# MCG-NKU/E2FGVI

Hardware: AMD Instinct MI355X
Metric: inpainted frames/sec at 432x240 T=10 (higher is better)
Workload: dtype f32; 1 GPU; BASELINE.json configs[1]: e2fgvi 432x240 T=10 l_t=10, 1 clip(s) per GPU per forward (1 in the job), random-init weights, torch.rand frames + box mask (SURVEY.md 8d); clips_per_gpu=1, precision=fp32, kernel_selection=e2fgvi_amd/tile_table.py (checked in, deterministic: ops.py), hip_graph=True, forwards_in_flight=2

## Files before the change

### e2fgvi_amd/csrc/attention_x3.hip

```cpp
#include "common.h"
#include <stdlib.h>

namespace {

constexpr int HD = 128, NH = 4, CQ = 1536, CP = 1024;
constexpr int WS0 = 5, WS1 = 9, WTOK = 45, SLOTS = 210;
constexpr int TK = 32;
constexpr float LOG2E = 1.4426950408889634f;
constexpr int X_KB = TK * HD * 2;
constexpr int X_STAGE = 6 * X_KB;

typedef __bf16 bf16x8 __attribute__((ext_vector_type(8)));
typedef unsigned int u32x4 __attribute__((ext_vector_type(4)));
typedef __attribute__((address_space(3))) void x_lds_void;
typedef int x_i32x4 __attribute__((ext_vector_type(4)));
typedef short s16x4 __attribute__((ext_vector_type(4)));
typedef short s16x8 __attribute__((ext_vector_type(8)));
typedef __attribute__((address_space(3))) s16x4 x_lds_s16x4;

__device__ __forceinline__ void x_dma16(x_i32x4 rsrc, unsigned lds_dst, unsigned voff) {
    unsigned keep;
    asm volatile("s_nop 4\n\ts_mov_b32 %0, m0\n\ts_mov_b32 m0, %3\n\ts_nop 0\n\tbuffer_load_dwordx4 %1, %2, 0 offen lds\n\ts_mov_b32 m0, %0"
                 : "=&s"(keep) : "v"(voff), "s"(rsrc), "s"(lds_dst) : "memory");
}
__device__ __forceinline__ x_i32x4 x_rsrc_words(const void* base, unsigned bytes) {
    const unsigned long long b = (unsigned long long)base;
    x_i32x4 r;
    r[0] = __builtin_amdgcn_readfirstlane((int)(unsigned)b);
    r[1] = __builtin_amdgcn_readfirstlane((int)((unsigned)(b >> 32) & 0xFFFFu));
    r[2] = __builtin_amdgcn_readfirstlane((int)bytes);
    r[3] = 0x00020000;
    return r;
}

__device__ __forceinline__ void x_split8(const f32x4& v0, const f32x4& v1, bf16x8& hi, bf16x8& mid, bf16x8& lo) {
    e2_split8(v0, v1, hi, mid, lo);
}

__global__ void split3_kv_kernel(const float* __restrict__ src, unsigned short* __restrict__ planes, long long rows) {
    const long long idx = (long long)blockIdx.x * blockDim.x + threadIdx.x;
    if (idx >= rows * (CP / 8)) return;
    const long long row = idx / (CP / 8);
    const int c8 = (int)(idx - row * (CP / 8)) * 8;
    const float* s = src + row * CQ + 512 + c8;
    bf16x8 hi, mid, lo;
    x_split8(*reinterpret_cast<const f32x4*>(s), *reinterpret_cast<const f32x4*>(s + 4), hi, mid, lo);
    const long long plane = rows * CP;
    unsigned short* o = planes + row * CP + c8;
    *reinterpret_cast<bf16x8*>(o) = hi;
    *reinterpret_cast<bf16x8*>(o + plane) = mid;
    *reinterpret_cast<bf16x8*>(o + 2 * plane) = lo;
}

template <int NW, int KS>
__global__ __launch_bounds__(64 * NW * KS, 1) void focal_attn_x3_kernel(const float* __restrict__ qkv, const int* __restrict__ key_tab,
                                                                  int tab_ld, const int* __restrict__ nkeys,
                                                                  float* __restrict__ out, int B, int T, int fh, int fw,
                                                                  const char* planes, unsigned planes_bytes, unsigned plane_stride,
                                                                  unsigned pooled_row0) {
#if defined(__HIP_DEVICE_COMPILE__)
    constexpr int NT = 64 * NW;
    constexpr int PIECES = 8 / NW;
    constexpr unsigned OOB = 0xFFFFF000u;
    static_assert(NW == 2 || NW == 4 || NW == 8, "waves per workgroup");
    constexpr int RING = KS == 1 ? 2 * X_STAGE : 9 * X_KB;
    __shared__ __attribute__((aligned(1024))) unsigned char smem[KS * RING];
    __shared__ int stab[256];
    extern __shared__ __attribute__((aligned(16))) unsigned ktab[];

    const int kg = (KS == 1) ? 0 : __builtin_amdgcn_readfirstlane((int)(threadIdx.x / NT));
    const int tid = threadIdx.x - kg * NT;
    const int lane = tid & 63, wave = __builtin_amdgcn_readfirstlane(tid >> 6);
    const int i = lane & 31, h = lane >> 5;
    const int nWw = fw / WS1, nWh = fh / WS0, nWin = nWh * nWw;
    const int nqc = (T * WTOK + 32 * NW - 1) / (32 * NW);
    const int logical = (int)blockIdx.x;
    const int qchunk = logical % nqc;
    const int wh = (logical / nqc) % (nWin * NH);
    const int b = logical / (nqc * nWin * NH);
    const int win = wh / NH, head = wh - win * NH;
    const int wy = win / nWw, wx = win - wy * nWw;
    const int NQ = T * WTOK;
    const int ntok = fh * fw;
    const x_i32x4 rsrc = x_rsrc_words(planes, planes_bytes);

    const int nv = nkeys[win];
    const int NK = T * nv;
    const int ntiles = (NK + TK - 1) / TK;
    const int nIter = (ntiles + KS - 1) / KS;
    const int* tab = key_tab + (long long)win * tab_ld;
    for (int e = threadIdx.x; e < nv && e < 256; e += KS * NT) stab[e] = tab[e];
    __syncthreads();
    {
        int t = 0, sl = threadIdx.x;
        while (sl >= nv) { sl -= nv; ++t; }
        const unsigned head_off = (unsigned)(head * HD * 2);
        for (int k = threadIdx.x; k < KS * nIter * TK; k += KS * NT) {
            unsigned e = OOB;
            if (k < NK) {
                const int ref = stab[sl];
                const bool pooled = ref < 0;
                const unsigned rowi = pooled ? pooled_row0 + (unsigned)((b * T + t) * nWin + (-(ref + 1))) : (unsigned)((b * T + t) * ntok + ref);
                e = rowi * (unsigned)(CP * 2) + head_off;
            }
            ktab[k] = e;
            sl += KS * NT;
            while (sl >= nv) { sl -= nv; ++t; }
        }
    }
    __syncthreads();

    const int q0 = (qchunk * NW + wave) * 32;
// ... 175 lines not shown
        const unsigned char* const ring = smem + kg * RING;
        issue_half(kg, 0u, false);
        issue_half(kg, 6u * X_KB, true);
        asm volatile("s_waitcnt vmcnt(0)" ::: "memory");
        __syncthreads();
        int cur = 0;
        if (kg == 1) __syncthreads();
        for (int itr = 0; itr < nIter; ++itr) {
            const int kt = kg + itr * KS;
            const bool more = itr + 1 < nIter;
            if (more) issue_half(kt + KS, (unsigned)((cur ^ 1) * 3 * X_KB), false);
            if (wave_active) s_phase(ring + cur * 3 * X_KB, kt);
            if (more) asm volatile("s_waitcnt vmcnt(%0)" ::"n"(3 * PIECES) : "memory");
            else asm volatile("s_waitcnt vmcnt(0)" ::: "memory");
            __syncthreads();
            if (wave_active) pv_phase(ring + 6 * X_KB);
            asm volatile("s_waitcnt vmcnt(0)" ::: "memory");
            __syncthreads();
            if (more) issue_half(kt + KS, 6u * X_KB, true);
            cur ^= 1;
        }
        if (kg == 0) __syncthreads();
        float* scr = reinterpret_cast<float*>(smem + RING);
        if (kg > 0) {
            scr[tid] = m_run;
            scr[NT + tid] = l_run;
#pragma unroll
            for (int dt = 0; dt < 4; ++dt)
#pragma unroll
                for (int r = 0; r < 16; ++r) scr[(2 + dt * 16 + r) * NT + tid] = acc[dt][r];
        }
        __syncthreads();
        if (kg > 0) return;
        {
            const float m_o = scr[tid], l_o = scr[NT + tid];
            const float m_new = fmaxf(m_run, m_o);
            const float a0 = __builtin_amdgcn_exp2f(m_run - m_new), a1 = __builtin_amdgcn_exp2f(m_o - m_new);
            l_run = l_run * a0 + l_o * a1;
            m_run = m_new;
#pragma unroll
            for (int dt = 0; dt < 4; ++dt)
#pragma unroll
                for (int r = 0; r < 16; ++r) acc[dt][r] = acc[dt][r] * a0 + scr[(2 + dt * 16 + r) * NT + tid] * a1;
        }
    }

    if (wave_active) {
        float l = l_run + __shfl_xor(l_run, 32);
        const float nmask = (float)(T * (SLOTS - nv));
        l = add_pad_mass(l, nmask, m_run);
        const float inv = 1.f / l;
        bool ok;
        const long long row = query_row(ok);
        if (ok) {
            float* op = out + row * (NH * HD) + head * HD;
#pragma unroll
            for (int dt = 0; dt < 4; ++dt)
#pragma unroll
                for (int rq = 0; rq < 4; ++rq) {
                    const f32x4 v = {acc[dt][rq * 4 + 0] * inv, acc[dt][rq * 4 + 1] * inv, acc[dt][rq * 4 + 2] * inv, acc[dt][rq * 4 + 3] * inv};
                    *reinterpret_cast<f32x4*>(op + dt * 32 + 8 * rq + 4 * h) = v;
                }
        }
    }
#endif
}

}

extern "C" int e2fgvi_split3_kv(const float* qkv_rows, void* planes, int64_t rows, void* stream) {
    E2_REQUIRE(qkv_rows && planes && rows > 0, E2FGVI_EINVAL, "split3_kv: null pointer / no rows");
    E2_REQUIRE(((uintptr_t)qkv_rows & 15) == 0 && ((uintptr_t)planes & 15) == 0, E2FGVI_EINVAL, "split3_kv: buffers must be 16-byte aligned");
    const long long items = rows * (CP / 8);
    hipLaunchKernelGGL(split3_kv_kernel, dim3((unsigned)cdiv64(items, 256)), dim3(256), 0, (hipStream_t)stream, qkv_rows,
                       (unsigned short*)planes, (long long)rows);
    E2_LAUNCH_CHECK("split3_kv");
    return 0;
}

extern "C" int e2fgvi_focal_attention_x3(const float* qkv, const void* planes, const int32_t* key_tab, int32_t tab_ld,
                                         const int32_t* nkeys, float* out, int32_t B, int32_t T, int32_t fh, int32_t fw,
                                         int32_t waves, void* stream) {
    E2_REQUIRE(qkv && planes && key_tab && nkeys && out, E2FGVI_EINVAL, "focal_attention_x3: null pointer");
    E2_REQUIRE(B > 0 && T > 0 && fh > 0 && fw > 0 && fh % WS0 == 0 && fw % WS1 == 0, E2FGVI_EINVAL,
               "focal_attention_x3: token grid %dx%d must be a positive multiple of (5,9)", fh, fw);
    E2_REQUIRE(tab_ld >= SLOTS, E2FGVI_EINVAL, "focal_attention_x3: tab_ld < 210");
    E2_REQUIRE(((uintptr_t)qkv & 15) == 0 && ((uintptr_t)planes & 15) == 0 && ((uintptr_t)out & 15) == 0, E2FGVI_EINVAL,
               "focal_attention_x3: buffers must be 16-byte aligned");
    const int nWin = (fh / WS0) * (fw / WS1);
    const long long rows = (long long)B * T * fh * fw + (long long)B * T * nWin;
    const long long plane_bytes = rows * CP * 2;
    E2_REQUIRE(3 * plane_bytes < 0xFFFFF000LL, E2FGVI_EUNSUP, "focal_attention_x3: the three k / v planes span >= 4 GiB (split the batch)");
    int ks = 1;
    if (waves == 14) { ks = 2; waves = 4; }
    const int ntiles = cdiv(T * SLOTS, TK);
    size_t dyn = (size_t)ntiles * TK * 4;
    const size_t dyn2 = (size_t)cdiv(ntiles, 2) * 2 * TK * 4;
    const bool fits2 = dyn2 + 2 * 9 * X_KB + 1024 + 256 <= 160 * 1024;
    E2_REQUIRE(dyn + 2 * X_STAGE + 1024 + 256 <= 160 * 1024, E2FGVI_EUNSUP, "focal_attention_x3: window of %d frames does not fit the LDS key table", T);
    if (waves <= 0) {
        const long long wg4 = (long long)cdiv(T * WTOK, 128) * nWin * NH * B;
        const long long qblocks = (long long)cdiv(T * WTOK, 32) * nWin * NH * B;
        waves = wg4 >= 512 ? 8 : 4;
        if (wg4 < 192) waves = 2;
        if (waves == 4 && qblocks < 2048 && fits2) ks = 2;
    }
    E2_REQUIRE(waves == 2 || waves == 4 || waves == 8, E2FGVI_EINVAL, "focal_attention_x3: waves must be 0, 2, 4, 8 or 14");
    E2_REQUIRE(ks == 1 || fits2, E2FGVI_EUNSUP, "focal_attention_x3: two key groups do not fit the LDS for a window of %d frames", T);
    if (ks == 2) dyn = dyn2;
    const long long nblk = (long long)cdiv(T * WTOK, 32 * waves) * nWin * NH * B;
    E2_REQUIRE(nblk < 2147483647LL, E2FGVI_EUNSUP, "focal_attention_x3: more than 2^31 workgroups");
    dim3 grid((unsigned)nblk), block(64 * waves * ks);
#define E2_ATT_X3(NW_, KS_)                                                                                                       \
    do {                                                                                                                          \
        hipError_t ea = hipFuncSetAttribute((const void*)focal_attn_x3_kernel<NW_, KS_>, hipFuncAttributeMaxDynamicSharedMemorySize, \
                                            (int)dyn);                                                                            \
        E2_REQUIRE(ea == hipSuccess, (int)ea, "focal_attention_x3: cannot reserve %zu bytes of dynamic LDS", dyn);                \
        hipLaunchKernelGGL((focal_attn_x3_kernel<NW_, KS_>), grid, block, dyn, (hipStream_t)stream, qkv, key_tab, tab_ld, nkeys, out, \
                           B, T, fh, fw, (const char*)planes, (unsigned)(3 * plane_bytes), (unsigned)plane_bytes,                 \
                           (unsigned)((long long)B * T * fh * fw));                                                               \
    } while (0)
    if (ks == 2) E2_ATT_X3(4, 2);
    else if (waves == 2) E2_ATT_X3(2, 1);
    else if (waves == 4) E2_ATT_X3(4, 1);
    else E2_ATT_X3(8, 1);
#undef E2_ATT_X3
    E2_LAUNCH_CHECK("focal_attention_x3");
    return 0;
}
```

### e2fgvi_amd/csrc/common.h

```cpp
#pragma once
#include <hip/hip_runtime.h>
#include <stdint.h>
#include <stdio.h>
#include <stdarg.h>

#include "../../include/e2fgvi_hip.h"

typedef float f32x4 __attribute__((ext_vector_type(4)));
typedef float f32x16 __attribute__((ext_vector_type(16)));

void e2fgvi_set_error(const char* fmt, ...);

#define E2_REQUIRE(cond, code, ...)            \
    do {                                       \
        if (!(cond)) {                         \
            e2fgvi_set_error(__VA_ARGS__);     \
            return (code);                     \
        }                                      \
    } while (0)

#define E2_LAUNCH_CHECK(name)                                                        \
    do {                                                                             \
        hipError_t e__ = hipGetLastError();                                          \
        if (e__ != hipSuccess) {                                                     \
// ... 6 lines not shown
static inline int64_t cdiv64(int64_t a, int64_t b) { return (a + b - 1) / b; }
static inline int round_up(int a, int b) { return cdiv(a, b) * b; }

template <int TM, int TN, int BK, int LDA, int BN>
__device__ __forceinline__ void mma_ktile(const float* __restrict__ sA, const float* __restrict__ sB,
                                          f32x16 (&acc)[TM][TN], int a_row0, int b_col0, int lane) {
    const int i = lane & 31, h = lane >> 5;
#pragma unroll
    for (int m8 = 0; m8 < BK / 8; ++m8) {
        f32x4 a[TM], b[TN];
#pragma unroll
        for (int tm = 0; tm < TM; ++tm)
            a[tm] = *reinterpret_cast<const f32x4*>(sA + (a_row0 + tm * 32 + i) * LDA + (2 * m8 + h) * 4);
#pragma unroll
        for (int tn = 0; tn < TN; ++tn)
            b[tn] = *reinterpret_cast<const f32x4*>(sB + ((2 * m8 + h) * BN + b_col0 + tn * 32 + i) * 4);
#pragma unroll
        for (int e = 0; e < 4; ++e)
#pragma unroll
            for (int tm = 0; tm < TM; ++tm)
#pragma unroll
                for (int tn = 0; tn < TN; ++tn)
                    acc[tm][tn] = __builtin_amdgcn_mfma_f32_32x32x2f32(a[tm][e], b[tn][e], acc[tm][tn], 0, 0, 0);
    }
}

__device__ __forceinline__ int xcd_remap(int bid, int nblk) {
    const int q = nblk >> 3, r = nblk & 7;
    const int xcd = bid & 7, idx = bid >> 3;
    return (xcd < r ? xcd * (q + 1) : r * (q + 1) + (xcd - r) * q) + idx;
}

__device__ __forceinline__ float e2_fast_sigmoid(float x) {
    return __builtin_amdgcn_rcpf(1.f + __builtin_amdgcn_exp2f(-1.4426950408889634f * x));
}
__device__ __forceinline__ float e2_fast_tanh(float x) {
    return 1.f - 2.f * __builtin_amdgcn_rcpf(1.f + __builtin_amdgcn_exp2f(2.8853900817779268f * x));
}

__device__ __forceinline__ float add_pad_mass(float l, float nmask, float m_run) {
    if (nmask > 0.f) l += nmask * __builtin_amdgcn_exp2f(-100.f * 1.4426950408889634f - m_run);
    return l;
}

__device__ __forceinline__ void e2_split2(float x0, float x1, unsigned& H, unsigned& M, unsigned& L) {
    const unsigned b0 = __builtin_bit_cast(unsigned, x0), b1 = __builtin_bit_cast(unsigned, x1);
    const float r0 = x0 - __builtin_bit_cast(float, b0 & 0xFFFF0000u), r1 = x1 - __builtin_bit_cast(float, b1 & 0xFFFF0000u);
    const unsigned rb0 = __builtin_bit_cast(unsigned, r0), rb1 = __builtin_bit_cast(unsigned, r1);
    const float s0 = r0 - __builtin_bit_cast(float, rb0 & 0xFFFF0000u), s1 = r1 - __builtin_bit_cast(float, rb1 & 0xFFFF0000u);
    H = __builtin_amdgcn_perm(b1, b0, 0x07060302u);
    M = __builtin_amdgcn_perm(rb1, rb0, 0x07060302u);
    L = __builtin_amdgcn_perm(__builtin_bit_cast(unsigned, s1), __builtin_bit_cast(unsigned, s0), 0x07060302u);
}
typedef __bf16 e2_bf16x8 __attribute__((ext_vector_type(8)));
typedef unsigned int e2_u32x4 __attribute__((ext_vector_type(4)));
__device__ __forceinline__ void e2_split8(const f32x4& v0, const f32x4& v1, e2_bf16x8& hi, e2_bf16x8& mid, e2_bf16x8& lo) {
    float x[8];
#pragma unroll
    for (int j = 0; j < 4; ++j) { x[j] = v0[j]; x[4 + j] = v1[j]; }
    e2_u32x4 H, M, L;
#pragma unroll
    for (int j = 0; j < 4; ++j) {
        unsigned h, m, l;
        e2_split2(x[2 * j], x[2 * j + 1], h, m, l);
        H[j] = h; M[j] = m; L[j] = l;
    }
    hi = __builtin_bit_cast(e2_bf16x8, H);
    mid = __builtin_bit_cast(e2_bf16x8, M);
    lo = __builtin_bit_cast(e2_bf16x8, L);
}

typedef _Float16 e2_f16x8 __attribute__((ext_vector_type(8)));
template <bool F16> struct e2_h16;
template <> struct e2_h16<false> { typedef __bf16 T; typedef e2_bf16x8 V8; };
template <> struct e2_h16<true> { typedef _Float16 T; typedef e2_f16x8 V8; };
__device__ __forceinline__ f32x16 e2_mfma16(e2_bf16x8 a, e2_bf16x8 b, f32x16 c) {
    return __builtin_amdgcn_mfma_f32_32x32x16_bf16(a, b, c, 0, 0, 0);
}
__device__ __forceinline__ f32x16 e2_mfma16(e2_f16x8 a, e2_f16x8 b, f32x16 c) {
    return __builtin_amdgcn_mfma_f32_32x32x16_f16(a, b, c, 0, 0, 0);
}
template <bool F16> __device__ __forceinline__ float e2_h16_to_f32(unsigned short b) {
    if constexpr (F16) return (float)__builtin_bit_cast(_Float16, b);
    else return __builtin_bit_cast(float, (unsigned)b << 16);
}

__device__ __forceinline__ float apply_act(float v, int act, float slope) {
    if (act == E2FGVI_ACT_RELU) return fmaxf(v, 0.f);
    if (act == E2FGVI_ACT_LRELU) return v > 0.f ? v : v * slope;
    if (act == E2FGVI_ACT_TANH) return tanhf(v);
    return v;
}
```

### e2fgvi_amd/csrc/conv_bf16x.hip

```cpp
#include "common.h"

namespace {

typedef __bf16 bf16x8 __attribute__((ext_vector_type(8)));
typedef unsigned int u32x4 __attribute__((ext_vector_type(4)));
typedef __attribute__((address_space(3))) void lds_void;

struct ConvXParams {
    const void* src[E2FGVI_MAX_SRC];
    int ld[E2FGVI_MAX_SRC];
    int coff[E2FGVI_MAX_SRC];
    int cpg[E2FGVI_MAX_SRC];
    unsigned src_bytes[E2FGVI_MAX_SRC];
    int nsrc;
    int N, H, W, Ho, Wo, KH, KW, stride, pad;
    int padx;
    int osy, osx, opy, opx, oH, oW;
    int res_bcast;
    int Cout, Cout_g, Npad;
    int M;
    int tilesM, tilesN;
    int nsteps;
    unsigned wgroup_bytes;
    long long wgroup_elems;
    const void* w;
    const float* bias;
    const void* res;
    int res_ld, res_coff, res_bf16;
    void* dst;
    int dst_ld, dst_coff, dst_bf16, dst_nchw;
    __bf16* dst2;
    int dst2_ld, dst2_coff;
    int split_from;
    long long split_plane;
    int act;
    float slope;
    int tp_cq;
    unsigned tp_magic;
    unsigned tp_magic_cq;
    int dbg_noload;
};

__device__ __forceinline__ __amdgpu_buffer_rsrc_t make_rsrc(const void* base, unsigned bytes) {
    return __builtin_amdgcn_make_buffer_rsrc(const_cast<void*>(base), 0, (int)bytes, 0x00020000);
}

__device__ __forceinline__ float dcn_post(float v, int co, int C, const f32x4& fl, float max_residue) {
    const int noff = (C / 3) * 2;
    if (co >= noff) return e2_fast_sigmoid(v);
    const int which = (co * 2 >= noff) ? 2 : 0;
    return max_residue * e2_fast_tanh(v) + fl[which + ((co & 1) ? 0 : 1)];
}


__device__ __forceinline__ void split8(const f32x4& v0, const f32x4& v1, bf16x8& hi, bf16x8& mid, bf16x8& lo) {
    e2_split8(v0, v1, hi, mid, lo);
}

typedef int pp_i32x4 __attribute__((ext_vector_type(4)));
__device__ __forceinline__ pp_i32x4 pp_rsrc_words(const void* base, unsigned bytes) {
    const unsigned long long b = (unsigned long long)base;
    pp_i32x4 r;
    r[0] = __builtin_amdgcn_readfirstlane((int)(unsigned)b);
    r[1] = __builtin_amdgcn_readfirstlane((int)((unsigned)(b >> 32) & 0xFFFFu));
    r[2] = __builtin_amdgcn_readfirstlane((int)bytes);
    r[3] = 0x00020000;
    return r;
}
__device__ __forceinline__ void pp_dma16(pp_i32x4 rsrc, unsigned lds_dst, unsigned voff, unsigned soff) {
    unsigned keep;
    asm volatile("s_nop 4\n\ts_mov_b32 %0, m0\n\ts_mov_b32 m0, %3\n\ts_nop 0\n\tbuffer_load_dwordx4 %1, %2, %4 offen lds\n\ts_mov_b32 m0, %0"
                 : "=&s"(keep) : "v"(voff), "s"(rsrc), "s"(lds_dst), "s"(soff) : "memory");
}

template <int BM, int BN, int WGM, int WGN, bool S3, int MODE, bool PP = false>
__global__ __launch_bounds__(64 * WGM * WGN) void conv_bf16x_kernel(const ConvXParams p) {
#if defined(__HIP_DEVICE_COMPILE__)
    constexpr bool F32 = MODE == 1, X3 = MODE == 2, F16 = MODE == 3;
    typedef typename e2_h16<F16>::T E16;
    typedef typename e2_h16<F16>::V8 e16x8;
    static_assert(!PP || (X3 && !S3 && WGM * WGN == 8), "ping-pong halves: split-operand mode, 8 waves, no row-shift stages");
    constexpr int NT = 64 * WGM * WGN;
    constexpr int ESZ = (F32 || X3) ? 4 : 2;
    constexpr int CH = 16 / ESZ;
    constexpr int KC = 8 * CH;
    constexpr int TM = BM / (32 * WGM), TN = BN / (32 * WGN);
    constexpr int AR = S3 ? BM + 2 : BM;
    constexpr int B_CH = X3 ? 12 : 8;
    constexpr int A_BYTES = AR * 128, B_BYTES = BN * B_CH * 16;
    constexpr int A_IT = (AR * 8 + NT - 1) / NT, B_IT = (BN * B_CH + NT - 1) / NT;
    constexpr bool A_PART = (AR * 8) % NT != 0;
    constexpr bool B_PART = (BN * B_CH) % NT != 0;
    constexpr int R = TM * 32, CN = TN * 32;
    constexpr int ES = (WGM * WGN * R * (CN + 4) * 4 <= 150 * 1024) ? 1 : (TN % 2 == 0 ? 2 : TN);
    constexpr int TNH = TN / ES, CNH = CN / ES, LDE = CNH + 4;
    constexpr int EPI = WGM * WGN * R * LDE * 4;
    static_assert(TN % ES == 0 && EPI <= 160 * 1024, "epilogue region");
    constexpr int SMEM = 2 * (A_BYTES + B_BYTES) > EPI ? 2 * (A_BYTES + B_BYTES) : EPI;
    constexpr unsigned OOB = 0xFFFFFFFFu;
    static_assert(TM >= 1 && TN >= 1 && (BM * 8) % NT == 0 && (BN * B_CH) % 64 == 0 && SMEM <= 160 * 1024, "tile");

    __shared__ __attribute__((aligned(1024))) unsigned char smem[SMEM];

    const int tid = threadIdx.x;
    const int lane = tid & 63, wave = __builtin_amdgcn_readfirstlane(tid >> 6);
    const int wm = wave / WGN, wn = wave % WGN;
    const int g = blockIdx.y;
    const int logical = xcd_remap(blockIdx.x, p.tilesM * p.tilesN);
    const int tile_m = logical / p.tilesN, tile_n = logical - tile_m * p.tilesN;
    const int m0 = tile_m * BM, n0 = tile_n * BN;
    const int HoWo = p.Ho * p.Wo;

    int a_pix[A_IT];
    unsigned a_msk[A_IT];
    unsigned a_ch16[A_IT];
#pragma unroll
    for (int it = 0; it < A_IT; ++it) {
        const int item = tid + it * NT;
        const int row = item >> 3, slot = item & 7;
        a_ch16[it] = (unsigned)((slot ^ ((row >> 1) & 7)) * 16);
        const int m = S3 ? m0 + row - 1 : m0 + row;
        const bool ok = m >= 0 && m < p.M;
        const int mm = ok ? m : 0;
        const int img = mm / HoWo;
        const int rem = mm - img * HoWo;
        const int oy = rem / p.Wo, ox = rem - oy * p.Wo;
        const int by = oy * p.stride - p.pad;
        const int bx = S3 ? ox : ox * p.stride - p.padx;
        unsigned msk = 0;
        for (int k = 0; k < p.KH; ++k) msk |= ((unsigned)(by + k) < (unsigned)p.H ? 1u : 0u) << k;
        for (int k = 0; k < (S3 ? 1 : p.KW); ++k) msk |= ((unsigned)(bx + k) < (unsigned)p.W ? 1u : 0u) << (8 + k);
        a_msk[it] = ok ? msk : 0u;
        a_pix[it] = (img * p.H + by) * p.W + bx;
    }
    unsigned b_off[B_IT];
#pragma unroll
    for (int it = 0; it < B_IT; ++it) {
        const int item = tid + it * NT;
        const int koct = item / BN, n = item - koct * BN;
        b_off[it] = ((n0 + n) < p.Npad && koct < B_CH) ? (unsigned)((koct * p.Npad + n0 + n) * 16) : OOB;
    }
    const __amdgpu_buffer_rsrc_t wrsrc = make_rsrc(reinterpret_cast<const char*>(p.w) + (long long)g * p.wgroup_bytes, p.wgroup_bytes);
    const unsigned b_step = (unsigned)B_CH * (unsigned)p.Npad * 16u;

    const void* const sp0 = p.src[0]; const void* const sp1 = p.src[1]; const void* const sp2 = p.src[2]; const void* const sp3 = p.src[3];
    const unsigned sb0 = p.src_bytes[0], sb1 = p.src_bytes[1], sb2 = p.src_bytes[2], sb3 = p.src_bytes[3];
    const unsigned sl0 = (unsigned)p.ld[0] * ESZ, sl1 = (unsigned)p.ld[1] * ESZ, sl2 = (unsigned)p.ld[2] * ESZ, sl3 = (unsigned)p.ld[3] * ESZ;
    const unsigned sc0 = (unsigned)(p.coff[0] + g * p.cpg[0]) * ESZ, sc1 = (unsigned)(p.coff[1] + g * p.cpg[1]) * ESZ,
                   sc2 = (unsigned)(p.coff[2] + g * p.cpg[2]) * ESZ, sc3 = (unsigned)(p.coff[3] + g * p.cpg[3]) * ESZ;
    const int sg0 = p.cpg[0], sg1 = p.cpg[1], sg2 = p.cpg[2], sg3 = p.cpg[3];
    int ky = 0, kx = 0, s = 0, c0 = 0;
    int blk = 0;
    const void* cur_src = sp0;
    unsigned cur_bytes = sb0;
    unsigned cur_ld2 = sl0, cur_chan = sc0;
    int cur_cpg = sg0;
    unsigned a_off[A_IT];
    auto retarget = [&]() {
        if (p.nsrc > 1) {
            cur_src = s == 0 ? sp0 : s == 1 ? sp1 : s == 2 ? sp2 : sp3;
            cur_bytes = s == 0 ? sb0 : s == 1 ? sb1 : s == 2 ? sb2 : sb3;
            cur_ld2 = s == 0 ? sl0 : s == 1 ? sl1 : s == 2 ? sl2 : sl3;
            cur_chan = s == 0 ? sc0 : s == 1 ? sc1 : s == 2 ? sc2 : sc3;
            cur_cpg = s == 0 ? sg0 : s == 1 ? sg1 : s == 2 ? sg2 : sg3;
        }
        const int kxe = S3 ? 0 : kx;
        const int tap = ky * p.W + kxe;
#pragma unroll
        for (int it = 0; it < A_IT; ++it) {
            const bool ok = ((a_msk[it] >> ky) & (a_msk[it] >> (8 + kxe)) & 1u) != 0;
            a_off[it] = ok ? (unsigned)(a_pix[it] + tap) * cur_ld2 + cur_chan + a_ch16[it] : OOB;
        }
    };
    retarget();
    unsigned char* const smem_b = smem + 2 * A_BYTES;
    auto issue_a = [&](int stage) {
        if (p.dbg_noload & 16) return;
        unsigned char* sa = smem + stage * A_BYTES + wave * 1024;
        const __amdgpu_buffer_rsrc_t arsrc = make_rsrc(cur_src, cur_bytes);
        const unsigned soff = (unsigned)c0 * (unsigned)ESZ;
        if (c0 + KC <= cur_cpg) {
#pragma unroll
            for (int it = 0; it < A_IT; ++it)
                if (!A_PART || it + 1 < A_IT || tid + it * NT < AR * 8)
                    __builtin_amdgcn_raw_ptr_buffer_load_lds(arsrc, (lds_void*)(sa + it * NT * 16), 16, a_off[it], soff, 0, 0);
        } else {
#pragma unroll
            for (int it = 0; it < A_IT; ++it)
                if (!A_PART || it + 1 < A_IT || tid + it * NT < AR * 8)
                    __builtin_amdgcn_raw_ptr_buffer_load_lds(arsrc, (lds_void*)(sa + it * NT * 16), 16,
                                                             (c0 + (int)(a_ch16[it] / ESZ) < cur_cpg) ? a_off[it] : OOB, soff, 0, 0);
        }
    };
    auto issue_b = [&](int stage, int step) {
        if (p.dbg_noload & 32) return;
        unsigned char* sb = smem_b + stage * B_BYTES + wave * 1024;
        const unsigned soff = (unsigned)step * b_step;
#pragma unroll
        for (int it = 0; it < B_IT; ++it)
            if (!B_PART || it + 1 < B_IT || tid + it * NT < BN * B_CH)
                __builtin_amdgcn_raw_ptr_buffer_load_lds(wrsrc, (lds_void*)(sb + it * NT * 16), 16, b_off[it], soff, 0, 0);
    };
    auto advance = [&]() -> bool {
        c0 += KC;
        ++blk;
        if (c0 < cur_cpg) return false;
        c0 = 0;
        ++s;
        if (s == p.nsrc) {
            s = 0;
            blk = 0;
            if (S3) ++ky;
            else { ++kx; if (kx == p.KW) { kx = 0; ++ky; } }
        }
        return true;
    };

    f32x16 acc[TM][TN];
#pragma unroll
    for (int tm = 0; tm < TM; ++tm)
#pragma unroll
        for (int tn = 0; tn < TN; ++tn)
#pragma unroll
            for (int r = 0; r < 16; ++r) acc[tm][tn][r] = 0.f;

    const int i = lane & 31, h = lane >> 5;
    int a_row[TM], b_rd[TN];
    bool okl[TM], okr[TM];
#pragma unroll
    for (int tm = 0; tm < TM; ++tm) {
        a_row[tm] = (wm * TM + tm) * 32 + i;
        const int ox = (m0 + a_row[tm]) % p.Wo;
        okl[tm] = ox != 0;
        okr[tm] = ox != p.Wo - 1;
    }
#pragma unroll
    for (int tn = 0; tn < TN; ++tn) b_rd[tn] = ((wn * TN + tn) * 32 + i) * 16;

    auto compute = [&](const unsigned char* st, const unsigned char* stb, int kxs) {
        int a_rd[TM], a_key[TM];
        bool zero[TM];
#pragma unroll
        for (int tm = 0; tm < TM; ++tm) {
            const int row = a_row[tm] + (S3 ? kxs : 0);
            a_rd[tm] = row * 128;
            a_key[tm] = (row >> 1) & 7;
            zero[tm] = S3 && ((kxs == 0 && !okl[tm]) || (kxs == 2 && !okr[tm]));
        }
        if constexpr (X3) {
#pragma unroll
            for (int kk = 0; kk < 2; ++kk) {
                const int q = 2 * kk + h;
                bf16x8 ah[TM], am[TM], al[TM];
#pragma unroll
                for (int tm = 0; tm < TM; ++tm)
                    split8(*reinterpret_cast<const f32x4*>(st + a_rd[tm] + (((2 * q) ^ a_key[tm]) << 4)),
                           *reinterpret_cast<const f32x4*>(st + a_rd[tm] + (((2 * q + 1) ^ a_key[tm]) << 4)), ah[tm], am[tm], al[tm]);
#pragma unroll
                for (int tn = 0; tn < TN; ++tn) {
                    const bf16x8 bh = *reinterpret_cast<const bf16x8*>(stb + b_rd[tn] + q * (BN * 16));
                    const bf16x8 bm = *reinterpret_cast<const bf16x8*>(stb + b_rd[tn] + (4 + q) * (BN * 16));
                    const bf16x8 bl = *reinterpret_cast<const bf16x8*>(stb + b_rd[tn] + (8 + q) * (BN * 16));
#pragma unroll
                    for (int tm = 0; tm < TM; ++tm) acc[tm][tn] = __builtin_amdgcn_mfma_f32_32x32x16_bf16(al[tm], bh, acc[tm][tn], 0, 0, 0);
#pragma unroll
                    for (int tm = 0; tm < TM; ++tm) acc[tm][tn] = __builtin_amdgcn_mfma_f32_32x32x16_bf16(ah[tm], bl, acc[tm][tn], 0, 0, 0);
#pragma unroll
                    for (int tm = 0; tm < TM; ++tm) acc[tm][tn] = __builtin_amdgcn_mfma_f32_32x32x16_bf16(am[tm], bm, acc[tm][tn], 0, 0, 0);
#pragma unroll
                    for (int tm = 0; tm < TM; ++tm) acc[tm][tn] = __builtin_amdgcn_mfma_f32_32x32x16_bf16(am[tm], bh, acc[tm][tn], 0, 0, 0);
#pragma unroll
                    for (int tm = 0; tm < TM; ++tm) acc[tm][tn] = __builtin_amdgcn_mfma_f32_32x32x16_bf16(ah[tm], bm, acc[tm][tn], 0, 0, 0);
#pragma unroll
                    for (int tm = 0; tm < TM; ++tm) acc[tm][tn] = __builtin_amdgcn_mfma_f32_32x32x16_bf16(ah[tm], bh, acc[tm][tn], 0, 0, 0);
                }
            }
        } else {
#pragma unroll
        for (int kk = 0; kk < 4; ++kk) {
            if constexpr (F32) {
                f32x4 a[TM], b[TN];
#pragma unroll
                for (int tm = 0; tm < TM; ++tm)
                    a[tm] = *reinterpret_cast<const f32x4*>(st + a_rd[tm] + (((2 * kk + h) ^ a_key[tm]) << 4));
#pragma unroll
                for (int tn = 0; tn < TN; ++tn)
                    b[tn] = *reinterpret_cast<const f32x4*>(stb + b_rd[tn] + (2 * kk + h) * (BN * 16));
#pragma unroll
                for (int e = 0; e < 4; ++e)
#pragma unroll
                    for (int tm = 0; tm < TM; ++tm)
#pragma unroll
                        for (int tn = 0; tn < TN; ++tn)
                            acc[tm][tn] = __builtin_amdgcn_mfma_f32_32x32x2f32(a[tm][e], b[tn][e], acc[tm][tn], 0, 0, 0);
            } else {
                e16x8 a[TM], b[TN];
#pragma unroll
                for (int tm = 0; tm < TM; ++tm) {
                    a[tm] = *reinterpret_cast<const e16x8*>(st + a_rd[tm] + (((2 * kk + h) ^ a_key[tm]) << 4));
                    if (S3) {
                        u32x4 q = __builtin_bit_cast(u32x4, a[tm]);
#pragma unroll
                        for (int e = 0; e < 4; ++e) q[e] = zero[tm] ? 0u : q[e];
                        a[tm] = __builtin_bit_cast(e16x8, q);
                    }
                }
#pragma unroll
                for (int tn = 0; tn < TN; ++tn)
                    b[tn] = *reinterpret_cast<const e16x8*>(stb + b_rd[tn] + (2 * kk + h) * (BN * 16));
#pragma unroll
// ... 58 lines not shown
                for (int tm = 0; tm < TM; ++tm) acc[tm][tn] = __builtin_amdgcn_mfma_f32_32x32x16_bf16(fa[tm][0], bh, acc[tm][tn], 0, 0, 0);
                __builtin_amdgcn_sched_barrier(0);
            }
        };
        const unsigned smem_lds = (unsigned)(unsigned long long)(lds_void*)smem;
        const pp_i32x4 wrsrc_w = pp_rsrc_words(reinterpret_cast<const char*>(p.w) + (long long)g * p.wgroup_bytes, p.wgroup_bytes);
        auto pp_issue = [&](int stage, int step) __attribute__((always_inline)) {
            const pp_i32x4 arsrc_w = pp_rsrc_words(cur_src, cur_bytes);
            const unsigned soff = (unsigned)__builtin_amdgcn_readfirstlane(c0 * ESZ);
            const unsigned la = smem_lds + (unsigned)(stage * A_BYTES + wave * 1024);
            const bool whole = c0 + KC <= cur_cpg;
#pragma unroll
            for (int it = 0; it < A_IT; ++it)
                pp_dma16(arsrc_w, (unsigned)__builtin_amdgcn_readfirstlane((int)(la + it * NT * 16)),
                         (whole || c0 + (int)(a_ch16[it] / ESZ) < cur_cpg) ? a_off[it] : OOB, soff);
            const unsigned lb = smem_lds + (unsigned)(2 * A_BYTES + stage * B_BYTES + wave * 1024);
            const unsigned sb = (unsigned)__builtin_amdgcn_readfirstlane((int)((unsigned)step * b_step));
#pragma unroll
            for (int it = 0; it < B_IT; ++it)
                if (!B_PART || it + 1 < B_IT || tid + it * NT < BN * B_CH)
                    pp_dma16(wrsrc_w, (unsigned)__builtin_amdgcn_readfirstlane((int)(lb + it * NT * 16)), b_off[it], sb);
        };
        if (trail) pp_bar();
        for (int step = 0; step < p.nsteps; ++step) {
            const int cur = step & 1;
            const unsigned char* const sA = smem + cur * A_BYTES;
            const unsigned char* const sB = smem_b + cur * B_BYTES;
            if (trail) { if (step + 1 < p.nsteps) { if (advance()) retarget(); pp_issue((step & 1) ^ 1, step + 1); } }
            prep(sA, 0);
            pp_bar();
            mma(sB, 0);
            pp_bar();
            prep(sA, 1);
            if (!trail) { if (step + 1 < p.nsteps) { if (advance()) retarget(); pp_issue((step & 1) ^ 1, step + 1); } }
            if (trail) asm volatile("s_waitcnt vmcnt(0)" ::: "memory");
            pp_bar();
            mma(sB, 1);
            if (!trail) asm volatile("s_waitcnt vmcnt(0)" ::: "memory");
            pp_bar();
        }
        if (!trail) pp_bar();
    } else
    if constexpr (!S3) {
        if (p.tp_cq) {
            const int cq = p.tp_cq, KK = p.KH * p.KW;
            int t_c[A_IT];
#pragma unroll
            for (int it = 0; it < A_IT; ++it) t_c[it] = (int)(a_ch16[it] >> 4);
            const __amdgpu_buffer_rsrc_t arsrc = make_rsrc(sp0, sb0);
            auto issue_a_packed = [&](int stage, int step) {
                unsigned char* sa = smem + stage * A_BYTES + wave * 1024;
#pragma unroll
                for (int it = 0; it < A_IT; ++it) {
                    const int L = 8 * step + t_c[it];
                    const int tap = cq == 1 ? L : (int)__umulhi((unsigned)L, p.tp_magic_cq);
                    const int cc = L - tap * cq;
                    const int tky = (int)__umulhi((unsigned)tap, p.tp_magic), tkx = tap - tky * p.KW;
                    const bool ok = tap < KK && ((a_msk[it] >> tky) & (a_msk[it] >> (8 + tkx)) & 1u) != 0;
                    const unsigned off = ok ? (unsigned)(a_pix[it] + tky * p.W + tkx) * sl0 + sc0 + (unsigned)cc * 16u : OOB;
                    __builtin_amdgcn_raw_ptr_buffer_load_lds(arsrc, (lds_void*)(sa + it * NT * 16), 16, off, 0, 0, 0);
                }
            };
            issue_a_packed(0, 0);
            asm volatile("s_waitcnt vmcnt(0)" ::: "memory");
            __syncthreads();
            for (int step = 0; step < p.nsteps; ++step) {
                const int cur = step & 1;
                if (step + 1 < p.nsteps) {
                    issue_a_packed(cur ^ 1, step + 1);
                    issue_b(cur ^ 1, step + 1);
                }
                compute(smem + cur * A_BYTES, smem_b + cur * B_BYTES, 0);
                asm volatile("s_waitcnt vmcnt(0)" ::: "memory");
                __syncthreads();
            }
        } else
        for (int step = 0; step < p.nsteps; ++step) {
            const int cur = step & 1;
            const bool more = step + 1 < p.nsteps && !(p.dbg_noload & 1);
            if (more) {
                if (advance()) retarget();
                issue_a(cur ^ 1);
                issue_b(cur ^ 1, step + 1);
            }
            compute(smem + cur * A_BYTES, smem_b + cur * B_BYTES, 0);
            asm volatile("s_waitcnt vmcnt(0)" ::: "memory");
            __syncthreads();
        }
    } else if constexpr (!S3) {
        for (int step = 0; step < p.nsteps; ++step) {
            const int cur = step & 1;
            const bool more = step + 1 < p.nsteps && !(p.dbg_noload & 1);
            if (more) {
                if (advance()) retarget();
                issue_a(cur ^ 1);
                issue_b(cur ^ 1, step + 1);
            }
            compute(smem + cur * A_BYTES, smem_b + cur * B_BYTES, 0);
            asm volatile("s_waitcnt vmcnt(0)" ::: "memory");
            __syncthreads();
        }
    } else {
        const int spt = p.nsteps / 9;
        int acur = 0, kxs = 0;
        for (int step = 0; step < p.nsteps; ++step) {
            const bool more = step + 1 < p.nsteps && !(p.dbg_noload & 1);
            int kxn = kxs + 1;
            bool newblk = false;
            if (kxn == 3) {
                kxn = 0;
                if (more) { if (advance()) retarget(); newblk = true; }
            }
// ... 282 lines not shown
    if (idx >= p.total) return;
    const int g = (int)(idx / p.wgroup_elems);
    long long rem = idx - (long long)g * p.wgroup_elems;
    const int e = (int)(rem % p.ch);
    rem /= p.ch;
    const int n = (int)(rem % p.Npad);
    rem /= p.Npad;
    const int koct = (int)(rem & 7);
    const int step = (int)(rem >> 3);
    wp[idx] = (T)pack_value(w, p, g, step, koct, n, e);
}

__global__ void pack_conv_weight_x3_kernel(const float* __restrict__ w, unsigned short* __restrict__ wp, const PackX p) {
    const long long idx = (long long)blockIdx.x * blockDim.x + threadIdx.x;
    if (idx >= p.total) return;
    const int g = (int)(idx / p.wgroup_elems);
    long long rem = idx - (long long)g * p.wgroup_elems;
    const int e = (int)(rem & 3);
    rem >>= 2;
    const int n = (int)(rem % p.Npad);
    rem /= p.Npad;
    const int koct = (int)(rem & 7);
    const int step = (int)(rem >> 3);
    const float v = pack_value(w, p, g, step, koct, n, e);
    const unsigned xb = __builtin_bit_cast(unsigned, v);
    const float r = v - __builtin_bit_cast(float, xb & 0xFFFF0000u);
    const unsigned rb = __builtin_bit_cast(unsigned, r);
    const float r2 = r - __builtin_bit_cast(float, rb & 0xFFFF0000u);
    const long long plane = 4LL * p.Npad * 8;
    unsigned short* o = wp + (long long)g * p.wgroup_elems * 3 + (long long)step * 3 * plane +
                        ((long long)(koct >> 1) * p.Npad + n) * 8 + (koct & 1) * 4 + e;
    o[0] = (unsigned short)(xb >> 16);
    o[plane] = (unsigned short)(rb >> 16);
    o[2 * plane] = (unsigned short)(__builtin_bit_cast(unsigned, r2) >> 16);
}

template <int BM, int BN, int WGM, int WGN, bool S3, bool PP = false>
int launch_x(ConvXParams& p, int groups, hipStream_t st, int mode = 0) {
    p.tilesM = cdiv(p.M, BM);
    p.tilesN = cdiv(p.Cout_g, BN);
    if constexpr (PP) {
        if (mode != 2 || p.tp_cq) {
            e2fgvi_set_error("conv2d_x: the ping-pong tiles (107, 108) are for the split-operand mode without tap-packed weights");
            return E2FGVI_EUNSUP;
        }
        hipLaunchKernelGGL((conv_bf16x_kernel<BM, BN, WGM, WGN, false, 2, true>), dim3(p.tilesM * p.tilesN, groups, 1), dim3(64 * WGM * WGN), 0, st, p);
        E2_LAUNCH_CHECK("conv2d_x");
        return 0;
    } else {
    if (S3 && !(p.KH == 3 && p.KW == 3 && p.stride == 1 && p.pad == 1)) {
        e2fgvi_set_error("conv2d_x: the row-shift tiles (11..17) are for 3x3 stride-1 pad-1 layers");
        return E2FGVI_EINVAL;
    }
    if (mode == 1 || mode == 2) {
        if constexpr (!S3) {
            if (mode == 2)
                hipLaunchKernelGGL((conv_bf16x_kernel<BM, BN, WGM, WGN, false, 2>), dim3(p.tilesM * p.tilesN, groups, 1), dim3(64 * WGM * WGN), 0, st, p);
            else
                hipLaunchKernelGGL((conv_bf16x_kernel<BM, BN, WGM, WGN, false, 1>), dim3(p.tilesM * p.tilesN, groups, 1), dim3(64 * WGM * WGN), 0, st, p);
        } else {
            e2fgvi_set_error("conv2d_x: the row-shift tiles (11..18) take bf16 operands only");
            return E2FGVI_EUNSUP;
        }
    } else if (mode == 3) {
        hipLaunchKernelGGL((conv_bf16x_kernel<BM, BN, WGM, WGN, S3, 3>), dim3(p.tilesM * p.tilesN, groups, 1), dim3(64 * WGM * WGN), 0, st, p);
    } else {
        hipLaunchKernelGGL((conv_bf16x_kernel<BM, BN, WGM, WGN, S3, 0>), dim3(p.tilesM * p.tilesN, groups, 1), dim3(64 * WGM * WGN), 0, st, p);
    }
    E2_LAUNCH_CHECK("conv2d_x");
    return 0;
    }
}

}

static bool geometry_taps(int Cout, int KH, int KW, int cin, PackX* q, bool f32 = false) {
    const int32_t cpg[1] = {cin};
    if (cin > 56 || KW < 2 || !geometry_x(Cout, 1, KH, KW, 1, cpg, q, f32)) return false;
    q->tp_cq = cin / q->ch;
    const int steps = cdiv(KH * KW * q->tp_cq, 8);
    q->wgroup_elems = (long long)steps * q->kc * q->Npad;
    q->total = q->wgroup_elems;
    return true;
}

static int mode_x(const char* who, int32_t code) {
    switch (code) {
        case E2FGVI_BF16: return 0;
        case E2FGVI_F32: return 1;
        case E2FGVI_BF16X3: return 2;
        case E2FGVI_F16: return 3;
        default: break;
    }
    e2fgvi_set_error("%s: mode %d is none of E2FGVI_F32 (0), E2FGVI_BF16 (1), E2FGVI_BF16X3 (2), E2FGVI_F16 (3)", who, code);
    return -1;
}

static bool pack_geometry(const char* who, int mode, int tap_packed, int Cout, int groups, int KH, int KW, int nsrc,
                          const int32_t* src_cpg, PackX* q) {
    const bool f32 = mode == 1 || mode == 2;
    const int ch = f32 ? 4 : 8;
    if (!src_cpg) {
        e2fgvi_set_error("%s: null src_cpg", who);
        return false;
    }
    if (tap_packed) {
        if (groups == 1 && nsrc == 1 && geometry_taps(Cout, KH, KW, src_cpg[0], q, f32)) return true;
        e2fgvi_set_error("%s: tap-packed weights: one source of %d ... 56 channels (multiple of %d), no groups, KW >= 2", who, ch, ch);
        return false;
    }
    if (geometry_x(Cout, groups, KH, KW, nsrc, src_cpg, q, f32)) return true;
    e2fgvi_set_error("%s: bad geometry (channels per source must be multiples of %d)", who, ch);
    return false;
}

extern "C" int64_t e2fgvi_packed_conv_weight_x_size(int32_t mode, int32_t tap_packed, int32_t Cout, int32_t groups, int32_t KH,
                                                    int32_t KW, int32_t nsrc, const int32_t* src_cpg) {
    PackX q;
    const int m = mode_x("packed_conv_weight_x_size", mode);
    if (m < 0 || !pack_geometry("packed_conv_weight_x_size", m, tap_packed, Cout, groups, KH, KW, nsrc, src_cpg, &q)) return E2FGVI_EINVAL;
    return m == 2 ? 3 * q.total : q.total;
}

extern "C" int e2fgvi_pack_conv_weight_x(const float* w, void* wpacked, int32_t mode, int32_t tap_packed, int32_t Cout, int32_t groups,
                                         int32_t KH, int32_t KW, int32_t nsrc, const int32_t* src_cpg, void* stream) {
    PackX q;
    E2_REQUIRE(w && wpacked, E2FGVI_EINVAL, "pack_conv_weight_x: null pointer");
    const int m = mode_x("pack_conv_weight_x", mode);
    if (m < 0 || !pack_geometry("pack_conv_weight_x", m, tap_packed, Cout, groups, KH, KW, nsrc, src_cpg, &q)) return E2FGVI_EINVAL;
    const dim3 grid((unsigned)cdiv64(q.total, 256)), block(256);
    hipStream_t st = (hipStream_t)stream;
    switch (m) {
        case 0: hipLaunchKernelGGL(pack_conv_weight_x_kernel<__bf16>, grid, block, 0, st, w, (__bf16*)wpacked, q); break;
        case 1: hipLaunchKernelGGL(pack_conv_weight_x_kernel<float>, grid, block, 0, st, w, (float*)wpacked, q); break;
        case 2: hipLaunchKernelGGL(pack_conv_weight_x3_kernel, grid, block, 0, st, w, (unsigned short*)wpacked, q); break;
        default: hipLaunchKernelGGL(pack_conv_weight_x_kernel<_Float16>, grid, block, 0, st, w, (_Float16*)wpacked, q); break;
    }
    E2_LAUNCH_CHECK("pack_conv_weight_x");
    return 0;
}

static int conv2d_x(const e2fgvi_convx_desc* d, void* stream, int mode) {
    const bool f32 = mode == 1 || mode == 2;
    const int dt16 = mode == 3 ? E2FGVI_F16 : E2FGVI_BF16;
    E2_REQUIRE(d, E2FGVI_EINVAL, "conv2d_x: null descriptor");
    PackX q;
    const int esz = f32 ? 4 : 2;
    const int wbytes_num = mode == 2 ? 6 : esz;
    E2_REQUIRE(geometry_x(d->Cout, d->groups, d->KH, d->KW, d->nsrc, d->src_cpg, &q, f32), E2FGVI_EINVAL,
               "conv2d_x: bad geometry (channels per source must be multiples of 8 bf16 / 4 fp32)");
    E2_REQUIRE(d->N > 0 && d->H > 0 && d->W > 0 && d->Ho > 0 && d->Wo > 0 && d->stride > 0 && d->pad >= 0, E2FGVI_EINVAL,
               "conv2d_x: bad sizes");
    if (d->out_grid) {
        E2_REQUIRE(d->pad_left >= 0 && d->act != E2FGVI_ACT_DCNPOST && !d->dst_nchw && !d->tap_packed && (d->tile < 10 || d->tile > 20),
                   E2FGVI_EINVAL, "conv2d_x: explicit output grids take plain NHWC tiles only");
        if (d->out_sy || d->out_sx)
            E2_REQUIRE(d->out_sy > 0 && d->out_sx > 0 && d->out_py >= 0 && d->out_px >= 0 && d->out_H > 0 && d->out_W > 0 &&
                       (d->Ho - 1) * d->out_sy + d->out_py < d->out_H && (d->Wo - 1) * d->out_sx + d->out_px < d->out_W &&
                       (long long)d->N * d->out_H * d->out_W < 2147483647LL,
                       E2FGVI_EINVAL, "conv2d_x: the output scatter leaves the [N, out_H, out_W] image");
    } else {
        E2_REQUIRE(d->Ho == (d->H + 2 * d->pad - d->KH) / d->stride + 1 && d->Wo == (d->W + 2 * d->pad - d->KW) / d->stride + 1,
                   E2FGVI_EINVAL, "conv2d_x: Ho/Wo inconsistent with H/W/k/stride/pad");
        E2_REQUIRE(!d->out_sy && !d->out_sx && !d->pad_left, E2FGVI_EINVAL, "conv2d_x: pad_left / out_s* need out_grid = 1");
    }
    E2_REQUIRE(!d->res_bcast || (d->residual && d->act != E2FGVI_ACT_DCNPOST), E2FGVI_EINVAL, "conv2d_x: res_bcast without a residual");
    E2_REQUIRE((long long)d->N * d->Ho * d->Wo < 2147483647LL, E2FGVI_EUNSUP, "conv2d_x: more than 2^31 output pixels");
    E2_REQUIRE(d->KH <= 8 && d->KW <= 8, E2FGVI_EUNSUP, "conv2d_x: kernels larger than 8x8 are not supported");
    E2_REQUIRE(d->wpacked && d->dst, E2FGVI_EINVAL, "conv2d_x: null weight/dst");
    E2_REQUIRE((d->dst_dtype == E2FGVI_F32 || d->dst_dtype == dt16) && (d->res_dtype == E2FGVI_F32 || d->res_dtype == dt16),
               E2FGVI_EINVAL, mode == 3 ? "conv2d_x: dtype must be E2FGVI_F32 or E2FGVI_F16"
                                        : "conv2d_x: dtype must be E2FGVI_F32 or E2FGVI_BF16");
    ConvXParams p;
    for (int s = 0; s < E2FGVI_MAX_SRC; ++s) { p.src[s] = nullptr; p.ld[s] = 0; p.coff[s] = 0; p.cpg[s] = 0; p.src_bytes[s] = 0; }
    for (int s = 0; s < d->nsrc; ++s) {
        E2_REQUIRE(d->src[s], E2FGVI_EINVAL, "conv2d_x: null source %d", s);
        E2_REQUIRE(d->src_ld[s] % q.ch == 0 && d->src_coff[s] % q.ch == 0 && ((uintptr_t)d->src[s] & 15) == 0, E2FGVI_EINVAL,
                   "conv2d_x: source %d not 16-byte addressable (ld / coff multiples of 8 bf16 / 4 fp32)", s);
        E2_REQUIRE(d->src_coff[s] + d->groups * d->src_cpg[s] <= d->src_ld[s], E2FGVI_EINVAL,
                   "conv2d_x: source %d channel range exceeds its pixel stride", s);
        const long long bytes = (long long)d->N * d->H * d->W * d->src_ld[s] * esz;
        E2_REQUIRE(bytes < 4294967295LL, E2FGVI_EUNSUP, "conv2d_x: source %d spans >= 4 GiB (split the batch)", s);
        p.src[s] = d->src[s]; p.ld[s] = d->src_ld[s]; p.coff[s] = d->src_coff[s]; p.cpg[s] = d->src_cpg[s];
        p.src_bytes[s] = (unsigned)bytes;
    }
    E2_REQUIRE(q.wgroup_elems * wbytes_num < 4294967295LL, E2FGVI_EUNSUP, "conv2d_x: packed weight group >= 4 GiB");
    E2_REQUIRE(((uintptr_t)d->wpacked & 15) == 0, E2FGVI_EINVAL, "conv2d_x: packed weight not 16-byte aligned");
    if (d->dst_nchw)
        E2_REQUIRE(d->dst_dtype == E2FGVI_F32 && !d->dst2, E2FGVI_EINVAL, "conv2d_x: the NCHW destination is fp32, without a second copy");
    else
        E2_REQUIRE(d->dst_coff >= 0 && d->dst_coff + d->Cout <= d->dst_ld, E2FGVI_EINVAL, "conv2d_x: dst slice exceeds dst_ld");
    E2_REQUIRE(((uintptr_t)d->dst & 15) == 0 && (!d->dst2 || ((uintptr_t)d->dst2 & 15) == 0) &&
               (!d->residual || ((uintptr_t)d->residual & 15) == 0), E2FGVI_EINVAL, "conv2d_x: dst / dst2 / residual not 16-byte aligned");
    E2_REQUIRE(mode != 3 || !d->dst2_plane_stride, E2FGVI_EINVAL, "conv2d_x: no split planes (dst2 is an fp16 copy)");
    if (d->dst2_plane_stride) {
        E2_REQUIRE(d->dst2 && d->dst2_plane_stride > 0 && d->dst_dtype == E2FGVI_F32 && !d->dst_nchw && d->groups == 1 &&
                       !(d->out_grid && d->out_sy), E2FGVI_EINVAL,
                   "conv2d_x: split planes need dst2, an fp32 NHWC dst, groups = 1 and no output scatter");
        E2_REQUIRE(d->Cout % 8 == 0 && d->dst2_split_from >= 0 && d->dst2_split_from <= d->Cout && d->dst2_split_from % 8 == 0 &&
                       d->dst2_ld % 8 == 0 && d->dst2_coff % 8 == 0 && d->dst2_plane_stride % 8 == 0 && d->dst2_coff >= 0 &&
                       d->dst2_coff + d->Cout - d->dst2_split_from <= d->dst2_ld, E2FGVI_EINVAL,
                   "conv2d_x: split planes: Cout, dst2_split_from, dst2_ld, dst2_coff and dst2_plane_stride in multiples of 8, "
                   "the split channels inside dst2_ld");
    } else if (d->dst2)
        E2_REQUIRE(d->dst2_coff >= 0 && d->dst2_coff + d->Cout <= d->dst2_ld, E2FGVI_EINVAL, "conv2d_x: dst2 slice exceeds dst2_ld");
    if (d->act == E2FGVI_ACT_DCNPOST)
        E2_REQUIRE(d->residual && d->res_dtype == E2FGVI_F32 && d->Cout % 3 == 0 && d->groups == 1, E2FGVI_EINVAL,
                   "conv2d_x: ACT_DCNPOST needs the fp32 [pixel][4] flows as residual, Cout %% 3 == 0, groups == 1");
    p.nsrc = d->nsrc;
    p.N = d->N; p.H = d->H; p.W = d->W; p.Ho = d->Ho; p.Wo = d->Wo;
    p.KH = d->KH; p.KW = d->KW; p.stride = d->stride; p.pad = d->pad;
    p.padx = d->out_grid ? d->pad_left : d->pad;
    p.osy = d->out_grid ? d->out_sy : 0; p.osx = d->out_sx; p.opy = d->out_py; p.opx = d->out_px; p.oH = d->out_H; p.oW = d->out_W;
    p.res_bcast = d->res_bcast;
    p.Cout = d->Cout; p.Cout_g = q.Cout_g; p.Npad = q.Npad;
    p.M = d->N * d->Ho * d->Wo;
    p.nsteps = d->KH * d->KW * q.steps_per_tap;
    p.tp_cq = 0; p.tp_magic = 0; p.tp_magic_cq = 0;
    if (d->tap_packed) {
        PackX qt;
        E2_REQUIRE(d->nsrc == 1 && d->groups == 1 && geometry_taps(d->Cout, d->KH, d->KW, d->src_cpg[0], &qt, f32), E2FGVI_EINVAL,
                   "conv2d_x: tap-packed weights are for one source of <= 56 channels, no groups, KW >= 2");
        E2_REQUIRE(d->tile < 10 || d->tile > 20, E2FGVI_EUNSUP, "conv2d_x: the row-shift tiles do not take tap-packed weights");
        q.wgroup_elems = qt.wgroup_elems;
        p.tp_cq = qt.tp_cq;
        p.tp_magic = 0xFFFFFFFFu / (unsigned)d->KW + 1u;
        p.tp_magic_cq = qt.tp_cq > 1 ? 0xFFFFFFFFu / (unsigned)qt.tp_cq + 1u : 0u;
        p.nsteps = cdiv(d->KH * d->KW * qt.tp_cq, 8);
    }
    p.wgroup_elems = q.wgroup_elems; p.wgroup_bytes = (unsigned)(q.wgroup_elems * wbytes_num);
    p.w = d->wpacked; p.bias = d->bias;
    p.res = d->residual; p.res_ld = d->res_ld; p.res_coff = d->res_coff; p.res_bf16 = d->res_dtype == dt16;
    p.dst = d->dst; p.dst_ld = d->dst_ld; p.dst_coff = d->dst_coff; p.dst_bf16 = d->dst_dtype == dt16;
    p.dst_nchw = d->dst_nchw;
    p.dst2 = (__bf16*)d->dst2; p.dst2_ld = d->dst2_ld; p.dst2_coff = d->dst2_coff;
    p.split_from = d->dst2_split_from; p.split_plane = d->dst2_plane_stride;
    p.act = d->act; p.slope = d->slope;
    hipStream_t st = (hipStream_t)stream;
    int tile = d->tile;
    p.dbg_noload = 0;
    if (tile == 21 || tile == 24 || tile == 26 || tile == 27) { p.dbg_noload = 1; tile -= 20; }
    if (tile == 31 || tile == 34 || tile == 36) { p.dbg_noload = 2; tile -= 30; }
    if (tile == 41 || tile == 44 || tile == 46) { p.dbg_noload = 3; tile -= 40; }
    if (tile == 61 || tile == 66) { p.dbg_noload = 8; tile -= 60; }
    if (tile == 71 || tile == 74 || tile == 76 || tile == 77) { p.dbg_noload = 16; tile -= 70; }
    if (tile == 81 || tile == 84 || tile == 86 || tile == 87) { p.dbg_noload = 32; tile -= 80; }
    if (!tile) {
        if (p.Cout_g <= 32) tile = 3;
        else if (p.Cout_g <= 64) tile = 2;
        else tile = ((long long)cdiv(p.M, 128) * cdiv(p.Cout_g, 128) * d->groups >= 384) ? 1 : 4;
    }
    switch (tile) {
        case 1: return launch_x<128, 128, 2, 2, false>(p, d->groups, st, mode);
        case 2: return launch_x<128, 64, 2, 2, false>(p, d->groups, st, mode);
        case 3: return launch_x<128, 32, 4, 1, false>(p, d->groups, st, mode);
        case 4: return launch_x<64, 128, 2, 2, false>(p, d->groups, st, mode);
        case 5: return launch_x<64, 64, 2, 2, false>(p, d->groups, st, mode);
        case 6: return launch_x<256, 128, 4, 2, false>(p, d->groups, st, mode);
        case 7: return launch_x<256, 256, 4, 2, false>(p, d->groups, st, mode);
        case 8: return launch_x<256, 192, 4, 2, false>(p, d->groups, st, mode);
        case 107: return launch_x<256, 256, 4, 2, false, true>(p, d->groups, st, mode);
        case 108: return launch_x<256, 192, 4, 2, false, true>(p, d->groups, st, mode);
        case 11: return launch_x<128, 128, 2, 2, true>(p, d->groups, st, mode);
        case 12: return launch_x<128, 64, 2, 2, true>(p, d->groups, st, mode);
        case 13: return launch_x<128, 32, 4, 1, true>(p, d->groups, st, mode);
        case 14: return launch_x<64, 128, 2, 2, true>(p, d->groups, st, mode);
        case 16: return launch_x<256, 128, 4, 2, true>(p, d->groups, st, mode);
        case 17: return launch_x<256, 256, 4, 2, true>(p, d->groups, st, mode);
        case 18: return launch_x<256, 64, 4, 2, true>(p, d->groups, st, mode);
        default: break;
    }
    e2fgvi_set_error("conv2d_x: unknown tile %d", tile);
    return E2FGVI_EINVAL;
}

extern "C" int e2fgvi_conv2d_x(const e2fgvi_convx_desc* d, int32_t mode, void* stream) {
    const int m = mode_x("conv2d_x", mode);
    return m < 0 ? E2FGVI_EINVAL : conv2d_x(d, stream, m);
}
```

### e2fgvi_amd/csrc/misc.hip

```cpp
#include "common.h"

#include <type_traits>

namespace {

constexpr int NTH = 256;

typedef unsigned int u32x2 __attribute__((ext_vector_type(2)));
typedef __bf16 bf16x4 __attribute__((ext_vector_type(4)));
typedef _Float16 f16x4 __attribute__((ext_vector_type(4)));
typedef _Float16 f16x8 __attribute__((ext_vector_type(8)));
template <typename T> __device__ __forceinline__ f32x4 ld4(const T* p);
template <> __device__ __forceinline__ f32x4 ld4<float>(const float* p) { return *reinterpret_cast<const f32x4*>(p); }
template <> __device__ __forceinline__ f32x4 ld4<__bf16>(const __bf16* p) {
    const u32x2 q = *reinterpret_cast<const u32x2*>(p);
    f32x4 v = {__builtin_bit_cast(float, q[0] << 16), __builtin_bit_cast(float, q[0] & 0xFFFF0000u),
               __builtin_bit_cast(float, q[1] << 16), __builtin_bit_cast(float, q[1] & 0xFFFF0000u)};
    return v;
}
template <> __device__ __forceinline__ f32x4 ld4<_Float16>(const _Float16* p) {
    const f16x4 h = *reinterpret_cast<const f16x4*>(p);
    f32x4 v = {(float)h[0], (float)h[1], (float)h[2], (float)h[3]};
    return v;
}
// ... 690 lines not shown
            hipLaunchKernelGGL((prop_cond_kernel<T, T>), dim3(blocks_for(total)), dim3(NTH), 0, (hipStream_t)stream,
                               (const T*)feat_prop, fp_ld, (const T*)feat_n2, f2_ld, flow_a, flow_b, (long long)flow_img_stride,
                               (T*)cond, flows, (T*)flows8_bf16, N, H, W, C);
    });
    E2_LAUNCH_CHECK("prop_cond");
    return 0;
}

template <typename TO>
static int layernorm_launch(const float* x, const float* gamma, const float* beta, TO* y, int64_t rows, int32_t C, hipStream_t st) {
    const int wpb = 4;
    dim3 grid((unsigned)cdiv64(rows, wpb)), block(64 * wpb);
    switch (C / 256) {
        case 1: hipLaunchKernelGGL((layernorm_kernel<1, TO>), grid, block, 0, st, x, gamma, beta, y, (long long)rows, C); break;
        case 2: hipLaunchKernelGGL((layernorm_kernel<2, TO>), grid, block, 0, st, x, gamma, beta, y, (long long)rows, C); break;
        case 3: hipLaunchKernelGGL((layernorm_kernel<3, TO>), grid, block, 0, st, x, gamma, beta, y, (long long)rows, C); break;
        default: hipLaunchKernelGGL((layernorm_kernel<4, TO>), grid, block, 0, st, x, gamma, beta, y, (long long)rows, C); break;
    }
    E2_LAUNCH_CHECK("layernorm");
    return 0;
}
extern "C" int e2fgvi_layernorm(const float* x, const float* gamma, const float* beta, void* y, int32_t y_dtype, int64_t rows,
                                int32_t C, void* stream) {
    E2_REQUIRE(x && gamma && beta && y && rows > 0 && E2_DT_OK(y_dtype), E2FGVI_EINVAL, "layernorm: bad arguments");
    E2_REQUIRE(C == 256 || C == 512 || C == 768 || C == 1024, E2FGVI_EUNSUP, "layernorm: C must be 256/512/768/1024");
    int rc = 0;
    with_dtype(y_dtype, [&](auto z) { rc = layernorm_launch(x, gamma, beta, (E2_ELEM(z)*)y, rows, C, (hipStream_t)stream); });
    return rc;
}

extern "C" int e2fgvi_window_pool(const void* x, int32_t dtype, const float* w45, const float* bias1, void* pooled,
                                  int32_t BT, int32_t fh, int32_t fw, int32_t C, void* stream) {
    E2_REQUIRE(x && w45 && bias1 && pooled && BT > 0 && fh > 0 && fw > 0 && fh % 5 == 0 && fw % 9 == 0 && C % 4 == 0 &&
                   E2_DT_OK(dtype),
               E2FGVI_EINVAL, "window_pool: bad arguments");
    E2_REQUIRE(dtype == E2FGVI_F32 || C % 8 == 0, E2FGVI_EINVAL, "window_pool: 16-bit needs C %% 8 == 0");
    const long long total = (long long)BT * (fh / 5) * (fw / 9) * (C / (E2_DT16(dtype) ? 8 : 4));
    with_dtype(dtype, [&](auto z) {
        using T = E2_ELEM(z);
        hipLaunchKernelGGL(window_pool_kernel<T>, dim3(blocks_for(total)), dim3(NTH), 0, (hipStream_t)stream,
                           (const T*)x, w45, bias1, (T*)pooled, BT, fh, fw, C);
    });
    E2_LAUNCH_CHECK("window_pool");
    return 0;
}

static int check_fold(const char* name, int F, int fh, int fw, int H, int W, int C) {
    E2_REQUIRE(F > 0 && C > 0 && C % 4 == 0, E2FGVI_EINVAL, "%s: bad arguments", name);
    E2_REQUIRE(fh == (H + 6 - 7) / 3 + 1 && fw == (W + 6 - 7) / 3 + 1, E2FGVI_EINVAL,
               "%s: token grid %dx%d inconsistent with %dx%d", name, fh, fw, H, W);
    return 0;
}

extern "C" int e2fgvi_ffn_fold(const void* hid, void* folded, int32_t dtype, int32_t gelu, int32_t F, int32_t fh, int32_t fw,
                               int32_t H, int32_t W, int32_t C, void* stream) {
    const char* name = gelu ? "ffn_fold_gelu" : "ffn_fold";
    E2_REQUIRE(hid && folded && E2_DT_OK(dtype), E2FGVI_EINVAL, "%s: bad arguments", name);
    if (int rc = check_fold(name, F, fh, fw, H, W, C)) return rc;
    E2_REQUIRE(dtype == E2FGVI_F32 || C % 8 == 0, E2FGVI_EINVAL, "%s: 16-bit needs C %% 8 == 0", name);
    const long long total = (long long)F * H * W * (C / (E2_DT16(dtype) ? 8 : 4));
    with_dtype(dtype, [&](auto z) {
        using T = E2_ELEM(z);
        if (gelu)
            hipLaunchKernelGGL((fold_kernel<true, T, T, T, true>), dim3(blocks_for(total)), dim3(NTH), 0, (hipStream_t)stream,
                               (const T*)hid, (const float*)nullptr, (const T*)nullptr, (T*)folded, F, fh, fw, H, W, C);
        else
            hipLaunchKernelGGL((fold_kernel<true, T, T, T>), dim3(blocks_for(total)), dim3(NTH), 0, (hipStream_t)stream,
                               (const T*)hid, (const float*)nullptr, (const T*)nullptr, (T*)folded, F, fh, fw, H, W, C);
    });
    E2_LAUNCH_CHECK(name);
    return 0;
}

extern "C" int e2fgvi_ffn_unfold(const void* folded, void* out, int32_t dtype, int32_t gelu, int32_t F, int32_t fh, int32_t fw,
                                 int32_t H, int32_t W, int32_t C, void* stream) {
    const char* name = gelu ? "ffn_unfold_gelu" : "ffn_unfold";
    E2_REQUIRE(folded && out && E2_DT_OK(dtype), E2FGVI_EINVAL, "%s: bad arguments", name);
    if (int rc = check_fold(name, F, fh, fw, H, W, C)) return rc;
    E2_REQUIRE(dtype == E2FGVI_F32 || C % 8 == 0, E2FGVI_EINVAL, "%s: 16-bit needs C %% 8 == 0", name);
    const long long total = (long long)F * fh * fw * 49 * (C / (E2_DT16(dtype) ? 8 : 4));
    with_dtype(dtype, [&](auto z) {
        using T = E2_ELEM(z);
        if (gelu)
            hipLaunchKernelGGL(unfold_gelu_kernel<T>, dim3(blocks_for(total)), dim3(NTH), 0, (hipStream_t)stream,
                               (const T*)folded, (T*)out, F, fh, fw, H, W, C);
        else
            hipLaunchKernelGGL((unfold_gelu_kernel<T, false>), dim3(blocks_for(total)), dim3(NTH), 0, (hipStream_t)stream,
                               (const T*)folded, (T*)out, F, fh, fw, H, W, C);
    });
    E2_LAUNCH_CHECK(name);
    return 0;
}

extern "C" int e2fgvi_softcomp_fold(const void* emb, const float* bias_hwc, const void* residual, void* dst, int32_t dtype, int32_t F,
                                    int32_t fh, int32_t fw, int32_t H, int32_t W, int32_t C, void* stream) {
    E2_REQUIRE(emb && dst, E2FGVI_EINVAL, "softcomp_fold: null pointer");
    E2_REQUIRE(E2_DT_OK(dtype), E2FGVI_EINVAL, "softcomp_fold: dtype must be E2FGVI_F32, E2FGVI_BF16 or E2FGVI_F16");
    if (int rc = check_fold("softcomp_fold", F, fh, fw, H, W, C)) return rc;
    E2_REQUIRE(dtype == E2FGVI_F32 || C % 8 == 0, E2FGVI_EINVAL, "softcomp_fold: C %% 8 != 0");
    const long long total = (long long)F * H * W * (C / (E2_DT16(dtype) ? 8 : 4));
    with_dtype(dtype, [&](auto z) {
        using T = E2_ELEM(z);
        hipLaunchKernelGGL((fold_kernel<false, T, T, T>), dim3(blocks_for(total)), dim3(NTH), 0, (hipStream_t)stream,
                           (const T*)emb, bias_hwc, (const T*)residual, (T*)dst, F, fh, fw, H, W, C);
    });
    E2_LAUNCH_CHECK("softcomp_fold");
    return 0;
}

extern "C" int e2fgvi_cast(const void* src, int32_t src_dtype, void* dst, int32_t dst_dtype, int64_t n, void* stream) {
    E2_REQUIRE(src && dst && n > 0 && n % 4 == 0 && E2_DT_OK(src_dtype) && E2_DT_OK(dst_dtype) &&
                   (src_dtype == E2FGVI_F32) != (dst_dtype == E2FGVI_F32) && (((uintptr_t)src | (uintptr_t)dst) & 7) == 0,
// ... 40 lines not shown
```

### e2fgvi_amd/engine.py

```python
import numpy as np
import os

import torch

from . import ops
from .ops import ACT_DCNPOST, ACT_LRELU, ACT_RELU, ACT_TANH, PackedConvX

BF16 = torch.bfloat16
F16 = torch.float16
FC2_CONV = ops.X3_ENABLED
WIN = (5, 9)
JOIN_AT = int(os.environ.get("E2FGVI_JOIN_AT", "0") or 0)
if JOIN_AT not in (0, 10, 12, 14, 16, 18):
    raise ValueError("E2FGVI_JOIN_AT=%d: the join sits in front of encoder.layers.10 / 12 / 14 / 16 or behind the encoder (18)" % JOIN_AT)
PROP_SPLIT = os.environ.get("E2FGVI_PROP_SPLIT", "1") != "0"


def token_grid(h, w):
    return (h + 6 - 7) // 3 + 1, (w + 6 - 7) // 3 + 1


def build_key_table(fh, fw, valid_ind_rolled):
    nwh, nww = fh // WIN[0], fw // WIN[1]
    ex = (WIN[0] // 2, WIN[1] // 2)
    shifts = ((-ex[0], -ex[1]), (-ex[0], ex[1]), (ex[0], -ex[1]), (ex[0], ex[1]))
    vi = [int(v) for v in valid_ind_rolled]
    tab = np.zeros((nwh * nww, 212), np.int32)
    nk = np.zeros((nwh * nww,), np.int32)
    for wy in range(nwh):
        for wx in range(nww):
            refs = []
            for p in range(45):
                refs.append((wy * 5 + p // 9) * fw + wx * 9 + p % 9)
            for v in vi:
                n, p = divmod(v, 45)
                sy, sx = shifts[n]
                y = (wy * 5 + p // 9 - sy) % fh
                x = (wx * 9 + p % 9 - sx) % fw
                refs.append(y * fw + x)
            for ki in range(5):
                for kj in range(9):
                    py, px = wy - 2 + ki, wx - 4 + kj
                    if 0 <= py < nwh and 0 <= px < nww:
                        refs.append(-(py * nww + px + 1))
            w = wy * nww + wx
            nk[w] = len(refs)
            tab[w, :len(refs)] = refs
    return tab, nk


def split_prop_weights(w_off0, w_bb0, ch=128):
    return dict(off_rec=torch.cat([w_off0[:, :ch], w_off0[:, 2 * ch:]], 1).contiguous(), off_cur=w_off0[:, ch:2 * ch].contiguous(),
                bb_rec=w_bb0[:, -ch:].contiguous(), bb_pre=w_bb0[:, :-ch].contiguous())


class Engine:
    def __init__(self, state_dict, model="e2fgvi", device="cuda", precision="fp32", winograd=True, autotune=True):
        if precision not in ("fp32", "bf16", "fp16"):
            raise ValueError("precision must be 'fp32', 'bf16' or 'fp16'")
        self.precision = precision
        self.hq = model == "e2fgvi_hq"
        self.device = torch.device(device)
        sd = {k: v.detach().to(self.device) for k, v in state_dict.items()}
        self.sd = sd
        f = lambda k: sd[k].float().contiguous()
        self.x16 = x16 = precision in ("bf16", "fp16")
        self.dtype = {"bf16": BF16, "fp16": F16}.get(precision, torch.float32)
        x3 = not x16 and ops.X3_ENABLED
# ... 49 lines not shown
            if PROP_SPLIT and not x16:
                ws = split_prop_weights(f(p + "conv_offset.0.weight"), f(b + "0.weight"))
                self.prop_split[d] = dict(
                    off_rec=layer("deform_align.%sconv_offset.0 (recurrent part)" % d, None, [128, 128, 4], w=ws["off_rec"],
                                  b=f(p + "conv_offset.0.bias"), pad=1),
                    off_cur=layer("deform_align.%sconv_offset.0 (current-frame part)" % d, None, [128], w=ws["off_cur"], pad=1),
                    bb_rec=layer("backbone.%s0 (recurrent part)" % d, None, [128], w=ws["bb_rec"], b=f(b + "0.bias"), pad=1),
                    bb_pre=layer("backbone.%s0 (non-recurrent part)" % d, None, [128] * (nparts - 1), w=ws["bb_pre"], pad=1))
        self.fusion = layer("fusion", "feat_prop_module.fusion", [128, 128], tune=True)

        self.ss = layer("ss.embedding", "ss.embedding", [128], w=f("ss.embedding.weight").view(512, 128, 7, 7), stride=3, pad=3,
                        tune=True)
        wsc = f("sc.embedding.weight").view(128, 49, 512).permute(1, 0, 2).reshape(6272, 512).contiguous()
        bsc = f("sc.embedding.bias").view(128, 49).t().reshape(6272).contiguous()
        self.sc = layer("sc.embedding", None, w=wsc, b=bsc, tune=True)
        self.sc_bias_conv = layer("sc.bias_conv", "sc.bias_conv", [128], pad=1) if self.hq else None
        self.sc_bias_hwc = None if self.hq else f("sc.bias").permute(1, 2, 0).contiguous()
        self.sc_gather = (ops.SoftCompGather(f("sc.embedding.weight"), f("sc.embedding.bias"), 128, dtype=self.dtype)
                          if x16 and self.hq else None)

        self.blocks = []
        for i in range(8):
            p = "transformer.%d." % i
            w1 = f(p + "mlp.conv1.0.weight").view(40, 49, 512).permute(1, 0, 2).reshape(1960, 512).contiguous()
            b1 = f(p + "mlp.conv1.0.bias").view(40, 49).t().reshape(1960).contiguous()
            if FC2_CONV or x16:
                fc2 = layer(p + "fc2", p + "mlp.conv2.1", [40], w=f(p + "mlp.conv2.1.weight").view(512, 40, 7, 7), stride=3, pad=3,
                            taps=True, tune=True)
            else:
                w2 = f(p + "mlp.conv2.1.weight").view(512, 40, 49).permute(0, 2, 1).reshape(512, 1960).contiguous()
                fc2 = layer(p + "fc2", p + "mlp.conv2.1", w=w2, tune=True)
            self.blocks.append(dict(
                pool_w=f(p + "pool_layers.0.weight").view(45), pool_b=f(p + "pool_layers.0.bias"),
                n1w=f(p + "norm1.weight"), n1b=f(p + "norm1.bias"), n2w=f(p + "norm2.weight"), n2b=f(p + "norm2.bias"),
                qkv=layer(p + "qkv", p + "attn.qkv", tune=True),
                proj=layer(p + "proj", p + "attn.proj", tune=True),
                fc1=layer(p + "fc1", None, w=w1, b=b1, tune=True),
                fc2=fc2,
                valid=sd[p + "attn.valid_ind_rolled"].cpu().tolist()))

        self.spy = [[layer("spynet.%d.%d" % (lv, j), "update_spynet.basic_module.%d.basic_module.%d.conv" % (lv, j), [cin], pad=3,
                           nopk=True)
                     for j, cin in enumerate((8, 32, 64, 32, 16))] for lv in range(6)]
        mean = f("update_spynet.mean").view(3)
        std = f("update_spynet.std").view(3)
        one = torch.ones(1, device=self.device)
        self.spy_scale = torch.cat([1.0 / std, one]).contiguous()
        self.spy_shift = torch.cat([-mean / std, 0 * one]).contiguous()
        self.half = torch.full((4,), 0.5, device=self.device)
        self._tables = {}
        self._zeros = {}
        self.overlap_flows = True
        self._side = None
        self._given = None
        self.counters = {"encoder_frames": 0, "flow_pairs": 0, "decoder_frames": 0}
        torch.cuda.synchronize(self.device)

    def weight_bytes(self):
        seen, total = set(), 0

        def walk(o):
            nonlocal total
            if id(o) in seen:
                return
            seen.add(id(o))
            if isinstance(o, (list, tuple)):
                for v in o:
                    walk(v)
            elif isinstance(o, dict):
                for v in o.values():
                    walk(v)
            elif hasattr(o, "weight_bytes") and o is not self:
                total += o.weight_bytes()
            elif isinstance(getattr(o, "wpacked", None), torch.Tensor):
                total += o.wpacked.numel() * o.wpacked.element_size()
            elif hasattr(o, "__dict__") and type(o).__module__.startswith("e2fgvi_amd") and o is not self:
                walk(list(vars(o).values()))
        walk(list(vars(self).values()))
        return total

    def _fork_ok(self):
        return self.overlap_flows and not torch.cuda.is_current_stream_capturing()

    def _side_stream(self):
        if self._side is None:
            self._side = {}
        key = torch.cuda.current_stream(self.device).cuda_stream
        if key not in self._side:
            self._side[key] = torch.cuda.Stream(device=self.device)
        return self._side[key]

    def _zero(self, shape, dtype=torch.float32):
        return ops._lazy(self._zeros, (dtype,) + tuple(shape), "zero buffer %s" % (tuple(shape),),
                         lambda: torch.zeros(tuple(shape), dtype=dtype, device=self.device))

    def _table(self, fh, fw, blk):
        key = (fh, fw, tuple(blk["valid"]))
        if key not in self._tables:
            tab, nk = build_key_table(fh, fw, blk["valid"])
            self._tables[key] = (torch.from_numpy(tab).to(self.device), torch.from_numpy(nk).to(self.device))
        return self._tables[key]

    def pair_table(self, pairs):
        ref = [int(i) for i, _ in pairs]
        supp = [int(j) for _, j in pairs]
        return torch.tensor([ref + supp, supp + ref], dtype=torch.int32, device=self.device)
# ... 109 lines not shown
            beside([("off backward_", sb["off_cur"], [lb]), ("bb backward_", sb["bb_pre"], [lb]), ("off forward_", sf["off_cur"], [lf])])

        def partial(key, slot):
            ev = ready.pop(key, None)
            if ev is not None:
                main.wait_event(ev)
            return pre[key][slot]
        for name, flows in (("backward_", flows_a), ("forward_", flows_b)):
            off_convs, dcn, bb = self.prop[name]
            sp = self.prop_split.get(name) if split else None
            if sp is not None and name == "forward_":
                beside([("bb forward_", sp["bb_pre"], [lf, flat(feats["backward_"][1:])])])
            store = torch.empty((l_t, b, h, w, ch), dtype=self.dtype, device=dev)
            order = list(range(l_t))
            if name == "backward_":
                order = order[::-1]
            img_stride = (l_t - 1) * h * w * 2
            hist = []
            hist_dcn = [] if x16 else hist
            aligned = zero
            for i, idx in enumerate(order):
                cur = loc[idx]
                if i > 0:
                    flow_a = flows[0, i - 1]
                    flow_b = flows[0, i - 2] if i > 1 else None
                    feat_n2 = hist[-2] if i > 1 else None
                    if x16:
                        cond, fl, fl_src = ops.prop_cond(hist[-1], feat_n2, flow_a, flow_b, img_stride, cond_dtype=self.dtype, flows8=True)
                    else:
                        cond, fl = ops.prop_cond(hist[-1], feat_n2, flow_a, flow_b, img_stride)
                        fl_src = fl
                    if sp is not None:
                        slot = idx if name == "backward_" else idx - 1
                        x = sp["off_rec"]([(cond, 0), (cond, ch), fl], residual=partial("off " + name, slot), **lk)
                    else:
                        x = off_convs[0]([(cond, 0), cur, (cond, ch), fl_src], **lk)
                    x = off_convs[1]([x], **lk)
                    x = off_convs[2]([x], **lk)
                    offs = off_convs[3]([x], out_dtype=torch.float32, residual=fl, act=ACT_DCNPOST, slope=10.0)
                    aligned = dcn([hist_dcn[-1], hist_dcn[-2] if i > 1 else zero_dcn], offs, out_dtype=self.dtype, planar=x16)
                if sp is not None and i > 0:
                    y = sp["bb_rec"]([aligned], residual=partial("bb " + name, idx if name == "backward_" else idx - 1), **lk)
                else:
                    srcs = [cur, feats["backward_"][idx], aligned] if name == "forward_" else [cur, aligned]
                    y = bb[0](srcs, **lk)
                hist.append(bb[1]([y], residual=aligned, out=store[idx]))
                if x16 and i + 1 < l_t:
                    hist_dcn.append(ops.to_planar16(store[idx]))
            feats[name] = store
        out = self.fusion([feats["backward_"].view(l_t * b, h, w, ch), feats["forward_"].view(l_t * b, h, w, ch)],
                          residual=loc.view(l_t * b, h, w, ch), out=loc.view(l_t * b, h, w, ch) if inplace else None)
        return out.view(l_t, b, h, w, ch)

    def soft_split(self, feat):
        return self.ss([feat], out_dtype=torch.float32)

    def block(self, i, x, b, t, fh, fw, hw, out2=None):
        blk = self.blocks[i]
        H, W = hw
        tab, nk = self._table(fh, fw, blk)
        rows = x.shape[0]
        prow = b * t * (fh // 5) * (fw // 9)
        nbuf = torch.empty((rows + prow, 512), dtype=self.dtype, device=x.device)
        n1 = ops.layernorm(x, blk["n1w"], blk["n1b"], out=nbuf[:rows])
        ops.window_pool(n1, blk["pool_w"], blk["pool_b"], b * t, fh, fw, out=nbuf[rows:])
        if self.x16:
            both = blk["qkv"](nbuf)
            att = ops.focal_attention_bf16(both[:rows], both[rows:], tab, nk, b, t, fh, fw)
        elif ops.attention_x3_applies(b, t, fh, fw):
            planes = torch.empty((3, rows + prow, 1024), dtype=torch.bfloat16, device=x.device)
            both = blk["qkv"](nbuf, kv_planes=planes)
            att = ops.focal_attention_x3(both[:rows], planes, tab, nk, b, t, fh, fw)
        else:
            both = blk["qkv"](nbuf)
            att = ops.focal_attention(both[:rows], both[rows:], tab, nk, b, t, fh, fw)
        x1 = blk["proj"](att, out_dtype=torch.float32, residual=x)
        n2 = ops.layernorm(x1, blk["n2w"], blk["n2b"], out_dtype=self.dtype)
        hid = blk["fc1"](n2)
        folded = ops.ffn_fold_gelu(hid, b * t, fh, fw, H, W, 40)
        if isinstance(blk["fc2"], PackedConvX):
            y = torch.empty((rows, 512), dtype=torch.float32, device=x.device)
            blk["fc2"]([folded], out=y.view(b * t, fh, fw, 512), residual=x1.view(b * t, fh, fw, 512),
                       out2=None if out2 is None else out2.view(b * t, fh, fw, 512))
            return y, x1
        unf = ops.ffn_unfold(folded, fh, fw, out=hid)
        return blk["fc2"](unf, residual=x1), x1

    def compose(self, tokens, enc, b, t, fh, fw):
        _, h, w, ch = enc.shape
        if self.sc_gather is not None and (h, w) == (3 * fh, 3 * fw):
            folded = self.sc_gather(tokens.view(b * t, fh, fw, 512))
            return self.sc_bias_conv([folded], residual=enc)
        emb = self.sc(tokens)
        if self.hq:
            folded = ops.softcomp_fold(emb, b * t, fh, fw, h, w, ch)
            return self.sc_bias_conv([folded], residual=enc)
        return ops.softcomp_fold(emb, b * t, fh, fw, h, w, ch, bias_hwc=self.sc_bias_hwc, residual=enc)

    def decode(self, x):
        n, h, w, _ = x.shape
        self.counters["decoder_frames"] += n
        lr = dict(act=ACT_LRELU, slope=0.2)
        d = self.dec
        x = ops.resize_bilinear(x, (2 * h, 2 * w), True)
        x = d[0]([x], **lr)
        x = d[1]([x], **lr)
        x = ops.resize_bilinear(x, (4 * h, 4 * w), True)
        x = d[2]([x], **lr)
        return d[3]([x], act=ACT_TANH, out_nchw=True)

    def forward(self, frames, l_t, trace=None, given=None, decode_local=False):
        if given is None:
            given = self._given
        if frames is None:
            if given is None:
                raise ValueError("frames may be None only with given=((fwd, bwd), enc)")
            (g_fwd, _), g_enc = given
            b = g_fwd.shape[0]
            t, c, H, W = g_enc.shape[0] // b, 3, 4 * g_enc.shape[1], 4 * g_enc.shape[2]
        else:
            b, t, c, H, W = frames.shape
        if H % 4 or W % 4:
            raise ValueError("H and W must be multiples of 4")
        h, w = H // 4, W // 4
        fh, fw = token_grid(h, w)
        if fh % 5 or fw % 9:
            raise ValueError("token grid %dx%d is not a multiple of (5,9): pad H to a multiple of 60 and W to a "
                             "multiple of 108 (reference test.py:156-165)" % (fh, fw))
        if not self.hq and (h, w) != (60, 108):
            raise ValueError("model 'e2fgvi' is fixed to 432x240 inputs (sc.bias is [128,60,108]); use e2fgvi_hq")
        if not (1 <= l_t <= t):
            raise ValueError("num_local_frames must be in [1, t]")
        if decode_local and b != 1:
# ... 64 lines not shown
```

### e2fgvi_amd/lib.py

```python
import ctypes as C
import os

_HERE = os.path.dirname(os.path.abspath(__file__))
LIB_PATH = os.environ.get("E2FGVI_LIB") or os.path.join(_HERE, "csrc", "libe2fgvi_hip.so")

ABI_VERSION = 9
MAX_SRC = 4
ACT_NONE, ACT_RELU, ACT_LRELU, ACT_TANH, ACT_DCNPOST = 0, 1, 2, 3, 4
DT_F32, DT_BF16 = 0, 1
DT_BF16X3 = 2
DT_F16 = 3

_fp = C.c_void_p


class ConvDesc(C.Structure):
    _fields_ = [
        ("src", _fp * MAX_SRC), ("src_ld", C.c_int32 * MAX_SRC), ("src_coff", C.c_int32 * MAX_SRC),
        ("src_cpg", C.c_int32 * MAX_SRC), ("nsrc", C.c_int32),
        ("N", C.c_int32), ("H", C.c_int32), ("W", C.c_int32), ("Ho", C.c_int32), ("Wo", C.c_int32),
        ("KH", C.c_int32), ("KW", C.c_int32), ("stride", C.c_int32), ("pad", C.c_int32),
        ("groups", C.c_int32), ("Cout", C.c_int32), ("bk", C.c_int32),
        ("wpacked", _fp), ("bias", _fp), ("residual", _fp), ("res_ld", C.c_int32), ("res_coff", C.c_int32),
        ("dst", _fp), ("dst_ld", C.c_int32), ("dst_coff", C.c_int32), ("dst_nchw", C.c_int32),
        ("act", C.c_int32), ("slope", C.c_float), ("tile", C.c_int32),
    ]


class ConvXDesc(C.Structure):
    _fields_ = [
        ("src", _fp * MAX_SRC), ("src_ld", C.c_int32 * MAX_SRC), ("src_coff", C.c_int32 * MAX_SRC),
        ("src_cpg", C.c_int32 * MAX_SRC), ("nsrc", C.c_int32),
        ("N", C.c_int32), ("H", C.c_int32), ("W", C.c_int32), ("Ho", C.c_int32), ("Wo", C.c_int32),
        ("KH", C.c_int32), ("KW", C.c_int32), ("stride", C.c_int32), ("pad", C.c_int32),
        ("groups", C.c_int32), ("Cout", C.c_int32),
        ("wpacked", _fp), ("bias", _fp), ("residual", _fp), ("res_ld", C.c_int32), ("res_coff", C.c_int32),
        ("res_dtype", C.c_int32),
        ("dst", _fp), ("dst_ld", C.c_int32), ("dst_coff", C.c_int32), ("dst_dtype", C.c_int32),
        ("dst2", _fp), ("dst2_ld", C.c_int32), ("dst2_coff", C.c_int32),
        ("act", C.c_int32), ("slope", C.c_float), ("tile", C.c_int32), ("dst_nchw", C.c_int32), ("tap_packed", C.c_int32),
        ("out_grid", C.c_int32), ("pad_left", C.c_int32),
        ("out_sy", C.c_int32), ("out_sx", C.c_int32), ("out_py", C.c_int32), ("out_px", C.c_int32),
        ("out_H", C.c_int32), ("out_W", C.c_int32), ("res_bcast", C.c_int32),
        ("dst2_split_from", C.c_int32), ("dst2_plane_stride", C.c_int64),
    ]


class MdcnDesc(C.Structure):
    _fields_ = [
        ("src", _fp * 2), ("src_ld", C.c_int32 * 2), ("src_c", C.c_int32 * 2), ("nsrc", C.c_int32),
        ("N", C.c_int32), ("H", C.c_int32), ("W", C.c_int32), ("Ho", C.c_int32), ("Wo", C.c_int32),
        ("KH", C.c_int32), ("KW", C.c_int32), ("stride", C.c_int32), ("pad", C.c_int32), ("dil", C.c_int32),
        ("deform_groups", C.c_int32), ("Cout", C.c_int32),
        ("offset", _fp), ("off_ld", C.c_int32), ("mask", _fp), ("mask_ld", C.c_int32),
        ("flows", _fp), ("max_residue", C.c_float),
        ("wpacked", _fp), ("bias", _fp),
        ("dst", _fp), ("dst_ld", C.c_int32), ("dst_coff", C.c_int32), ("tile", C.c_int32), ("dst_dtype", C.c_int32),
        ("mfma_dtype", C.c_int32), ("src_dtype", C.c_int32), ("src_planar", C.c_int32),
    ]


_i32, _i64, _f = C.c_int32, C.c_int64, C.c_float
SYMBOLS = {
    "e2fgvi_last_error": (C.c_char_p, []),
    "e2fgvi_abi_version": (C.c_int, []),
    "e2fgvi_nhwc_to_planar16": (C.c_int, [_fp, _fp, _i64, _i32, _fp]),
    "e2fgvi_conv2d_nhwc": (C.c_int, [C.POINTER(ConvDesc), _fp]),
    "e2fgvi_conv2d_nhwc_nopk": (C.c_int, [C.POINTER(ConvDesc), _fp]),
    "e2fgvi_conv2d_x": (C.c_int, [C.POINTER(ConvXDesc), _i32, _fp]),
    "e2fgvi_packed_conv_weight_x_size": (_i64, [_i32, _i32, _i32, _i32, _i32, _i32, _i32, C.POINTER(_i32)]),
    "e2fgvi_pack_conv_weight_x": (C.c_int, [_fp, _fp, _i32, _i32, _i32, _i32, _i32, _i32, _i32, C.POINTER(_i32), _fp]),
    "e2fgvi_packed_conv_weight_size": (_i64, [_i32, _i32, _i32, _i32, _i32, C.POINTER(_i32), _i32]),
    "e2fgvi_pack_conv_weight": (C.c_int, [_fp, _fp, _i32, _i32, _i32, _i32, _i32, C.POINTER(_i32), _i32, _fp]),
    "e2fgvi_packed_winograd_weight_size": (_i64, [_i32, _i32, _i32, C.POINTER(_i32)]),
    "e2fgvi_pack_winograd_weight": (C.c_int, [_fp, _fp, _i32, _i32, _i32, C.POINTER(_i32), _fp]),
    "e2fgvi_conv3x3_winograd": (C.c_int, [C.POINTER(ConvDesc), _fp]),
    "e2fgvi_packed_winograd_weight_x3_size": (_i64, [_i32, _i32, _i32, C.POINTER(_i32)]),
    "e2fgvi_pack_winograd_weight_x3": (C.c_int, [_fp, _fp, _i32, _i32, _i32, C.POINTER(_i32), _fp]),
    "e2fgvi_conv3x3_winograd_x3": (C.c_int, [C.POINTER(ConvDesc), _fp]),
    "e2fgvi_packed_winograd4_weight_size": (_i64, [_i32, _i32, _i32, C.POINTER(_i32), _i32]),
    "e2fgvi_pack_winograd4_weight": (C.c_int, [_fp, _fp, _i32, _i32, _i32, C.POINTER(_i32), _i32, _fp]),
    "e2fgvi_conv3x3_winograd4": (C.c_int, [C.POINTER(ConvDesc), _i32, _fp]),
    "e2fgvi_packed_tail_weight_size": (_i64, [_i32, _i32]),
    "e2fgvi_pack_tail_weight": (C.c_int, [_fp, _fp, _i32, _i32, _i32, _fp]),
    "e2fgvi_conv3x3_tail": (C.c_int, [_fp, _i32, _i32, _fp, _fp, _fp, _i32, _i32, _i32, _i32, C.c_float, _fp]),
    "e2fgvi_mdcn_nhwc": (C.c_int, [C.POINTER(MdcnDesc), _fp]),
    "e2fgvi_packed_dcn_weight_size": (_i64, [_i32, _i32, _i32, _i32, _i32]),
    "e2fgvi_pack_dcn_weight": (C.c_int, [_fp, _fp, _i32, _i32, _i32, _i32, _i32, _i32, _fp]),
    "e2fgvi_focal_attention": (C.c_int, [_fp, _fp, _fp, _i32, _fp, _fp, _i32, _i32, _i32, _i32, _i32, _fp]),
    "e2fgvi_split3_kv": (C.c_int, [_fp, _fp, _i64, _fp]),
    "e2fgvi_focal_attention_x3": (C.c_int, [_fp, _fp, _fp, _i32, _fp, _fp, _i32, _i32, _i32, _i32, _i32, _fp]),
    "e2fgvi_nchw_to_nhwc": (C.c_int, [_fp, _fp, _i32, _i32, _i32, _i32, _i32, _i32, _f, _f, _fp]),
    "e2fgvi_nhwc_to_nchw": (C.c_int, [_fp, _i32, _fp, _i32, _i32, _i32, _i32, _fp]),
    "e2fgvi_resize_bilinear": (C.c_int, [_fp, _i32, _i32, _i32, _fp, _i32, _i32, _i32, _i32, _i32, _i32, _i32, _i32, _fp, _fp, _fp]),
    "e2fgvi_avgpool2_nhwc": (C.c_int, [_fp, _fp, _i32, _i32, _i32, _i32, _fp]),
    "e2fgvi_spynet_level_input": (C.c_int, [_fp, _fp, _fp, _fp, _fp, _fp, _i32, _i32, _i32, _i32, _fp]),
    "e2fgvi_prop_cond": (C.c_int, [_fp, _i32, _fp, _i32, _i32, _fp, _fp, _i64, _fp, _i32, _fp, _fp, _i32, _i32, _i32, _i32, _fp]),
    "e2fgvi_layernorm": (C.c_int, [_fp, _fp, _fp, _fp, _i32, _i64, _i32, _fp]),
    "e2fgvi_window_pool": (C.c_int, [_fp, _i32, _fp, _fp, _fp, _i32, _i32, _i32, _i32, _fp]),
    "e2fgvi_ffn_fold": (C.c_int, [_fp, _fp, _i32, _i32, _i32, _i32, _i32, _i32, _i32, _i32, _fp]),
    "e2fgvi_ffn_unfold": (C.c_int, [_fp, _fp, _i32, _i32, _i32, _i32, _i32, _i32, _i32, _i32, _fp]),
    "e2fgvi_mask_prepare": (C.c_int, [_fp, _i32, _i32, _i32, _fp, _fp, _fp, _i32, _i32, _i32, _fp]),
    "e2fgvi_masked_clip": (C.c_int, [_fp, _fp, _fp, _i32, _i32, _i32, _fp, _i32, _i32, _fp]),
    "e2fgvi_composite": (C.c_int, [_fp, _fp, _fp, _i32, _fp, _fp, _fp, _i32, _i32, _i32, _i32, _fp]),
    "e2fgvi_resample_u8": (C.c_int, [_fp, _fp, _i32, _i32, _i32, _i32, _i32, _fp, _fp, _i32, _fp]),
    "e2fgvi_restore_u8": (C.c_int, [_fp, _fp, _fp, _fp, _i32, _i32, _i32, _i32, _i32, _fp, _fp, _fp, _fp, _i32, _fp, _fp, _i32, _fp]),
    "e2fgvi_resample_rows_u8": (C.c_int, [_fp, _fp, _i32, _i32, _i32, _i32, _i32, _i32, _fp, _fp, _i32, _fp]),
    "e2fgvi_restore_box_u8": (C.c_int, [_fp, _fp, _fp, _fp, _i32, _i32, _i32, _i32, _i32, _i32, _i32, _i32, _i32, _fp, _fp, _fp, _fp, _i32,
                                        _fp, _fp, _i32, _fp]),
    "e2fgvi_hole_bbox": (C.c_int, [_fp, _i32, _i32, _i32, _fp, _fp]),
    "e2fgvi_hole_bbox_frames": (C.c_int, [_fp, _i32, _i32, _i32, _fp, _fp]),
    "e2fgvi_mask_prepare_ids": (C.c_int, [_fp, _i32, _fp, _i32, _i32, _i32, _fp, _fp, _fp, _i32, _i32, _i32, _fp]),
    "e2fgvi_resample_ids_u8": (C.c_int, [_fp, _i32, _fp, _i32, _fp, _i32, _i32, _i32, _i32, _fp, _fp, _i32, _fp]),
    "e2fgvi_resample_rows_ids_u8": (C.c_int, [_fp, _i32, _fp, _i32, _fp, _i32, _i32, _i32, _i32, _i32, _fp, _fp, _i32, _fp]),
    "e2fgvi_restore_blend": (C.c_int, [_fp, _fp, _fp, _fp, _fp, _fp] + [_i32] * 14 + [_fp, _fp, _fp, _fp, _i32, _fp, _fp, _i32, _fp]),
    "e2fgvi_u8_to_float": (C.c_int, [_fp, _fp, _i64, _fp]),
    "e2fgvi_float_to_u8": (C.c_int, [_fp, _fp, _i64, _fp]),
    "e2fgvi_pred_to_u8": (C.c_int, [_fp, _fp, _i32, _i32, _i32, _i32, _i32, _fp]),
    "e2fgvi_gather_slabs": (C.c_int, [_fp, _i32, _fp, _i32, _i64, _fp, _fp]),
    "e2fgvi_scatter_slabs": (C.c_int, [_fp, _fp, _i32, _i64, _fp, _i32, _fp]),
    "e2fgvi_psnr_ssim_workspace": (_i64, [_i32, _i32, _i32]),
    "e2fgvi_psnr_ssim": (C.c_int, [_fp, _fp, _i32, _i32, _i32, _i32, _fp, _fp, _fp]),
    "e2fgvi_softcomp_fold": (C.c_int, [_fp, _fp, _fp, _fp, _i32, _i32, _i32, _i32, _i32, _i32, _i32, _fp]),
    "e2fgvi_focal_attention_16": (C.c_int, [_fp, _fp, _fp, _i32, _fp, _fp, _i32, _i32, _i32, _i32, _i32, _fp]),
    "e2fgvi_focal_attention_16_variant": (C.c_int, [C.c_int]),
    "e2fgvi_cast": (C.c_int, [_fp, _i32, _fp, _i32, _i64, _fp]),
}

_lib = None

TRACE = None
NEXT_META = None


X3_PIPE = 6 * 157.3 / 2500.0


def useful_macs(kernel, macs, issued):
    import re
    k = str(kernel)
    f = 1.0
    m = re.match(r"conv_wino4<F\((\d)x4\)", k)
    if m:
        fy = int(m.group(1))
# ... 84 lines not shown
```

### e2fgvi_amd/ops.py

```python
import collections
import ctypes as C
import math
import os

import torch

from . import lib as _L

ACT_NONE, ACT_RELU, ACT_LRELU, ACT_TANH, ACT_DCNPOST = _L.ACT_NONE, _L.ACT_RELU, _L.ACT_LRELU, _L.ACT_TANH, _L.ACT_DCNPOST


def _stream():
    return C.c_void_p(torch.cuda.current_stream().cuda_stream)


def _chk(t, name, dtype=torch.float32):
    if not isinstance(t, torch.Tensor) or not t.is_cuda:
        raise TypeError("%s must be a CUDA (ROCm) tensor -- the HIP path has no CPU fallback" % name)
    if t.dtype != dtype:
        raise TypeError("%s must be %s, got %s" % (name, dtype, t.dtype))
    if not t.is_contiguous():
        raise ValueError("%s must be contiguous" % name)
    return t


def _ptr(t):
    return C.c_void_p(t.data_ptr()) if t is not None else C.c_void_p(0)


def empty_nhwc(n, h, w, c, device):
    return torch.empty((n, h, w, c), dtype=torch.float32, device=device)


TUNE_CANDIDATES = (0, 213, 223, 211, 219, 216)
WINO_CANDIDATES = (64, 132, 164, 32)
W4_CODES = {2464: (2, 64)}
_W4_MINPIX = 20000
XTUNE_CANDIDATES = (1, 4, 6, 7, 8, 2, 5, 3, 107, 108)
XTUNE_ROWSHIFT = (11, 16, 17, 12, 13, 18)
X3_ENABLED = os.environ.get("E2FGVI_X3", "1") != "0"
X3_MARGIN = 0.97
X3_BASE = 30000
W3_BASE = 40000
W3_CANDIDATES = (132, 164, 32, 5132, 6064)
W3_WIDE = 6064
W3_WIDE_FALLBACK = 164
DMA_BASE = 2000


def _decode(code):
    if code >= W3_BASE:
        return "w3", code - W3_BASE
    if code >= X3_BASE:
        return "x3", code - X3_BASE
    if code in W4_CODES:
        return "w4", code
    if DMA_BASE <= code < DMA_BASE + 100:
        return "dma", code - DMA_BASE
    return "own", code


_TUNED = {}
AUTOTUNE = os.environ.get("E2FGVI_AUTOTUNE", "0") == "1"
TUNE_REPS = max(1, int(os.environ.get("E2FGVI_TUNE_REPS", "1") or 1))
TABLE_FORMAT = 2
_SIZE_FIELD = 8


def _default_tune_file():
    try:
        st = os.stat(_L.LIB_PATH)
        d = os.environ.get("E2FGVI_CACHE_DIR") or os.path.join(os.path.dirname(os.path.abspath(__file__)), ".tile_cache")
        os.makedirs(d, exist_ok=True)
        dev = "gpu"
        if torch.cuda.is_available():
            dev = "".join(ch for ch in torch.cuda.get_device_properties(0).gcnArchName.split(":")[0] if ch.isalnum())
        return os.path.join(d, "tiles_v%d_%s_%x_%x.txt" % (TABLE_FORMAT, dev, st.st_size, int(st.st_mtime)))
    except (OSError, RuntimeError):
        return None


_TUNE_FILE = None
if AUTOTUNE:
    _TUNE_FILE = os.environ.get("E2FGVI_TUNE_FILE")
    if _TUNE_FILE is None:
        _TUNE_FILE = _default_tune_file()
    elif _TUNE_FILE in ("", "0"):
        _TUNE_FILE = None
    if _TUNE_FILE and os.path.exists(_TUNE_FILE):
        import ast
        for _line in open(_TUNE_FILE):
            try:
                _k, _v = ast.literal_eval(_line)
                _TUNED[_k] = _v
# ... 145 lines not shown

    def _srcs_out(self, sources, out, out_nchw, out_dtype):
        srcs = [(s, 0) if isinstance(s, torch.Tensor) else s for s in sources]
        if len(srcs) != len(self.cpg):
            raise ValueError("expected %d sources, got %d" % (len(self.cpg), len(srcs)))
        if out is None:
            N, H, W, _ = srcs[0][0].shape
            Ho, Wo = self.out_hw(H, W)
            out = torch.empty((N, self.Cout, Ho, Wo) if out_nchw else (N, Ho, Wo, self.Cout),
                              dtype=torch.float32 if out_nchw else out_dtype, device=srcs[0][0].device)
        return srcs, out

    def _x_alternative(self, **kw):
        alt = PackedConvX(self._w_raw, self.bias, self.cpg, groups=self.groups, stride=self.stride, pad=self.pad, dtype=torch.float32, **kw)
        alt.name = self.name
        return alt

    def _fill(self, d, src_dtype, chk, srcs, out, out_coff, act, slope, out_nchw):
        N, H, W, _ = srcs[0][0].shape
        Ho, Wo = self.out_hw(H, W)
        for i, (t, coff) in enumerate(srcs):
            _chk(t, "source %d" % i, src_dtype)
            if t.dim() != 4 or tuple(t.shape[:3]) != (N, H, W):
                raise ValueError("source %d shape %s does not match [%d,%d,%d,*]" % (i, tuple(t.shape), N, H, W))
            d.src[i], d.src_ld[i], d.src_coff[i], d.src_cpg[i] = t.data_ptr(), t.shape[3], coff, self.cpg[i]
        d.nsrc = len(srcs)
        d.N, d.H, d.W, d.Ho, d.Wo = N, H, W, Ho, Wo
        d.KH, d.KW, d.stride, d.pad = self.KH, self.KW, self.stride, self.pad
        d.groups, d.Cout = self.groups, self.Cout
        d.bias = self.bias.data_ptr() if self.bias is not None else None
        chk(out, "out")
        if out_nchw:
            if tuple(out.shape) != (N, self.Cout, Ho, Wo) or out.dtype != torch.float32:
                raise ValueError(self._NCHW_ERROR % dict(got=tuple(out.shape), want=(N, self.Cout, Ho, Wo)))
            d.dst_ld, d.dst_coff, d.dst_nchw = 0, 0, 1
        else:
            if out.dim() != 4 or tuple(out.shape[:3]) != (N, Ho, Wo):
                raise ValueError("out shape %s != [%d,%d,%d,*]" % (tuple(out.shape), N, Ho, Wo))
            d.dst_ld, d.dst_coff, d.dst_nchw = out.shape[3], out_coff, 0
        d.dst = out.data_ptr()
        d.act, d.slope, d.tile = act, slope, 0
        return d

    @staticmethod
    def _fill_residual(d, chk, residual, res_coff):
        if residual is not None:
            chk(residual, "residual")
            if residual.dim() != 4 or tuple(residual.shape[:3]) != (d.N, d.Ho, d.Wo):
                raise ValueError("residual shape %s != [%d,%d,%d,*]" % (tuple(residual.shape), d.N, d.Ho, d.Wo))
            d.residual, d.res_ld, d.res_coff = residual.data_ptr(), residual.shape[3], res_coff


_Plan = collections.namedtuple("_Plan", "family tile static from_table use_wino")
_Call = collections.namedtuple("_Call", "d srcs kw kv_planes")


class PackedConv(_ConvLayer):

    _NCHW_ERROR = "NCHW out shape %(got)s != %(want)s"

    def __init__(self, weight, bias, cpg, groups=1, stride=1, pad=0, bk=None, precision="fp32", algo="igemm"):
        lib = _L.load()
        w = self._init_layer(weight, bias, cpg, groups, stride, pad)
        if precision != "fp32":
            raise ValueError("PackedConv is the fp32 layer; the bf16 data path uses PackedConvX")
        self.precision = precision
        self.nopk = False
        self.alt = None
        self._w_raw = w
        if algo not in ("igemm", "winograd", "auto"):
            raise ValueError("algo must be 'igemm', 'winograd' or 'auto'")
        wino_ok = (self.KH, self.KW, stride, pad) == (3, 3, 1, 1) and not any(c % 4 for c in self.cpg)
        if algo == "winograd" and not wino_ok:
            raise ValueError("winograd needs fp32, 3x3 / stride 1 / pad 1 and channels per source in multiples of 4")
        if algo == "auto":
            algo = "auto" if wino_ok else "igemm"
        self.algo = algo
        self._w4 = {}
        self._w3 = None
        self._w_oihw = w if algo in ("winograd", "auto") else None
        self._own = {}
        if algo in ("winograd", "auto"):
            _L.check(min(0, int(lib.e2fgvi_packed_winograd_weight_size(*self._wgeom()))), "packed_winograd_weight_size")
        if algo == "winograd":
            self.bk = 8
            return
        if bk is None:
            pad32 = sum((c + 31) // 32 * 32 for c in self.cpg)
            pad16 = sum((c + 15) // 16 * 16 for c in self.cpg)
            bk = 32 if pad32 <= 1.08 * sum(self.cpg) else (16 if pad16 <= 1.08 * sum(self.cpg) else 8)
        self.bk = bk
        _L.check(min(0, int(lib.e2fgvi_packed_conv_weight_size(self.Cout, groups, self.KH, self.KW, len(self.cpg), self._cpg_arr(), bk))),
                 "packed_conv_weight_size")

    def _wgeom(self):
        return self.Cout, self.groups, len(self.cpg), self._cpg_arr()

    @property
    def wino_packed(self):
        if self.algo not in ("winograd", "auto"):
            return None

        def build():
            lib = _L.load()
            return _pack_weights(lib.e2fgvi_packed_winograd_weight_size, lib.e2fgvi_pack_winograd_weight, self._w_raw, torch.float32,
                                 "winograd_weight", *self._wgeom())
        return _lazy(self._own, "wino", self.name + " (Winograd F(2x2,3x3) weights)", build)
# ... 32 lines not shown

    def _wino_x3(self):
        if self._w_oihw is None:
            return None

        def build():
            lib = _L.load()
            return _pack_weights(lib.e2fgvi_packed_winograd_weight_x3_size, lib.e2fgvi_pack_winograd_weight_x3, self._w_oihw,
                                 torch.bfloat16, "winograd_weight_x3", *self._wgeom())
        return _lazy(vars(self), "_w3", self.name + " (split-operand Winograd weights)", build)

    def _alt3(self):
        if any(c % 4 for c in self.cpg):
            return self.alt3
        return _lazy(vars(self), "alt3", self.name + " (split-operand GEMM alternative)", lambda: self._x_alternative(x3=True))

    def _work(self, d, use_wino, family, tile):
        N, H, W, Ho, Wo = d.N, d.H, d.W, d.Ho, d.Wo
        cin_g, cout_g, K2 = sum(self.cpg), self.Cout // self.groups, self.KH * self.KW
        macs = N * Ho * Wo * self.Cout * cin_g * K2
        asked = int(tile)
        if family == "w4":
            fy, bn = W4_CODES[tile]
            pix = N * (-(-H // (8 * fy)) * 8 * fy) * (-(-W // 16) * 16)
            cin_p = sum(-(-c // 8) * 8 for c in self.cpg)
            issued = pix * (-(-cout_g // bn) * bn) * self.groups * cin_p * (fy + 2) * 6 // (fy * 4)
            kern = "conv_wino4<F(%dx4),%d>" % (fy, bn)
        elif family == "w3":
            asked = W3_BASE + tile
            shape = tile % 1000
            mt, bn = (2, shape) if shape < 100 else (1, shape - 100)
            pix = N * (-(-H // (8 * mt)) * 8 * mt) * (-(-W // 16) * 16)
            cin_p = -(-sum(-(-c // 8) for c in self.cpg) // 2) * 16
            issued = int(pix * (-(-cout_g // bn) * bn) * self.groups * cin_p * 4 * 6 * 157.3 / 2500.0)
            kern = ("conv_wino_x3w<%d>" % bn) if tile >= 6000 else ("conv_wino_x3p4<%d>" % bn) if tile >= 5000 else "conv_wino_x3<%d,%d>" % (mt, bn)
        elif use_wino:
            if not tile:
                big = N * -(-H // 16) * -(-W // 16) * -(-cout_g // 64) * self.groups
                tile = 64 if (cout_g >= 256 and big >= 128) else 132
            mt, bn = (2, tile) if tile < 100 else (1, tile - 100)
            pix = N * (-(-H // (8 * mt)) * 8 * mt) * (-(-W // 16) * 16)
            cin_p = sum(-(-c // 8) * 8 for c in self.cpg)
            issued = pix * (-(-cout_g // bn) * bn) * self.groups * cin_p * 4
            kern = "conv_wino<%d,%d>" % (mt, bn)
        else:
            g = self.bk
            cin_p = sum(-(-c // g) * g for c in self.cpg)
            issued = N * Ho * Wo * (-(-cout_g // 32) * 32) * self.groups * cin_p * K2
            kern = "conv_igemm/halo tile=%d" % tile
        return dict(layer=self.name, kernel=kern, shape="N%d %dx%d %d->%d k%d s%d g%d" % (
            N, H, W, cin_g * self.groups, self.Cout, self.KH, self.stride, self.groups), macs=macs, issued=issued, tile=asked)

    def __call__(self, sources, out=None, out_coff=0, residual=None, res_coff=0, act=ACT_NONE, slope=0.0,
                 out_nchw=False, tile=0, kv_planes=None, out_dtype=None):
        if out_dtype not in (None, torch.float32):
            raise ValueError("PackedConv writes fp32 results")
        srcs, out = self._srcs_out(sources, out, out_nchw, torch.float32)
        N, H, W, _ = srcs[0][0].shape
        kw = dict(out_coff=out_coff, res_coff=res_coff, act=act, slope=slope, out_nchw=out_nchw)
        chunks = list(_image_chunks(N, max(H * W * t.shape[3] * 4 for t, _ in srcs)))
        if len(chunks) > 1:
            for n0, n1 in chunks:
                self([(t[n0:n1], c) for t, c in srcs], out=out[n0:n1], residual=None if residual is None else residual[n0:n1],
                     tile=tile, **kw)
        else:
            kw.update(out=out, residual=residual)
            call = _Call(self._desc(srcs, **kw), srcs, kw, kv_planes)
            if self._launch(call, self._select(call, tile)):
                return out
        if kv_planes is not None:
            split3_kv(out.view(-1, out.shape[-1]), out=kv_planes)
        return out

    def _desc(self, srcs, out, out_coff, residual, res_coff, act, slope, out_nchw):
        d = self._fill(_L.ConvDesc(), torch.float32, _chk, srcs, out, out_coff, act, slope, out_nchw)
        self._fill_residual(d, _chk, residual, res_coff)
        d.bk = self.bk
        return d

    def _select(self, call, tile):
        d, kw = call.d, call.kw
        N, H, W, Ho, Wo = d.N, d.H, d.W, d.Ho, d.Wo
        out, residual = kw["out"], kw["residual"]
        use_wino = self.algo == "winograd" or (self.algo == "auto" and H % 2 == 0 and W % 2 == 0 and not kw["out_nchw"]
                                               and (tile in (0, 32, 64, 132, 164) or _decode(tile)[0] in ("w4", "w3")))
        asked = _decode(tile) if use_wino else ("own", tile)
        static = self._wino4_rule(N, H, W) if use_wino and (tile == 0 or asked[0] == "w3") else tile
        own = ("w4" if use_wino and static in W4_CODES else "own", static)
        family, arg = asked if asked[0] == "w3" else own
        plan = _Plan(family, arg, own, False, use_wino)
        x3 = self.try_x3 and X3_ENABLED
        if not (tile == 0 and (static == 0 or not self.tune) and (self.tune or x3) and N * Ho * Wo >= 2048):
            return plan
        key = (self.Cout, tuple(self.cpg), self.KH, self.KW, self.stride, self.pad, self.groups, self.bk,
               int(4.0 * math.log2(N * Ho * Wo)), residual is not None, kw["act"], use_wino, bool(self.tune), int(static)) + (("x3",) if x3 else ())
        best = _decision(key)
        from_table = best is not None
        if best is None and AUTOTUNE and not torch.cuda.is_current_stream_capturing() and (
                residual is None or residual.data_ptr() != out.data_ptr()):
            best = _remember(key, self._tune(call, own, use_wino, x3))
        family, arg = _decode(best or 0)
        if family in ("w3", "x3") or (self.tune and (family == "dma" or (family == "own" and arg < DMA_BASE))):
            plan = plan._replace(family=family, tile=arg)
        return plan._replace(from_table=from_table)

    def _tune(self, call, own, use_wino, x3):
        d, srcs, kw, kv_planes = call
        best = self._autotune(d, use_wino) if self.tune else own[1]
        base = own if own[0] == "w4" else ("own", best)
        mine = None

        def time_mine():
            self._run(d, *base, use_wino)
            return min(_time_launches(lambda: self._run(d, *base, use_wino), 3) for _ in range(TUNE_REPS))
        if self.tune and not use_wino and not self.nopk:
            alt = self._alt()
            mine = time_mine()
            res = alt._time_tiles(alt._desc(srcs, out2=None, **kw))
            if res and min(res.values()) < mine:
                best, mine = DMA_BASE + min(res, key=res.get), min(res.values())
        if x3 and self._alt3() is not None:
            if mine is None:
                mine = time_mine()
            d3 = self.alt3._desc(srcs, out2=None, **kw)
            if kv_planes is not None:
                self.alt3._set_planes(d3, kv_planes, self.Cout - kv_planes.shape[2], d.N * d.Ho * d.Wo)
            res = self.alt3._time_tiles(d3)
            if res and min(res.values()) < X3_MARGIN * mine:
                best, mine = X3_BASE + min(res, key=res.get), min(res.values())
        if x3 and use_wino and self._wino_x3() is not None:
            w3 = {}
            for shape in W3_CANDIDATES:
                def run():
                    return self._run(d, "w3", shape, use_wino)[0]
                if run() == 0:
                    w3[shape] = min(_time_launches(run, 3) for _ in range(TUNE_REPS))
            if w3 and min(w3.values()) < X3_MARGIN * mine:
                best, mine = W3_BASE + min(w3, key=w3.get), min(w3.values())
        return best

    def _autotune(self, d, wino):
        lib = _L.load()
        best, best_ms = 0, float("inf")
        st = _stream()
        fn = lib.e2fgvi_conv3x3_winograd if wino else lib.e2fgvi_conv2d_nhwc
        d.tile, d.wpacked = 0, (self.wino_packed if wino else self.wpacked).data_ptr()
        for _ in range(3):
            fn(C.byref(d), st)
        for code in (WINO_CANDIDATES if wino else TUNE_CANDIDATES):
            d.tile = code
            if fn(C.byref(d), st) != 0:
                continue
            ms = min(_time_launches(lambda: fn(C.byref(d), st), 2) for _ in range(TUNE_REPS))
            if ms < best_ms:
                best, best_ms = code, ms
        return best

    def _run(self, d, family, tile, use_wino):
        lib, st = _L.load(), _stream()
        if family == "w3":
            d.tile, d.wpacked = tile, self._wino_x3().data_ptr()
            return lib.e2fgvi_conv3x3_winograd_x3(C.byref(d), st), "conv3x3_winograd_x3"
        if family == "w4":
            fy, d.tile = W4_CODES[tile]
            d.wpacked = self._wino4(fy).data_ptr()
            return lib.e2fgvi_conv3x3_winograd4(C.byref(d), fy, st), "conv3x3_winograd4"
        d.tile = tile
        d.wpacked = (self.wino_packed if use_wino else self.wpacked).data_ptr()
        if use_wino:
            return lib.e2fgvi_conv3x3_winograd(C.byref(d), st), "conv3x3_winograd"
        if self.nopk:
            return lib.e2fgvi_conv2d_nhwc_nopk(C.byref(d), st), "conv2d_nhwc_nopk"
        return lib.e2fgvi_conv2d_nhwc(C.byref(d), st), "conv2d_nhwc"

    def _launch(self, call, plan):
        d, srcs, kw, kv_planes = call
        family, tile = plan.family, plan.tile
        try:
            if family == "x3" and self._alt3() is not None:
                self.alt3(srcs, tile=tile, planes=kv_planes, split_from=(self.Cout - kv_planes.shape[2]) if kv_planes is not None else 0,
                          **kw)
                return True
            if family == "dma":
                self._alt()(srcs, tile=tile, **kw)
                return False
            if family == "x3" or (family == "w3" and self._wino_x3() is None):
                family, tile = plan.static
        except _L.HipError:
            if not plan.from_table:
                raise
            family, tile = plan.static
        if _L.TRACE is not None:
            _L.annotate(**self._work(d, plan.use_wino, family, tile))
        rc, what = self._run(d, family, tile, plan.use_wino)
        if rc != 0 and (family, tile) != plan.static:
            rc, what = self._run(d, *plan.static, plan.use_wino)
        _L.check(rc, what)
        return False


HALF16 = (torch.bfloat16, torch.float16)


_DT_CODE = {torch.float32: _L.DT_F32, torch.bfloat16: _L.DT_BF16, torch.float16: _L.DT_F16}


def _dt(t):
    try:
        return _DT_CODE[t.dtype]
    except KeyError:
        raise TypeError("tensor must be float32, bfloat16 or float16, got %s" % t.dtype) from None


def _dt_key(t):
    return _L.DT_BF16 if t.dtype == torch.float16 else _dt(t)


def _chk_any(t, name):
    if not isinstance(t, torch.Tensor) or not t.is_cuda:
        raise TypeError("%s must be a CUDA (ROCm) tensor -- the HIP path has no CPU fallback" % name)
    if not t.is_contiguous():
        raise ValueError("%s must be contiguous" % name)
    _dt(t)
    return t


class PackedConvX(_ConvLayer):

    _NCHW_ERROR = "NCHW out must be fp32 %(want)s"

    def __init__(self, weight, bias, cpg, groups=1, stride=1, pad=0, dtype=torch.bfloat16, taps=None, x3=False):
        lib = _L.load()
        w = self._init_layer(weight, bias, cpg, groups, stride, pad)
        self.dtype = dtype
        self.f32 = dtype == torch.float32
        self.x3 = bool(x3)
        if self.x3 and not self.f32:
            raise ValueError("x3 splitting is for fp32 sources")
        self.f16 = dtype == torch.float16
        if not self.f32 and dtype not in HALF16:
            raise TypeError("PackedConvX: dtype must be float32, bfloat16 or float16")
        self._mode = mode = _L.DT_BF16X3 if self.x3 else _DT_CODE[dtype]
        conv2d_x = lib.e2fgvi_conv2d_x
        self._fn = lambda desc_ref, stream: conv2d_x(desc_ref, mode, stream)
        self._w_raw = w if (self.f32 and not self.x3) else None
        self._taps_arg = taps
        self.taps = (len(self.cpg) == 1 and groups == 1 and self.cpg[0] <= 56 and self.KW > 1
                     and (taps is True if self.f32 else taps is not False))
        self._wdtype = torch.bfloat16 if self.x3 else dtype
        self._wp = None
        if self._w_raw is None:
            self._wp = self._pack(w)
        else:
            _L.check(min(0, int(lib.e2fgvi_packed_conv_weight_x_size(*self._wgeom()))), "packed_conv_weight_x_size")

    @property
    def wpacked(self):
        return _lazy(vars(self), "_wp", self.name + " (LDS-DMA GEMM weights)", lambda: self._pack(self._w_raw))

    def weight_bytes(self):
        return (0 if self._wp is None else self._wp.numel() * self._wp.element_size()) + (self.alt3.weight_bytes() if self.alt3 is not None else 0)

    def _wgeom(self):
        return self._mode, int(self.taps), self.Cout, self.groups, self.KH, self.KW, len(self.cpg), self._cpg_arr()

    def _pack(self, w):
        lib = _L.load()
        return _pack_weights(lib.e2fgvi_packed_conv_weight_x_size, lib.e2fgvi_pack_conv_weight_x, w, self._wdtype, "conv_weight_x",
                             *self._wgeom())

    def _alt3(self):
        if self._w_raw is None:
            return self.alt3
        return _lazy(vars(self), "alt3", self.name + " (split-operand GEMM alternative)",
                     lambda: self._x_alternative(taps=self._taps_arg, x3=True))

    def _desc(self, srcs, out, out_coff, residual, res_coff, act, slope, out2, out_nchw):
        d = self._fill(_L.ConvXDesc(), self.dtype, _chk_any, srcs, out, out_coff, act, slope, out_nchw)
        d.wpacked = None if self._wp is None else self._wp.data_ptr()
        d.dst_dtype = _dt(out)
        if out2 is not None:
            _chk(out2, "out2", torch.float16 if self.f16 else torch.bfloat16)
            if out2.dim() != 4 or tuple(out2.shape[:3]) != (d.N, d.Ho, d.Wo):
                raise ValueError("out2 shape %s != [%d,%d,%d,*]" % (tuple(out2.shape), d.N, d.Ho, d.Wo))
            d.dst2, d.dst2_ld, d.dst2_coff = out2.data_ptr(), out2.shape[3], 0
        self._fill_residual(d, _chk_any, residual, res_coff)
        if residual is not None:
            d.res_dtype = _dt(residual)
        d.tap_packed = 1 if self.taps else 0
        return d

    @staticmethod
    def _set_planes(d, planes, split_from, rows):
        _chk(planes, "planes", torch.bfloat16)
        if planes.dim() != 3 or planes.shape[0] != 3 or planes.shape[1] != rows or planes.shape[2] != d.Cout - split_from:
            raise ValueError("planes must be [3, %d, %d] bf16, got %s" % (rows, d.Cout - split_from, tuple(planes.shape)))
        d.dst2, d.dst2_ld, d.dst2_coff = planes.data_ptr(), planes.shape[2], 0
        d.dst2_split_from, d.dst2_plane_stride = split_from, planes.shape[1] * planes.shape[2]

    def __call__(self, sources, out=None, out_dtype=None, out_coff=0, residual=None, res_coff=0, act=ACT_NONE,
                 slope=0.0, out2=None, tile=0, out_nchw=False, planes=None, split_from=0):
        if out_dtype is None:
            out_dtype = self.dtype
        srcs, out = self._srcs_out(sources, out, out_nchw, out_dtype)
        N, H, W, _ = srcs[0][0].shape
        Ho, Wo = self.out_hw(H, W)
        kw = dict(out_coff=out_coff, res_coff=res_coff, act=act, slope=slope, out_nchw=out_nchw)
        chunks = list(_image_chunks(N, max(H * W * t.shape[3] * (4 if self.f32 else 2) for t, _ in srcs)))
        if len(chunks) > 1:
            if planes is not None:
                raise ValueError("split planes: the batch spans >= 4 GiB (call in chunks)")
            for n0, n1 in chunks:
                self([(t[n0:n1], c) for t, c in srcs], out=out[n0:n1], residual=None if residual is None else residual[n0:n1],
                     out2=None if out2 is None else out2[n0:n1], tile=tile, **kw)
            return out
        kw.update(out=out, residual=residual, out2=out2)
        d = self._desc(srcs, **kw)
        if planes is not None:
            self._set_planes(d, planes, split_from, N * Ho * Wo)
        if tile == 0 and self.tune and N * Ho * Wo >= 2048:
            family, tile = self._select(d, srcs, kw)
            if family == "x3":
                try:
                    return self.alt3(srcs, out_dtype=out_dtype, tile=tile, planes=planes, split_from=split_from, **kw)
                except _L.HipError:
                    tile = 0
        d.tile = tile
        if _L.TRACE is not None:
            _L.annotate(**self._work(d))
        d.wpacked = self.wpacked.data_ptr()
        rc = self._fn(C.byref(d), _stream())
        if rc != 0 and d.tile and self.tune:
            d.tile = 0
            rc = self._fn(C.byref(d), _stream())
        _L.check(rc, "conv2d_x")
        return out

    def _select(self, d, srcs, kw):
        out, residual = kw["out"], kw["residual"]
        x3 = self.try_x3 and X3_ENABLED and self.f32 and not self.x3
        key = (("x3" if self.x3 else ("x32+3" if x3 else "x32")) if self.f32 else "x", self.Cout, tuple(self.cpg), self.KH, self.KW, self.stride, self.pad, self.groups,
               int(4.0 * math.log2(d.N * d.Ho * d.Wo)), _dt_key(out), kw["out_nchw"], self.taps)
        best = _decision(key)
        if best is None and AUTOTUNE and not torch.cuda.is_current_stream_capturing() and (
                residual is None or residual.data_ptr() != out.data_ptr()):
            best = _remember(key, self._tune(d, srcs, kw, x3))
        if _decode(best or 0)[0] in ("x3", "w3"):
            return ("x3", best - X3_BASE) if self._alt3() is not None else ("own", 0)
        return "own", best or 0

    def _tune(self, d, srcs, kw, x3):
        res = self._time_tiles(d)
        best = min(res, key=res.get) if res else 0
        if x3 and self._alt3() is not None:
            res3 = self.alt3._time_tiles(self.alt3._desc(srcs, **kw))
            if res3 and (not res or min(res3.values()) < X3_MARGIN * min(res.values())):
                best = X3_BASE + min(res3, key=res3.get)
        return best

    def _work(self, d):
        N, H, W, Ho, Wo, tile = d.N, d.H, d.W, d.Ho, d.Wo, d.tile
        cin_g, cout_g, K2 = sum(self.cpg), self.Cout // self.groups, self.KH * self.KW
        kc = 32 if self.f32 else 64
        cin_p = sum(-(-c // kc) * kc for c in self.cpg)
        if self.taps:
            cin_p = -(-K2 * (self.cpg[0] // (4 if self.f32 else 8)) // 8) * kc / K2
        return dict(layer=self.name, kernel="conv_%s tile=%d%s" % (("f32x3" if self.x3 else "f32x") if self.f32 else
                                                                   "f16x" if self.f16 else "bf16x", tile, " taps" if self.taps else ""),
                    shape="N%d %dx%d %d->%d k%d s%d g%d" % (N, H, W, cin_g * self.groups, self.Cout, self.KH, self.stride, self.groups),
                    macs=N * Ho * Wo * self.Cout * cin_g * K2, tile=int(tile),
                    issued=int(N * Ho * Wo * (-(-cout_g // 32) * 32) * self.groups * cin_p * K2 * (_L.X3_PIPE if self.x3 else 1)))

    def _time_tiles(self, d, reps=3, rounds=2):
        st = _stream()
        res = {}
        d.tile = 0
        d.wpacked = self.wpacked.data_ptr()

        def run():
            return self._fn(C.byref(d), st)
        for _ in range(2):
            run()
        for _ in range(rounds * TUNE_REPS):
            rowshift = (self.KH, self.KW, self.stride, self.pad) == (3, 3, 1, 1) and not self.f32 and not self.taps
            for code in XTUNE_CANDIDATES + (XTUNE_ROWSHIFT if rowshift else ()):
                if code % 10 == 3 and self.Cout // self.groups > 64:
                    continue
                if code in (12, 18) and self.Cout // self.groups > 64:
                    continue
                d.tile = code
                if run() == 0:
                    res[code] = min(res.get(code, float("inf")), _time_launches(run, reps))
        d.tile = 0
        return res


class SoftCompGather:

    def __init__(self, weight, bias, channels=128, dtype=torch.bfloat16):
        w = _chk(weight.detach().float().contiguous(), "weight")
        if w.dim() != 2 or w.shape[0] != 49 * channels:
            raise ValueError("SoftComp embedding weight must be [%d, hidden]" % (49 * channels))
        self.C, self.hidden, self.dtype = channels, w.shape[1], dtype
        w4 = w.view(channels, 7, 7, self.hidden)
        self.phases = []
        for py in range(3):
            ky_taps = [6, 3, 0] if py == 0 else [py + 3, py]
            for px in range(3):
                kx_taps = [6, 3, 0] if px == 0 else [px + 3, px]
                wp = w4[:, ky_taps][:, :, kx_taps].permute(0, 3, 1, 2).contiguous()
                layer = PackedConvX(wp, None, [self.hidden], dtype=dtype)
                layer.name = "sc.embedding phase (%d,%d)" % (py, px)
                self.phases.append((py, px, 1 if py == 0 else 0, 1 if px == 0 else 0, layer))
        self.bias = None if bias is None else _chk(bias.detach().float().contiguous(), "bias")
        self._bias_img = {}
        self.tile = 0

    def bias_image(self, fh, fw):
        if self.bias is None:
            return None
# ... 13 lines not shown
            out = torch.empty((F_, H, W, self.C), dtype=out_dtype or self.dtype, device=tokens.device)
        if tuple(out.shape) != (F_, H, W, self.C):
            raise ValueError("out must be [%d,%d,%d,%d]" % (F_, H, W, self.C))
        chunks = list(_image_chunks(F_, fh * fw * hid * tokens.element_size()))
        if len(chunks) > 1:
            for n0, n1 in chunks:
                self(tokens[n0:n1], out=out[n0:n1])
            return out
        bimg = self.bias_image(fh, fw)
        for py, px, pad_y, pad_x, layer in self.phases:
            d = _L.ConvXDesc()
            d.src[0], d.src_ld[0], d.src_coff[0], d.src_cpg[0], d.nsrc = tokens.data_ptr(), hid, 0, hid, 1
            d.N, d.H, d.W, d.Ho, d.Wo = F_, fh, fw, fh, fw
            d.KH, d.KW, d.stride, d.pad = layer.KH, layer.KW, 1, pad_y
            d.groups, d.Cout = 1, self.C
            d.wpacked = layer.wpacked.data_ptr()
            d.dst, d.dst_ld, d.dst_coff, d.dst_dtype = out.data_ptr(), self.C, 0, _dt(out)
            if bimg is not None:
                d.residual, d.res_ld, d.res_coff, d.res_dtype, d.res_bcast = bimg.data_ptr(), self.C, 0, _L.DT_F32, 1
            d.out_grid, d.pad_left = 1, pad_x
            d.out_sy, d.out_sx, d.out_py, d.out_px, d.out_H, d.out_W = 3, 3, py, px, H, W
            d.act, d.slope, d.tile = ACT_NONE, 0.0, self.tile
            if _L.TRACE is not None:
                kc = 32 if layer.f32 else 64
                macs = F_ * fh * fw * self.C * hid * layer.KH * layer.KW
                _L.annotate(layer=layer.name, kernel="conv_%s (gather-form SoftComp)" % ("f32x" if layer.f32 else "f16x" if layer.f16 else "bf16x"),
                            shape="N%d %dx%d %d->%d k%dx%d scatter s3" % (F_, fh, fw, hid, self.C, layer.KH, layer.KW),
                            macs=macs, issued=macs // hid * (-(-hid // kc) * kc))
            _L.check(layer._fn(C.byref(d), _stream()), "conv2d_x (SoftComp phase)")
        return out


class PackedLinearX(PackedConvX):

    def __init__(self, weight, bias, dtype=torch.bfloat16):
        super().__init__(weight, bias, [weight.shape[1]], dtype=dtype)

    def __call__(self, x, out=None, out_dtype=None, residual=None, act=ACT_NONE, slope=0.0, out2=None, tile=0):
        rows = x.numel() // x.shape[-1]
        if out is None:
            out = torch.empty((rows, self.Cout), dtype=out_dtype or self.dtype, device=x.device)
        r4 = None if residual is None else residual.view(rows, 1, 1, residual.shape[-1])
        o2 = None if out2 is None else out2.view(rows, 1, 1, out2.shape[-1])
        super().__call__([x.view(rows, 1, 1, x.shape[-1])], out=out.view(rows, 1, 1, out.shape[-1]), residual=r4, act=act,
                         slope=slope, out2=o2, tile=tile)
        return out


class PackedLinear(PackedConv):

    def __init__(self, weight, bias, bk=None, precision="fp32"):
        super().__init__(weight, bias, [weight.shape[1]], bk=bk, precision=precision)

    def __call__(self, x, out=None, residual=None, act=ACT_NONE, slope=0.0, tile=0, kv_planes=None, out_dtype=None):
        if out_dtype not in (None, torch.float32):
            raise ValueError("PackedLinear writes fp32 results")
        _chk(x, "x")
        rows = x.numel() // x.shape[-1]
        x4 = x.view(rows, 1, 1, x.shape[-1])
        if out is None:
            out = torch.empty((rows, self.Cout), dtype=torch.float32, device=x.device)
        o4 = out.view(rows, 1, 1, out.shape[-1])
        r4 = None if residual is None else residual.view(rows, 1, 1, residual.shape[-1])
        super().__call__([x4], out=o4, residual=r4, act=act, slope=slope, tile=tile, kv_planes=kv_planes)
        return out


class PackedTailConv:

    def __init__(self, weight, bias, dtype=torch.float32):
        lib = _L.load()
        w = _chk(weight.detach().float().contiguous(), "weight")
        self.Cout, self.Cin, self.KH, self.KW = w.shape
        if (self.KH, self.KW) != (3, 3):
            raise ValueError("PackedTailConv: 3x3 kernels only")
        self.dtype = dtype
        if dtype not in _DT_CODE:
            raise TypeError("tensor must be float32, bfloat16 or float16, got %s" % dtype)
        self.wpacked = _pack_weights(lib.e2fgvi_packed_tail_weight_size, lib.e2fgvi_pack_tail_weight, w, dtype, "tail_weight",
                                     self.Cout, self.Cin, extra=(_DT_CODE[dtype],))
        self.bias = None if bias is None else _chk(bias.detach().float().contiguous(), "bias")
        self.name = "conv_tail"

    def __call__(self, sources, out=None, act=ACT_NONE, slope=0.0, out_nchw=True, tile=0):
        x = sources[0] if isinstance(sources, (list, tuple)) else sources
        if not out_nchw:
            raise ValueError("PackedTailConv writes NCHW frames")
        _chk(x, "x", self.dtype)
        N, H, W, ld = x.shape
        if out is None:
            out = torch.empty((N, self.Cout, H, W), dtype=torch.float32, device=x.device)
        _chk(out, "out")
        if tuple(out.shape) != (N, self.Cout, H, W):
            raise ValueError("out shape %s != %s" % (tuple(out.shape), (N, self.Cout, H, W)))
        macs = N * H * W * self.Cout * self.Cin * 9
        tiles = N * -(-H // 16) * -(-W // 32)
        _L.annotate(layer=self.name, kernel="conv_tail", shape="N%d %dx%d %d->%d k3 s1 g1" % (N, H, W, self.Cin, self.Cout),
                    macs=macs, issued=tiles * 640 * 64 * 32)
        _L.check(_L.load().e2fgvi_conv3x3_tail(_ptr(x), _dt(x), ld, _ptr(self.wpacked), _ptr(self.bias), _ptr(out), N, H, W, act,
                                               float(slope), _stream()), "conv3x3_tail")
        return out


_DCN_PACKING = {"fp32": (_L.DT_F32, torch.float32, "mdcn"), "bf16": (_L.DT_BF16, torch.bfloat16, "mdcn_bf16"),
                "fp16": (_L.DT_F16, torch.float16, "mdcn_f16"), "x3": (_L.DT_BF16X3, torch.bfloat16, "mdcn_x3")}


class PackedDcn:
    def __init__(self, weight, bias, deform_groups, stride=1, pad=0, dil=1, mfma="fp32"):
        lib = _L.load()
        if mfma not in _DCN_PACKING:
            raise ValueError("mfma must be 'fp32', 'bf16', 'fp16' or 'x3'")
        self._mfma_dtype, wdtype, self._kernel = _DCN_PACKING[mfma]
        self.mfma_bf16, self.mfma_f16, self.mfma_x3 = mfma == "bf16", mfma == "fp16", mfma == "x3"
        w = _chk(weight.detach().float().contiguous(), "weight")
        self.Cout, self.C, self.KH, self.KW = w.shape
        self.dg, self.stride, self.pad, self.dil = deform_groups, stride, pad, dil
# ... 61 lines not shown
                        macs=m, issued=int(m * 6 * 157.3 / 2500.0) if self._mfma_dtype == _L.DT_BF16X3 else m)
        _L.check(lib.e2fgvi_mdcn_nhwc(C.byref(d), _stream()), "mdcn_nhwc")
        return out


def _attn_work(B, T, fh, fw, nkeys):
    qpad = -(-(45 * T) // 32) * 32
    return dict(shape="B%d T%d grid %dx%d" % (B, T, fh, fw), macs=B * (fh // 5) * (fw // 9) * 4 * (45 * T) * (210 * T) * 128 * 2,
                issued=B * 4 * qpad * 128 * 2 * sum(-(-(T * k) // 32) * 32 for k in nkeys.tolist()))


def focal_attention(qkv, kv_pool, key_tab, nkeys, B, T, fh, fw, out=None, waves=0):
    lib = _L.load()
    _chk(qkv, "qkv"); _chk(kv_pool, "kv_pool")
    _chk(key_tab, "key_tab", torch.int32); _chk(nkeys, "nkeys", torch.int32)
    rows = B * T * fh * fw
    if tuple(qkv.shape) != (rows, 1536):
        raise ValueError("qkv must be [%d,1536], got %s" % (rows, tuple(qkv.shape)))
    nwin = (fh // 5) * (fw // 9)
    if tuple(kv_pool.shape) != (B * T * nwin, 1536):
        raise ValueError("kv_pool must be [%d,1536], got %s" % (B * T * nwin, tuple(kv_pool.shape)))
    if key_tab.shape[0] != nwin or nkeys.shape[0] != nwin:
        raise ValueError("key table must have %d rows" % nwin)
    if out is None:
        out = torch.empty((rows, 512), dtype=torch.float32, device=qkv.device)
    _chk(out, "out")
    rpc, ppc = T * fh * fw, T * nwin
    chunks = list(_image_chunks(B, rpc * 1536 * 4))
    if len(chunks) > 1:
        for b0, b1 in chunks:
            focal_attention(qkv[b0 * rpc:b1 * rpc], kv_pool[b0 * ppc:b1 * ppc], key_tab, nkeys, b1 - b0, T, fh, fw,
                            out=out[b0 * rpc:b1 * rpc], waves=waves)
        return out
    if _L.TRACE is not None:
        _L.annotate(layer="attention", kernel="focal_attn", **_attn_work(B, T, fh, fw, nkeys))
    _L.check(lib.e2fgvi_focal_attention(_ptr(qkv), _ptr(kv_pool), _ptr(key_tab), key_tab.shape[1], _ptr(nkeys),
                                        _ptr(out), B, T, fh, fw, waves, _stream()), "focal_attention")
    return out


def split3_kv(rows_1536, out=None):
    lib = _L.load()
    _chk(rows_1536, "qkv rows")
    if rows_1536.dim() != 2 or rows_1536.shape[1] != 1536:
        raise ValueError("split3_kv takes [rows, 1536] fp32 rows")
    rows = rows_1536.shape[0]
    if out is None:
        out = torch.empty((3, rows, 1024), dtype=torch.bfloat16, device=rows_1536.device)
    _chk(out, "planes", torch.bfloat16)
    _L.check(lib.e2fgvi_split3_kv(_ptr(rows_1536), _ptr(out), rows, _stream()), "split3_kv")
    return out


def focal_attention_x3(qkv, planes, key_tab, nkeys, B, T, fh, fw, out=None, waves=0):
    lib = _L.load()
    _chk(qkv, "qkv"); _chk(planes, "planes", torch.bfloat16)
    _chk(key_tab, "key_tab", torch.int32); _chk(nkeys, "nkeys", torch.int32)
    rows = B * T * fh * fw
    nwin = (fh // 5) * (fw // 9)
    if tuple(qkv.shape) != (rows, 1536):
        raise ValueError("qkv must be [%d,1536], got %s" % (rows, tuple(qkv.shape)))
    if tuple(planes.shape) != (3, rows + B * T * nwin, 1024):
        raise ValueError("planes must be [3,%d,1024], got %s" % (rows + B * T * nwin, tuple(planes.shape)))
    if key_tab.shape[0] != nwin or nkeys.shape[0] != nwin:
        raise ValueError("key table must have %d rows" % nwin)
    if out is None:
        out = torch.empty((rows, 512), dtype=torch.float32, device=qkv.device)
    _chk(out, "out")
    if _L.TRACE is not None:
        work = _attn_work(B, T, fh, fw, nkeys)
        work["issued"] = int(work["issued"] * 6 * 157.3 / 2500.0)
        _L.annotate(layer="attention", kernel="focal_attn_x3", **work)
    _L.check(lib.e2fgvi_focal_attention_x3(_ptr(qkv), _ptr(planes), _ptr(key_tab), key_tab.shape[1], _ptr(nkeys), _ptr(out),
                                           B, T, fh, fw, waves, _stream()), "focal_attention_x3")
    return out


def attention_x3_applies(B, T, fh, fw):
    rows = B * T * (fh * fw + (fh // 5) * (fw // 9))
    return (X3_ENABLED and 3 * rows * 2048 < 0xFFFFF000
            and -(-(T * 210) // 32) * 128 + 2 * 49152 + 1280 <= 160 * 1024)


def focal_attention_bf16(qkv, kv_pool, key_tab, nkeys, B, T, fh, fw, out=None, variant=None):
    lib = _L.load()
    if variant is not None:
        prev = lib.e2fgvi_focal_attention_16_variant(int(variant))
        try:
            return focal_attention_bf16(qkv, kv_pool, key_tab, nkeys, B, T, fh, fw, out=out)
        finally:
            lib.e2fgvi_focal_attention_16_variant(prev)
    dt = qkv.dtype if isinstance(qkv, torch.Tensor) and qkv.dtype == torch.float16 else torch.bfloat16
    _chk(qkv, "qkv", dt); _chk(kv_pool, "kv_pool", dt)
    _chk(key_tab, "key_tab", torch.int32); _chk(nkeys, "nkeys", torch.int32)
    rows = B * T * fh * fw
    nwin = (fh // 5) * (fw // 9)
    if tuple(qkv.shape) != (rows, 1536) or tuple(kv_pool.shape) != (B * T * nwin, 1536):
        raise ValueError("qkv must be [%d,1536] and kv_pool [%d,1536]" % (rows, B * T * nwin))
    if key_tab.shape[0] != nwin or nkeys.shape[0] != nwin:
        raise ValueError("key table must have %d rows" % nwin)
    if out is None:
        out = torch.empty((rows, 512), dtype=dt, device=qkv.device)
    _chk(out, "out", dt)
    if _L.TRACE is not None:
        _L.annotate(layer="attention", kernel="focal_attn_f16" if dt == torch.float16 else "focal_attn_bf16",
                    **_attn_work(B, T, fh, fw, nkeys))
    _L.check(lib.e2fgvi_focal_attention_16(_ptr(qkv), _ptr(kv_pool), _ptr(key_tab), key_tab.shape[1], _ptr(nkeys), _ptr(out),
                                           _dt(qkv), B, T, fh, fw, _stream()),
             "focal_attention_f16" if dt == torch.float16 else "focal_attention_bf16")
    return out


def nchw_to_nhwc(x, ld=None, scale=1.0, shift=0.0, out_dtype=torch.float32):
    lib = _L.load()
    _chk(x, "x")
    N, Cc, H, W = x.shape
    ld = Cc if ld is None else ld
    out = torch.empty((N, H, W, ld), dtype=out_dtype, device=x.device)
    _L.check(lib.e2fgvi_nchw_to_nhwc(_ptr(x), _ptr(out), _dt(out), N, Cc, H, W, ld, scale, shift, _stream()), "nchw_to_nhwc")
    return out


def cast(x, dtype):
    lib = _L.load()
    _chk_any(x, "x")
    out = torch.empty(x.shape, dtype=dtype, device=x.device)
    _L.check(lib.e2fgvi_cast(_ptr(x), _dt(x), _ptr(out), _dt(out), x.numel(), _stream()), "cast")
# ... 72 lines not shown
                                           _dt(out16) if out16 is not None else _L.DT_F32, Np, h, w, _stream()),
             "spynet_level_input")
    return (out, out16) if copy_dtype is not None else out


def prop_cond(feat_prop, feat_n2, flow_a, flow_b, flow_img_stride, cond=None, flows=None, cond_dtype=torch.float32,
              flows8=False):
    lib = _L.load()
    _chk_any(feat_prop, "feat_prop")
    N, H, W, Cc = feat_prop.shape
    if cond is None:
        cond = torch.empty((N, H, W, 2 * Cc), dtype=cond_dtype, device=feat_prop.device)
    if flows is None:
        flows = empty_nhwc(N, H, W, 4, feat_prop.device)
    fl8 = (torch.empty((N, H, W, 8), dtype=cond.dtype if cond.dtype == torch.float16 else torch.bfloat16, device=feat_prop.device)
           if flows8 else None)
    f2_ld = 0
    if flow_b is not None:
        _chk(feat_n2, "feat_n2", feat_prop.dtype)
        f2_ld = feat_n2.shape[3]
    _L.check(lib.e2fgvi_prop_cond(_ptr(feat_prop), Cc, _ptr(feat_n2) if flow_b is not None else None, f2_ld, _dt(feat_prop),
                                  C.c_void_p(flow_a.data_ptr()),
                                  C.c_void_p(flow_b.data_ptr()) if flow_b is not None else None,
                                  flow_img_stride, _ptr(cond), _dt(cond), _ptr(flows), _ptr(fl8), N, H, W, Cc, _stream()),
             "prop_cond")
    return (cond, flows, fl8) if flows8 else (cond, flows)


def layernorm(x, gamma, beta, out=None, out_dtype=torch.float32):
    lib = _L.load()
    _chk(x, "x"); _chk(gamma, "gamma"); _chk(beta, "beta")
    Cc = x.shape[-1]
    rows = x.numel() // Cc
    if out is None:
        out = torch.empty(x.shape, dtype=out_dtype, device=x.device)
    _chk_any(out, "out")
    _L.check(lib.e2fgvi_layernorm(_ptr(x), _ptr(gamma), _ptr(beta), _ptr(out), _dt(out), rows, Cc, _stream()), "layernorm")
    return out


def window_pool(x, w45, bias1, BT, fh, fw, out=None):
    lib = _L.load()
    _chk_any(x, "x"); _chk(w45, "w45"); _chk(bias1, "bias1")
    Cc = x.shape[-1]
    rows = BT * (fh // 5) * (fw // 9)
    if out is None:
        out = torch.empty((rows, Cc), dtype=x.dtype, device=x.device)
    elif tuple(_chk(out, "out", x.dtype).shape) != (rows, Cc):
        raise ValueError("window_pool out must be [%d,%d]" % (rows, Cc))
    _L.check(lib.e2fgvi_window_pool(_ptr(x), _dt(x), _ptr(w45), _ptr(bias1), _ptr(out), BT, fh, fw, Cc, _stream()), "window_pool")
    return out


def _ffn_fold(hid, F_, fh, fw, H, W, Cc, gelu):
    lib = _L.load()
    _chk_any(hid, "hid")
    out = torch.empty((F_, H, W, Cc), dtype=hid.dtype, device=hid.device)
    _L.check(lib.e2fgvi_ffn_fold(_ptr(hid), _ptr(out), _dt(hid), gelu, F_, fh, fw, H, W, Cc, _stream()),
             "ffn_fold_gelu" if gelu else "ffn_fold")
    return out


def ffn_fold(hid, F_, fh, fw, H, W, Cc):
    return _ffn_fold(hid, F_, fh, fw, H, W, Cc, 0)


def ffn_fold_gelu(hid, F_, fh, fw, H, W, Cc):
    return _ffn_fold(hid, F_, fh, fw, H, W, Cc, 1)


def _ffn_unfold(folded, fh, fw, out, gelu):
    lib = _L.load()
    _chk_any(folded, "folded")
    F_, H, W, Cc = folded.shape
    if out is None:
        out = torch.empty((F_ * fh * fw, 49 * Cc), dtype=folded.dtype, device=folded.device)
    _chk(out, "out", folded.dtype)
    _L.check(lib.e2fgvi_ffn_unfold(_ptr(folded), _ptr(out), _dt(folded), gelu, F_, fh, fw, H, W, Cc, _stream()),
             "ffn_unfold_gelu" if gelu else "ffn_unfold")
    return out


def ffn_unfold(folded, fh, fw, out=None):
    return _ffn_unfold(folded, fh, fw, out, 0)


def ffn_unfold_gelu(folded, fh, fw, out=None):
    return _ffn_unfold(folded, fh, fw, out, 1)


def to_planar16(x, out=None):
    dt = x.dtype if isinstance(x, torch.Tensor) and x.dtype == torch.float16 else torch.bfloat16
    _chk(x, "x", dt)
    N, H, W, Cc = x.shape
    if out is None:
        out = torch.empty((Cc // 16, N, H, W, 16), dtype=dt, device=x.device)
    _chk(out, "out", dt)
    _L.check(_L.load().e2fgvi_nhwc_to_planar16(_ptr(x), _ptr(out), N * H * W, Cc, _stream()), "nhwc_to_planar16")
    return out


def softcomp_fold(emb, F_, fh, fw, H, W, Cc, bias_hwc=None, residual=None):
    lib = _L.load()
    dt = emb.dtype if isinstance(emb, torch.Tensor) and emb.dtype in HALF16 else torch.float32
    _chk(emb, "emb", dt)
    out = torch.empty((F_, H, W, Cc), dtype=dt, device=emb.device)
    if bias_hwc is not None:
        _chk(bias_hwc, "bias_hwc")
    if residual is not None:
        _chk(residual, "residual", dt)
    _L.check(lib.e2fgvi_softcomp_fold(_ptr(emb), _ptr(bias_hwc), _ptr(residual), _ptr(out), _dt(out), F_, fh, fw, H, W, Cc,
                                      _stream()), "softcomp_fold")
    return out


def _u8(t, name):
    return _chk(t, name, torch.uint8)


def _frame_ids(ids, device):
    _chk(ids, "ids", torch.int32)
# ... 269 lines not shown
```

### include/e2fgvi_hip.h

```cpp
#ifndef E2FGVI_HIP_H
#define E2FGVI_HIP_H

#include <stdint.h>

#ifdef __cplusplus
extern "C" {
#endif

#define E2FGVI_EINVAL (-1)
#define E2FGVI_EUNSUP (-2)

#define E2FGVI_ACT_NONE 0
#define E2FGVI_ACT_RELU 1
#define E2FGVI_ACT_LRELU 2
#define E2FGVI_ACT_TANH 3
int e2fgvi_mask_prepare(const uint8_t* masks, int32_t L, int32_t Hin, int32_t Win, const int32_t* ytab, const int32_t* xtab,
                        uint8_t* out, int32_t H, int32_t W, int32_t iterations, void* stream);
int e2fgvi_mask_prepare_ids(const uint8_t* masks, int32_t L, const int32_t* ids, int32_t n, int32_t Hin, int32_t Win,
                            const int32_t* ytab, const int32_t* xtab, uint8_t* out, int32_t H, int32_t W, int32_t iterations,
                            void* stream);
int e2fgvi_masked_clip(const uint8_t* frames, const uint8_t* masks, const int32_t* ids, int32_t t, int32_t H, int32_t W,
                       float* clip, int32_t Hp, int32_t Wp, void* stream);
int e2fgvi_composite(const float* pred, const int32_t* ids, const uint8_t* first, int32_t n, const uint8_t* frames,
                     const uint8_t* masks, float* comp, int32_t H, int32_t W, int32_t Hp, int32_t Wp, void* stream);
int e2fgvi_resample_u8(const uint8_t* src, uint8_t* dst, int32_t L, int32_t H, int32_t W, int32_t n_out, int32_t axis,
                       const int32_t* bounds, const int32_t* coeffs, int32_t ksize, void* stream);
int e2fgvi_resample_rows_u8(const uint8_t* src, uint8_t* dst, int32_t L, int32_t H, int32_t W, int32_t n_out, int32_t row0,
                            int32_t rows, const int32_t* bounds, const int32_t* coeffs, int32_t ksize, void* stream);
int e2fgvi_resample_ids_u8(const uint8_t* src, int32_t L, const int32_t* ids, int32_t n, uint8_t* dst, int32_t H, int32_t W,
                           int32_t n_out, int32_t axis, const int32_t* bounds, const int32_t* coeffs, int32_t ksize, void* stream);
int e2fgvi_resample_rows_ids_u8(const uint8_t* src, int32_t L, const int32_t* ids, int32_t n, uint8_t* dst, int32_t H, int32_t W,
                                int32_t n_out, int32_t row0, int32_t rows, const int32_t* bounds, const int32_t* coeffs, int32_t ksize,
                                void* stream);
int e2fgvi_hole_bbox(const uint8_t* masks, int32_t L, int32_t Hm, int32_t Wm, int32_t* box, void* stream);
int e2fgvi_hole_bbox_frames(const uint8_t* masks, int32_t L, int32_t Hm, int32_t Wm, int32_t* boxes, void* stream);
int e2fgvi_restore_u8(const uint8_t* lo, const uint8_t* mask_lo, const uint8_t* src, uint8_t* out, int32_t L, int32_t h, int32_t w,
                      int32_t H, int32_t W, const int32_t* ytab, const int32_t* xtab, const int32_t* bounds_x,
                      const int32_t* coeffs_x, int32_t ksize_x, const int32_t* bounds_y, const int32_t* coeffs_y, int32_t ksize_y,
                      void* stream);
int e2fgvi_restore_box_u8(const uint8_t* lo, const uint8_t* mask_lo, const uint8_t* src, uint8_t* out, int32_t L, int32_t h,
                          int32_t w, int32_t H, int32_t W, int32_t left, int32_t upper, int32_t Bw, int32_t Bh, const int32_t* ytab,
                          const int32_t* xtab, const int32_t* bounds_x, const int32_t* coeffs_x, int32_t ksize_x,
                          const int32_t* bounds_y, const int32_t* coeffs_y, int32_t ksize_y, void* stream);
int e2fgvi_restore_blend(const uint8_t* lo, const uint8_t* mask_lo, const uint8_t* src, const int32_t* ids, const uint8_t* first,
                         float* acc, int32_t n, int32_t L, int32_t h, int32_t w, int32_t H, int32_t W, int32_t left, int32_t upper,
                         int32_t Bw, int32_t Bh, int32_t touch_left, int32_t touch_upper, int32_t Tw, int32_t Th, const int32_t* ytab,
                         const int32_t* xtab, const int32_t* bounds_x, const int32_t* coeffs_x, int32_t ksize_x,
                         const int32_t* bounds_y, const int32_t* coeffs_y, int32_t ksize_y, void* stream);
int e2fgvi_u8_to_float(const uint8_t* src, float* dst, int64_t n, void* stream);
int e2fgvi_float_to_u8(const float* src, uint8_t* dst, int64_t n, void* stream);
int e2fgvi_pred_to_u8(const float* pred, uint8_t* dst, int32_t N, int32_t H, int32_t W, int32_t Hp, int32_t Wp, void* stream);
int e2fgvi_gather_slabs(const void* cache, int32_t slots, const int32_t* ids, int32_t n, int64_t slab_bytes, void* window,
                        void* stream);
int e2fgvi_scatter_slabs(const void* rows, const int32_t* ids, int32_t n, int64_t slab_bytes, void* cache, int32_t slots,
                         void* stream);

int64_t e2fgvi_psnr_ssim_workspace(int32_t N, int32_t H, int32_t W);
int e2fgvi_psnr_ssim(const float* img1, const float* img2, int32_t N, int32_t H, int32_t W, int32_t win_size,
                     void* workspace, double* out, void* stream);

#define E2FGVI_ACT_DCNPOST 4

#define E2FGVI_MAX_SRC 4

#define E2FGVI_F32 0
#define E2FGVI_BF16 1
#define E2FGVI_BF16X3 2
#define E2FGVI_F16 3

const char* e2fgvi_last_error(void);
int e2fgvi_abi_version(void);

typedef struct {
    const float* src[E2FGVI_MAX_SRC];
    int32_t src_ld[E2FGVI_MAX_SRC];
    int32_t src_coff[E2FGVI_MAX_SRC];
    int32_t src_cpg[E2FGVI_MAX_SRC];
    int32_t nsrc;
    int32_t N, H, W;
    int32_t Ho, Wo;
    int32_t KH, KW, stride, pad;
    int32_t groups;
    int32_t Cout;
    int32_t bk;
    const float* wpacked;
    const float* bias;
    const float* residual;
    int32_t res_ld, res_coff;
    float* dst;
    int32_t dst_ld, dst_coff;
    int32_t dst_nchw;
    int32_t act;
    float slope;
    int32_t tile;
} e2fgvi_conv_desc;

int e2fgvi_conv2d_nhwc(const e2fgvi_conv_desc* d, void* stream);
int e2fgvi_conv2d_nhwc_nopk(const e2fgvi_conv_desc* d, void* stream);

int64_t e2fgvi_packed_conv_weight_size(int32_t Cout, int32_t groups, int32_t KH, int32_t KW,
                                       int32_t nsrc, const int32_t* src_cpg, int32_t bk);
int e2fgvi_pack_conv_weight(const float* w, float* wpacked, int32_t Cout, int32_t groups,
                            int32_t KH, int32_t KW, int32_t nsrc, const int32_t* src_cpg,
                            int32_t bk, void* stream);

int64_t e2fgvi_packed_winograd_weight_size(int32_t Cout, int32_t groups, int32_t nsrc, const int32_t* src_cpg);
int e2fgvi_pack_winograd_weight(const float* w, float* wpacked, int32_t Cout, int32_t groups, int32_t nsrc,
                                const int32_t* src_cpg, void* stream);
int e2fgvi_conv3x3_winograd(const e2fgvi_conv_desc* d, void* stream);

int64_t e2fgvi_packed_winograd4_weight_size(int32_t Cout, int32_t groups, int32_t nsrc, const int32_t* src_cpg, int32_t fy);
int e2fgvi_pack_winograd4_weight(const float* w, float* wpacked, int32_t Cout, int32_t groups, int32_t nsrc,
                                 const int32_t* src_cpg, int32_t fy, void* stream);
int e2fgvi_conv3x3_winograd4(const e2fgvi_conv_desc* d, int32_t fy, void* stream);

int64_t e2fgvi_packed_tail_weight_size(int32_t Cout, int32_t Cin);
int e2fgvi_pack_tail_weight(const float* w, void* wpacked, int32_t Cout, int32_t Cin, int32_t dtype, void* stream);
int e2fgvi_conv3x3_tail(const void* src, int32_t src_dtype, int32_t src_ld, const void* wpacked, const float* bias, float* dst,
                        int32_t N, int32_t H, int32_t W, int32_t act, float slope, void* stream);

typedef struct {
    const void* src[2];
// ... 15 lines not shown
    int32_t dst_dtype;
    int32_t mfma_dtype;
    int32_t src_dtype;
    int32_t src_planar;
} e2fgvi_mdcn_desc;

int e2fgvi_mdcn_nhwc(const e2fgvi_mdcn_desc* d, void* stream);
int64_t e2fgvi_packed_dcn_weight_size(int32_t mfma_dtype, int32_t Cout, int32_t C, int32_t KH, int32_t KW);
int e2fgvi_pack_dcn_weight(const float* w, void* wpacked, int32_t mfma_dtype, int32_t Cout, int32_t C, int32_t KH, int32_t KW,
                           int32_t deform_groups, void* stream);

int e2fgvi_nhwc_to_planar16(const void* src, void* dst, int64_t P, int32_t C, void* stream);

int e2fgvi_focal_attention(const float* qkv, const float* kv_pool, const int32_t* key_tab,
                           int32_t tab_ld, const int32_t* nkeys, float* out, int32_t B, int32_t T,
                           int32_t fh, int32_t fw, int32_t waves, void* stream);

int e2fgvi_nchw_to_nhwc(const float* src, void* dst, int32_t dst_dtype, int32_t N, int32_t C, int32_t H, int32_t W,
                        int32_t ld, float scale, float shift, void* stream);
int e2fgvi_nhwc_to_nchw(const float* src, int32_t ld, float* dst, int32_t N, int32_t C, int32_t H,
                        int32_t W, void* stream);

int e2fgvi_resize_bilinear(const void* src, int32_t dtype, int32_t src_nchw, int32_t src_ld, void* dst,
                           int32_t dst_ld, int32_t N, int32_t C, int32_t H, int32_t W, int32_t Ho,
                           int32_t Wo, int32_t align_corners, const float* scale,
                           const float* shift, void* stream);

int e2fgvi_avgpool2_nhwc(const float* src, float* dst, int32_t N, int32_t H, int32_t W, int32_t C,
                         void* stream);

int e2fgvi_spynet_level_input(const float* pyr, const int32_t* ref_idx, const int32_t* supp_idx,
                              const float* flow_prev, float* out, void* out16, int32_t out16_dtype, int32_t Np,
                              int32_t h, int32_t w, void* stream);

int e2fgvi_prop_cond(const void* feat_prop, int32_t fp_ld, const void* feat_n2, int32_t f2_ld, int32_t src_dtype,
                     const float* flow_a, const float* flow_b, int64_t flow_img_stride, void* cond, int32_t cond_dtype,
                     float* flows, void* flows8_bf16, int32_t N, int32_t H, int32_t W, int32_t C, void* stream);

int e2fgvi_layernorm(const float* x, const float* gamma, const float* beta, void* y, int32_t y_dtype, int64_t rows,
                     int32_t C, void* stream);

int e2fgvi_window_pool(const void* x, int32_t dtype, const float* w45, const float* bias1, void* pooled,
                       int32_t BT, int32_t fh, int32_t fw, int32_t C, void* stream);

int e2fgvi_ffn_fold(const void* hid, void* folded, int32_t dtype, int32_t gelu, int32_t F, int32_t fh, int32_t fw, int32_t H,
                    int32_t W, int32_t C, void* stream);
int e2fgvi_ffn_unfold(const void* folded, void* out, int32_t dtype, int32_t gelu, int32_t F, int32_t fh, int32_t fw,
                      int32_t H, int32_t W, int32_t C, void* stream);

int e2fgvi_softcomp_fold(const void* emb, const float* bias_hwc, const void* residual,
                         void* dst, int32_t dtype, int32_t F, int32_t fh, int32_t fw, int32_t H, int32_t W,
                         int32_t C, void* stream);
int e2fgvi_cast(const void* src, int32_t src_dtype, void* dst, int32_t dst_dtype, int64_t n, void* stream);

typedef struct {
    const void* src[E2FGVI_MAX_SRC];
    int32_t src_ld[E2FGVI_MAX_SRC];
    int32_t src_coff[E2FGVI_MAX_SRC];
    int32_t src_cpg[E2FGVI_MAX_SRC];
    int32_t nsrc;
    int32_t N, H, W, Ho, Wo;
    int32_t KH, KW, stride, pad;
    int32_t groups;
    int32_t Cout;
    const void* wpacked;
    const float* bias;
    const void* residual;
    int32_t res_ld, res_coff, res_dtype;
    void* dst;
    int32_t dst_ld, dst_coff, dst_dtype;
    void* dst2;
    int32_t dst2_ld, dst2_coff;
    int32_t act;
    float slope;
    int32_t tile;
    int32_t dst_nchw;
    int32_t tap_packed;
    int32_t out_grid, pad_left;
    int32_t out_sy, out_sx, out_py, out_px, out_H, out_W;
    int32_t res_bcast;
    int32_t dst2_split_from;
    int64_t dst2_plane_stride;
} e2fgvi_convx_desc;

int e2fgvi_conv2d_x(const e2fgvi_convx_desc* d, int32_t mode, void* stream);
int64_t e2fgvi_packed_conv_weight_x_size(int32_t mode, int32_t tap_packed, int32_t Cout, int32_t groups, int32_t KH, int32_t KW,
                                         int32_t nsrc, const int32_t* src_cpg);
int e2fgvi_pack_conv_weight_x(const float* w, void* wpacked, int32_t mode, int32_t tap_packed, int32_t Cout, int32_t groups,
                              int32_t KH, int32_t KW, int32_t nsrc, const int32_t* src_cpg, void* stream);

int e2fgvi_conv3x3_winograd_x3(const e2fgvi_conv_desc* d, void* stream);
int64_t e2fgvi_packed_winograd_weight_x3_size(int32_t Cout, int32_t groups, int32_t nsrc, const int32_t* src_cpg);
int e2fgvi_pack_winograd_weight_x3(const float* w, void* wpacked, int32_t Cout, int32_t groups, int32_t nsrc,
                                   const int32_t* src_cpg, void* stream);

int e2fgvi_split3_kv(const float* qkv_rows, void* planes, int64_t rows, void* stream);
int e2fgvi_focal_attention_x3(const float* qkv, const void* planes, const int32_t* key_tab, int32_t tab_ld, const int32_t* nkeys,
                              float* out, int32_t B, int32_t T, int32_t fh, int32_t fw, int32_t waves, void* stream);

int e2fgvi_focal_attention_16(const void* qkv, const void* kv_pool, const int32_t* key_tab, int32_t tab_ld,
                              const int32_t* nkeys, void* out, int32_t dtype, int32_t B, int32_t T, int32_t fh, int32_t fw,
                              void* stream);
int e2fgvi_focal_attention_16_variant(int variant);

#ifdef __cplusplus
}
#endif
#endif
```

Before: 966.4 frames/s.

## Pre-split fp32 activations into bf16x3 planes in producers for split-operand convs

Adds a pre-split activation format (BF16X3A) in which each group of 8 fp32 channels is stored as interleaved hi/mid/lo bf16 triples. The attention epilogue and the FFN fold can now emit this format directly, and the conv kernel gains a mode that loads the pre-split A operand instead of splitting fp32 values in its inner loop. The aim is to take the per-tile split arithmetic out of the GEMM main loop, at the cost of 1.5x the activation bytes and a padded LDS pitch. Whether it runs is decided by an X3A_ENABLED flag and the tile table.

```diff
diff --git a/e2fgvi_amd/csrc/attention_x3.hip b/e2fgvi_amd/csrc/attention_x3.hip
--- a/e2fgvi_amd/csrc/attention_x3.hip
+++ b/e2fgvi_amd/csrc/attention_x3.hip
@@ -33,6 +33,7 @@
     return r;
 }
 
+typedef unsigned int x_u32x2 __attribute__((ext_vector_type(2)));
 __device__ __forceinline__ void x_split8(const f32x4& v0, const f32x4& v1, bf16x8& hi, bf16x8& mid, bf16x8& lo) {
     e2_split8(v0, v1, hi, mid, lo);
 }
@@ -57,7 +58,7 @@
                                                                   int tab_ld, const int* __restrict__ nkeys,
                                                                   float* __restrict__ out, int B, int T, int fh, int fw,
                                                                   const char* planes, unsigned planes_bytes, unsigned plane_stride,
-                                                                  unsigned pooled_row0) {
+                                                                  unsigned pooled_row0, int out_a3) {
 #if defined(__HIP_DEVICE_COMPILE__)
     constexpr int NT = 64 * NW;
     constexpr int PIECES = 8 / NW;
@@ -339,7 +340,25 @@
         const float inv = 1.f / l;
         bool ok;
         const long long row = query_row(ok);
-        if (ok) {
+        if (ok && out_a3) {
+            unsigned short* op = reinterpret_cast<unsigned short*>(out) + row * (NH * HD * 3) + head * (HD * 3) + 4 * h;
+#pragma unroll
+            for (int dt = 0; dt < 4; ++dt)
+#pragma unroll
+                for (int rq = 0; rq < 4; ++rq) {
+                    x_u32x2 H, M, L;
+#pragma unroll
+                    for (int j = 0; j < 2; ++j) {
+                        unsigned hh, mm, ll;
+                        e2_split2(e2_rounded(acc[dt][rq * 4 + 2 * j] * inv), e2_rounded(acc[dt][rq * 4 + 2 * j + 1] * inv), hh, mm, ll);
+                        H[j] = hh; M[j] = mm; L[j] = ll;
+                    }
+                    unsigned short* o = op + (dt * 4 + rq) * 24;
+                    *reinterpret_cast<x_u32x2*>(o) = H;
+                    *reinterpret_cast<x_u32x2*>(o + 8) = M;
+                    *reinterpret_cast<x_u32x2*>(o + 16) = L;
+                }
+        } else if (ok) {
             float* op = out + row * (NH * HD) + head * HD;
 #pragma unroll
             for (int dt = 0; dt < 4; ++dt)
@@ -365,9 +384,9 @@
     return 0;
 }
 
-extern "C" int e2fgvi_focal_attention_x3(const float* qkv, const void* planes, const int32_t* key_tab, int32_t tab_ld,
-                                         const int32_t* nkeys, float* out, int32_t B, int32_t T, int32_t fh, int32_t fw,
-                                         int32_t waves, void* stream) {
+static int focal_attention_x3(const float* qkv, const void* planes, const int32_t* key_tab, int32_t tab_ld,
+                              const int32_t* nkeys, float* out, int out_a3, int32_t B, int32_t T, int32_t fh, int32_t fw,
+                              int32_t waves, void* stream) {
     E2_REQUIRE(qkv && planes && key_tab && nkeys && out, E2FGVI_EINVAL, "focal_attention_x3: null pointer");
     E2_REQUIRE(B > 0 && T > 0 && fh > 0 && fw > 0 && fh % WS0 == 0 && fw % WS1 == 0, E2FGVI_EINVAL,
                "focal_attention_x3: token grid %dx%d must be a positive multiple of (5,9)", fh, fw);
@@ -405,7 +424,7 @@
         E2_REQUIRE(ea == hipSuccess, (int)ea, "focal_attention_x3: cannot reserve %zu bytes of dynamic LDS", dyn);                \
         hipLaunchKernelGGL((focal_attn_x3_kernel<NW_, KS_>), grid, block, dyn, (hipStream_t)stream, qkv, key_tab, tab_ld, nkeys, out, \
                            B, T, fh, fw, (const char*)planes, (unsigned)(3 * plane_bytes), (unsigned)plane_bytes,                 \
-                           (unsigned)((long long)B * T * fh * fw));                                                               \
+                           (unsigned)((long long)B * T * fh * fw), out_a3);                                                       \
     } while (0)
     if (ks == 2) E2_ATT_X3(4, 2);
     else if (waves == 2) E2_ATT_X3(2, 1);
@@ -415,3 +434,17 @@
     E2_LAUNCH_CHECK("focal_attention_x3");
     return 0;
 }
+
+extern "C" int e2fgvi_focal_attention_x3(const float* qkv, const void* planes, const int32_t* key_tab, int32_t tab_ld,
+                                         const int32_t* nkeys, float* out, int32_t B, int32_t T, int32_t fh, int32_t fw,
+                                         int32_t waves, void* stream) {
+    return focal_attention_x3(qkv, planes, key_tab, tab_ld, nkeys, out, 0, B, T, fh, fw, waves, stream);
+}
+
+extern "C" int e2fgvi_focal_attention_x3a(const float* qkv, const void* planes, const int32_t* key_tab, int32_t tab_ld,
+                                          const int32_t* nkeys, void* out, int32_t out_dtype, int32_t B, int32_t T, int32_t fh,
+                                          int32_t fw, int32_t waves, void* stream) {
+    E2_REQUIRE(out_dtype == E2FGVI_F32 || out_dtype == E2FGVI_BF16X3A, E2FGVI_EINVAL,
+               "focal_attention_x3a: out_dtype must be E2FGVI_F32 or E2FGVI_BF16X3A");
+    return focal_attention_x3(qkv, planes, key_tab, tab_ld, nkeys, (float*)out, out_dtype == E2FGVI_BF16X3A, B, T, fh, fw, waves, stream);
+}
diff --git a/e2fgvi_amd/csrc/common.h b/e2fgvi_amd/csrc/common.h
--- a/e2fgvi_amd/csrc/common.h
+++ b/e2fgvi_amd/csrc/common.h
@@ -82,6 +82,10 @@
     M = __builtin_amdgcn_perm(rb1, rb0, 0x07060302u);
     L = __builtin_amdgcn_perm(__builtin_bit_cast(unsigned, s1), __builtin_bit_cast(unsigned, s0), 0x07060302u);
 }
+__device__ __forceinline__ float e2_rounded(float x) {
+    asm volatile("" : "+v"(x));
+    return x;
+}
 typedef __bf16 e2_bf16x8 __attribute__((ext_vector_type(8)));
 typedef unsigned int e2_u32x4 __attribute__((ext_vector_type(4)));
 __device__ __forceinline__ void e2_split8(const f32x4& v0, const f32x4& v1, e2_bf16x8& hi, e2_bf16x8& mid, e2_bf16x8& lo) {
diff --git a/e2fgvi_amd/csrc/conv_bf16x.hip b/e2fgvi_amd/csrc/conv_bf16x.hip
--- a/e2fgvi_amd/csrc/conv_bf16x.hip
+++ b/e2fgvi_amd/csrc/conv_bf16x.hip
@@ -76,20 +76,22 @@
 template <int BM, int BN, int WGM, int WGN, bool S3, int MODE, bool PP = false>
 __global__ __launch_bounds__(64 * WGM * WGN) void conv_bf16x_kernel(const ConvXParams p) {
 #if defined(__HIP_DEVICE_COMPILE__)
-    constexpr bool F32 = MODE == 1, X3 = MODE == 2, F16 = MODE == 3;
+    constexpr bool F32 = MODE == 1, X3A = MODE == 4, X3 = MODE == 2 || X3A, F16 = MODE == 3;
     typedef typename e2_h16<F16>::T E16;
     typedef typename e2_h16<F16>::V8 e16x8;
-    static_assert(!PP || (X3 && !S3 && WGM * WGN == 8), "ping-pong halves: split-operand mode, 8 waves, no row-shift stages");
+    static_assert(!PP || (X3 && !X3A && !S3 && WGM * WGN == 8), "ping-pong halves: split-operand mode, 8 waves, no row-shift stages");
+    static_assert(!X3A || !S3, "pre-split activations: no row-shift stages");
     constexpr int NT = 64 * WGM * WGN;
-    constexpr int ESZ = (F32 || X3) ? 4 : 2;
-    constexpr int CH = 16 / ESZ;
-    constexpr int KC = 8 * CH;
+    constexpr int ESZ = X3A ? 6 : (F32 || X3) ? 4 : 2;
+    constexpr int KC = (F32 || X3) ? 32 : 64;
+    constexpr int A_SL = X3A ? 13 : 8;
+    constexpr int A_PITCH = A_SL * 16;
     constexpr int TM = BM / (32 * WGM), TN = BN / (32 * WGN);
     constexpr int AR = S3 ? BM + 2 : BM;
     constexpr int B_CH = X3 ? 12 : 8;
-    constexpr int A_BYTES = AR * 128, B_BYTES = BN * B_CH * 16;
-    constexpr int A_IT = (AR * 8 + NT - 1) / NT, B_IT = (BN * B_CH + NT - 1) / NT;
-    constexpr bool A_PART = (AR * 8) % NT != 0;
+    constexpr int A_BYTES = AR * A_PITCH, B_BYTES = BN * B_CH * 16;
+    constexpr int A_IT = (AR * A_SL + NT - 1) / NT, B_IT = (BN * B_CH + NT - 1) / NT;
+    constexpr bool A_PART = (AR * A_SL) % NT != 0;
     constexpr bool B_PART = (BN * B_CH) % NT != 0;
     constexpr int R = TM * 32, CN = TN * 32;
     constexpr int ES = (WGM * WGN * R * (CN + 4) * 4 <= 150 * 1024) ? 1 : (TN % 2 == 0 ? 2 : TN);
@@ -98,7 +100,7 @@
     static_assert(TN % ES == 0 && EPI <= 160 * 1024, "epilogue region");
     constexpr int SMEM = 2 * (A_BYTES + B_BYTES) > EPI ? 2 * (A_BYTES + B_BYTES) : EPI;
     constexpr unsigned OOB = 0xFFFFFFFFu;
-    static_assert(TM >= 1 && TN >= 1 && (BM * 8) % NT == 0 && (BN * B_CH) % 64 == 0 && SMEM <= 160 * 1024, "tile");
+    static_assert(TM >= 1 && TN >= 1 && (BM * A_SL) % 64 == 0 && (X3A || (BM * 8) % NT == 0) && (BN * B_CH) % 64 == 0 && SMEM <= 160 * 1024, "tile");
 
     __shared__ __attribute__((aligned(1024))) unsigned char smem[SMEM];
 
@@ -117,10 +119,10 @@
 #pragma unroll
     for (int it = 0; it < A_IT; ++it) {
         const int item = tid + it * NT;
-        const int row = item >> 3, slot = item & 7;
-        a_ch16[it] = (unsigned)((slot ^ ((row >> 1) & 7)) * 16);
+        const int row = item / A_SL, slot = item - row * A_SL;
+        a_ch16[it] = X3A ? (unsigned)(slot * 16) : (unsigned)((slot ^ ((row >> 1) & 7)) * 16);
         const int m = S3 ? m0 + row - 1 : m0 + row;
-        const bool ok = m >= 0 && m < p.M;
+        const bool ok = m >= 0 && m < p.M && !(X3A && slot == 12);
         const int mm = ok ? m : 0;
         const int img = mm / HoWo;
         const int rem = mm - img * HoWo;
@@ -182,14 +184,14 @@
         if (c0 + KC <= cur_cpg) {
 #pragma unroll
             for (int it = 0; it < A_IT; ++it)
-                if (!A_PART || it + 1 < A_IT || tid + it * NT < AR * 8)
+                if (!A_PART || it + 1 < A_IT || tid + it * NT < AR * A_SL)
                     __builtin_amdgcn_raw_ptr_buffer_load_lds(arsrc, (lds_void*)(sa + it * NT * 16), 16, a_off[it], soff, 0, 0);
         } else {
 #pragma unroll
             for (int it = 0; it < A_IT; ++it)
-                if (!A_PART || it + 1 < A_IT || tid + it * NT < AR * 8)
+                if (!A_PART || it + 1 < A_IT || tid + it * NT < AR * A_SL)
                     __builtin_amdgcn_raw_ptr_buffer_load_lds(arsrc, (lds_void*)(sa + it * NT * 16), 16,
-                                                             (c0 + (int)(a_ch16[it] / ESZ) < cur_cpg) ? a_off[it] : OOB, soff, 0, 0);
+                                                             (c0 + (int)(X3A ? a_ch16[it] / 48 * 8 : a_ch16[it] / ESZ) < cur_cpg) ? a_off[it] : OOB, soff, 0, 0);
         }
     };
     auto issue_b = [&](int stage, int step) {
@@ -243,7 +245,7 @@
 #pragma unroll
         for (int tm = 0; tm < TM; ++tm) {
             const int row = a_row[tm] + (S3 ? kxs : 0);
-            a_rd[tm] = row * 128;
+            a_rd[tm] = row * A_PITCH;
             a_key[tm] = (row >> 1) & 7;
             zero[tm] = S3 && ((kxs == 0 && !okl[tm]) || (kxs == 2 && !okr[tm]));
         }
@@ -253,9 +255,15 @@
                 const int q = 2 * kk + h;
                 bf16x8 ah[TM], am[TM], al[TM];
 #pragma unroll
-                for (int tm = 0; tm < TM; ++tm)
+                for (int tm = 0; tm < TM; ++tm) {
+                    if constexpr (X3A) {
+                        ah[tm] = *reinterpret_cast<const bf16x8*>(st + a_rd[tm] + q * 48);
+                        am[tm] = *reinterpret_cast<const bf16x8*>(st + a_rd[tm] + q * 48 + 16);
+                        al[tm] = *reinterpret_cast<const bf16x8*>(st + a_rd[tm] + q * 48 + 32);
+                    } else
                     split8(*reinterpret_cast<const f32x4*>(st + a_rd[tm] + (((2 * q) ^ a_key[tm]) << 4)),
                            *reinterpret_cast<const f32x4*>(st + a_rd[tm] + (((2 * q + 1) ^ a_key[tm]) << 4)), ah[tm], am[tm], al[tm]);
+                }
 #pragma unroll
                 for (int tn = 0; tn < TN; ++tn) {
                     const bf16x8 bh = *reinterpret_cast<const bf16x8*>(stb + b_rd[tn] + q * (BN * 16));
@@ -420,12 +428,15 @@
                 unsigned char* sa = smem + stage * A_BYTES + wave * 1024;
 #pragma unroll
                 for (int it = 0; it < A_IT; ++it) {
-                    const int L = 8 * step + t_c[it];
+                    if (A_PART && it + 1 == A_IT && tid + it * NT >= AR * A_SL) continue;
+                    const int oct = X3A ? t_c[it] / 3 : 0;
+                    const int L = X3A ? 2 * (4 * step + oct) : 8 * step + t_c[it];
                     const int tap = cq == 1 ? L : (int)__umulhi((unsigned)L, p.tp_magic_cq);
                     const int cc = L - tap * cq;
                     const int tky = (int)__umulhi((unsigned)tap, p.tp_magic), tkx = tap - tky * p.KW;
                     const bool ok = tap < KK && ((a_msk[it] >> tky) & (a_msk[it] >> (8 + tkx)) & 1u) != 0;
-                    const unsigned off = ok ? (unsigned)(a_pix[it] + tky * p.W + tkx) * sl0 + sc0 + (unsigned)cc * 16u : OOB;
+                    const unsigned in_row = X3A ? (unsigned)(cc * 24 + (t_c[it] - 3 * oct) * 16) : (unsigned)cc * 16u;
+                    const unsigned off = ok ? (unsigned)(a_pix[it] + tky * p.W + tkx) * sl0 + sc0 + in_row : OOB;
                     __builtin_amdgcn_raw_ptr_buffer_load_lds(arsrc, (lds_void*)(sa + it * NT * 16), 16, off, 0, 0, 0);
                 }
             };
@@ -814,7 +825,14 @@
         e2fgvi_set_error("conv2d_x: the row-shift tiles (11..17) are for 3x3 stride-1 pad-1 layers");
         return E2FGVI_EINVAL;
     }
-    if (mode == 1 || mode == 2) {
+    if (mode == 4) {
+        if constexpr (!S3 && BN == 128 && (BM == 64 || BM == 128) && WGM * WGN == 4) {
+            hipLaunchKernelGGL((conv_bf16x_kernel<BM, BN, WGM, WGN, false, 4>), dim3(p.tilesM * p.tilesN, groups, 1), dim3(64 * WGM * WGN), 0, st, p);
+        } else {
+            e2fgvi_set_error("conv2d_x: pre-split activations (E2FGVI_BF16X3A) run on tiles 1 (128x128) and 4 (64x128) only");
+            return E2FGVI_EUNSUP;
+        }
+    } else if (mode == 1 || mode == 2) {
         if constexpr (!S3) {
             if (mode == 2)
                 hipLaunchKernelGGL((conv_bf16x_kernel<BM, BN, WGM, WGN, false, 2>), dim3(p.tilesM * p.tilesN, groups, 1), dim3(64 * WGM * WGN), 0, st, p);
@@ -846,7 +864,8 @@
     return true;
 }
 
-static int mode_x(const char* who, int32_t code) {
+static int mode_x(const char* who, int32_t code, bool conv = false) {
+    if (conv && code == E2FGVI_BF16X3A) return 4;
     switch (code) {
         case E2FGVI_BF16: return 0;
         case E2FGVI_F32: return 1;
@@ -903,12 +922,13 @@
 }
 
 static int conv2d_x(const e2fgvi_convx_desc* d, void* stream, int mode) {
-    const bool f32 = mode == 1 || mode == 2;
+    const bool a3 = mode == 4;
+    const bool f32 = mode == 1 || mode == 2 || a3;
     const int dt16 = mode == 3 ? E2FGVI_F16 : E2FGVI_BF16;
     E2_REQUIRE(d, E2FGVI_EINVAL, "conv2d_x: null descriptor");
     PackX q;
-    const int esz = f32 ? 4 : 2;
-    const int wbytes_num = mode == 2 ? 6 : esz;
+    const int esz = a3 ? 6 : f32 ? 4 : 2;
+    const int wbytes_num = (mode == 2 || a3) ? 6 : esz;
     E2_REQUIRE(geometry_x(d->Cout, d->groups, d->KH, d->KW, d->nsrc, d->src_cpg, &q, f32), E2FGVI_EINVAL,
                "conv2d_x: bad geometry (channels per source must be multiples of 8 bf16 / 4 fp32)");
     E2_REQUIRE(d->N > 0 && d->H > 0 && d->W > 0 && d->Ho > 0 && d->Wo > 0 && d->stride > 0 && d->pad >= 0, E2FGVI_EINVAL,
@@ -939,6 +959,8 @@
         E2_REQUIRE(d->src[s], E2FGVI_EINVAL, "conv2d_x: null source %d", s);
         E2_REQUIRE(d->src_ld[s] % q.ch == 0 && d->src_coff[s] % q.ch == 0 && ((uintptr_t)d->src[s] & 15) == 0, E2FGVI_EINVAL,
                    "conv2d_x: source %d not 16-byte addressable (ld / coff multiples of 8 bf16 / 4 fp32)", s);
+        E2_REQUIRE(!a3 || (d->src_ld[s] % 8 == 0 && d->src_coff[s] % 8 == 0 && d->src_cpg[s] % 8 == 0), E2FGVI_EINVAL,
+                   "conv2d_x: pre-split source %d: ld / coff / channels per group in multiples of 8 (src_ld counts channels)", s);
         E2_REQUIRE(d->src_coff[s] + d->groups * d->src_cpg[s] <= d->src_ld[s], E2FGVI_EINVAL,
                    "conv2d_x: source %d channel range exceeds its pixel stride", s);
         const long long bytes = (long long)d->N * d->H * d->W * d->src_ld[s] * esz;
@@ -1037,6 +1059,6 @@
 }
 
 extern "C" int e2fgvi_conv2d_x(const e2fgvi_convx_desc* d, int32_t mode, void* stream) {
-    const int m = mode_x("conv2d_x", mode);
+    const int m = mode_x("conv2d_x", mode, true);
     return m < 0 ? E2FGVI_EINVAL : conv2d_x(d, stream, m);
 }
diff --git a/e2fgvi_amd/csrc/misc.hip b/e2fgvi_amd/csrc/misc.hip
--- a/e2fgvi_amd/csrc/misc.hip
+++ b/e2fgvi_amd/csrc/misc.hip
@@ -766,12 +766,85 @@
     return 0;
 }
 
+__global__ void split3_kernel(const float* __restrict__ src, unsigned short* __restrict__ a3, long long pixels, int C, int ld) {
+    const int oq = C / 8;
+    const long long idx = (long long)blockIdx.x * blockDim.x + threadIdx.x;
+    if (idx >= pixels * oq) return;
+    const long long pix = idx / oq;
+    const int o = (int)(idx - pix * oq);
+    const float* s = src + pix * ld + o * 8;
+    e2_bf16x8 hi, mid, lo;
+    e2_split8(*reinterpret_cast<const f32x4*>(s), *reinterpret_cast<const f32x4*>(s + 4), hi, mid, lo);
+    unsigned short* d = a3 + idx * 24;
+    *reinterpret_cast<e2_bf16x8*>(d) = hi;
+    *reinterpret_cast<e2_bf16x8*>(d + 8) = mid;
+    *reinterpret_cast<e2_bf16x8*>(d + 16) = lo;
+}
+
+extern "C" int e2fgvi_split3(const float* src, void* a3, int64_t pixels, int32_t C, int32_t ld, void* stream) {
+    E2_REQUIRE(src && a3 && pixels > 0 && C > 0 && C % 8 == 0 && ld >= C && ld % 4 == 0, E2FGVI_EINVAL,
+               "split3: null pointer, no pixels, or C not a multiple of 8 / ld not a multiple of 4 and >= C");
+    E2_REQUIRE(((uintptr_t)src & 15) == 0 && ((uintptr_t)a3 & 15) == 0, E2FGVI_EINVAL, "split3: buffers must be 16-byte aligned");
+    hipLaunchKernelGGL(split3_kernel, dim3(blocks_for(pixels * (C / 8))), dim3(NTH), 0, (hipStream_t)stream, src,
+                       (unsigned short*)a3, (long long)pixels, C, ld);
+    E2_LAUNCH_CHECK("split3");
+    return 0;
+}
+
+__global__ void fold_gelu_a3_kernel(const float* __restrict__ emb, unsigned short* __restrict__ a3, int F, int fh, int fw, int H,
+                                    int W, int C) {
+    const int oq = C / 8;
+    const long long idx = (long long)blockIdx.x * blockDim.x + threadIdx.x;
+    if (idx >= (long long)F * H * W * oq) return;
+    FlatIdx fi(idx, (long long)F * H * W * oq);
+    const int o = fi.pop(oq);
+    const int X = fi.pop(W);
+    const int Y = fi.pop(H);
+    const long long f = fi.rest();
+    int ly0, ly1, lx0, lx1;
+    fold_range(Y, fh, ly0, ly1);
+    fold_range(X, fw, lx0, lx1);
+    f32x4 acc[2] = {f32x4{0.f, 0.f, 0.f, 0.f}, f32x4{0.f, 0.f, 0.f, 0.f}};
+    const int row_len = 49 * C;
+    for (int ly = ly0; ly <= ly1; ++ly) {
+        const int ki = Y + 3 - 3 * ly;
+        for (int lx = lx0; lx <= lx1; ++lx) {
+            const int kj = X + 3 - 3 * lx;
+            f32x4 v[2];
+            ldf<2>(emb + ((f * fh + ly) * fw + lx) * row_len + (ki * 7 + kj) * C + o * 8, v);
+            acc[0] = acc[0] + v[0];
+            acc[1] = acc[1] + v[1];
+        }
+    }
+    const float cnt = (float)((ly1 - ly0 + 1) * (lx1 - lx0 + 1));
+#pragma unroll
+    for (int q = 0; q < 2; ++q) {
+        acc[q] = acc[q] / cnt;
+#pragma unroll
+        for (int e = 0; e < 4; ++e) acc[q][e] = e2_rounded(gelu_exact(acc[q][e]));
+    }
+    e2_bf16x8 hi, mid, lo;
+    e2_split8(acc[0], acc[1], hi, mid, lo);
+    unsigned short* d = a3 + idx * 24;
+    *reinterpret_cast<e2_bf16x8*>(d) = hi;
+    *reinterpret_cast<e2_bf16x8*>(d + 8) = mid;
+    *reinterpret_cast<e2_bf16x8*>(d + 16) = lo;
+}
+
 extern "C" int e2fgvi_ffn_fold(const void* hid, void* folded, int32_t dtype, int32_t gelu, int32_t F, int32_t fh, int32_t fw,
                                int32_t H, int32_t W, int32_t C, void* stream) {
     const char* name = gelu ? "ffn_fold_gelu" : "ffn_fold";
-    E2_REQUIRE(hid && folded && E2_DT_OK(dtype), E2FGVI_EINVAL, "%s: bad arguments", name);
+    E2_REQUIRE(hid && folded && (E2_DT_OK(dtype) || dtype == E2FGVI_BF16X3A), E2FGVI_EINVAL, "%s: bad arguments", name);
     if (int rc = check_fold(name, F, fh, fw, H, W, C)) return rc;
     E2_REQUIRE(dtype == E2FGVI_F32 || C % 8 == 0, E2FGVI_EINVAL, "%s: 16-bit needs C %% 8 == 0", name);
+    if (dtype == E2FGVI_BF16X3A) {
+        E2_REQUIRE(gelu && ((uintptr_t)hid & 15) == 0 && ((uintptr_t)folded & 15) == 0, E2FGVI_EINVAL,
+                   "ffn_fold: the pre-split output goes with gelu = 1 and 16-byte aligned buffers");
+        hipLaunchKernelGGL(fold_gelu_a3_kernel, dim3(blocks_for((long long)F * H * W * (C / 8))), dim3(NTH), 0, (hipStream_t)stream,
+                           (const float*)hid, (unsigned short*)folded, F, fh, fw, H, W, C);
+        E2_LAUNCH_CHECK(name);
+        return 0;
+    }
     const long long total = (long long)F * H * W * (C / (E2_DT16(dtype) ? 8 : 4));
     with_dtype(dtype, [&](auto z) {
         using T = E2_ELEM(z);
diff --git a/e2fgvi_amd/engine.py b/e2fgvi_amd/engine.py
--- a/e2fgvi_amd/engine.py
+++ b/e2fgvi_amd/engine.py
@@ -14,6 +14,7 @@
 if JOIN_AT not in (0, 10, 12, 14, 16, 18):
     raise ValueError("E2FGVI_JOIN_AT=%d: the join sits in front of encoder.layers.10 / 12 / 14 / 16 or behind the encoder (18)" % JOIN_AT)
 PROP_SPLIT = os.environ.get("E2FGVI_PROP_SPLIT", "1") != "0"
+A3_SS = os.environ.get("E2FGVI_X3A_SS", "0") == "1"
 
 
 def token_grid(h, w):
@@ -169,6 +170,7 @@
         self._zeros = {}
         self.overlap_flows = True
         self._side = None
+        self._a3_plans = {}
         self._given = None
         self.counters = {"encoder_frames": 0, "flow_pairs": 0, "decoder_frames": 0}
         torch.cuda.synchronize(self.device)
@@ -384,8 +386,21 @@
                           residual=loc.view(l_t * b, h, w, ch), out=loc.view(l_t * b, h, w, ch) if inplace else None)
         return out.view(l_t, b, h, w, ch)
 
+    def _a3(self, layer, N, H, W, **call):
+        if self.x16 or not ops.X3A_ENABLED:
+            return False
+        key = (id(layer), N, H, W)
+        if key not in self._a3_plans:
+            tile = layer.a3_plan(N, H, W, **call)
+            if torch.cuda.is_current_stream_capturing() or (ops.AUTOTUNE and not tile):
+                return bool(tile)
+            self._a3_plans[key] = bool(tile)
+        return self._a3_plans[key]
+
     def soft_split(self, feat):
-        return self.ss([feat], out_dtype=torch.float32)
+        N, H, W, _ = feat.shape
+        a3 = [ops.split3(feat)] if A3_SS and self._a3(self.ss, N, H, W) else None
+        return self.ss([feat], out_dtype=torch.float32, a3=a3)
 
     def block(self, i, x, b, t, fh, fw, hw, out2=None):
         blk = self.blocks[i]
@@ -402,15 +417,17 @@
         elif ops.attention_x3_applies(b, t, fh, fw):
             planes = torch.empty((3, rows + prow, 1024), dtype=torch.bfloat16, device=x.device)
             both = blk["qkv"](nbuf, kv_planes=planes)
-            att = ops.focal_attention_x3(both[:rows], planes, tab, nk, b, t, fh, fw)
+            att_a3 = self._a3(blk["proj"], rows, 1, 1, residual=True)
+            att = ops.focal_attention_x3(both[:rows], planes, tab, nk, b, t, fh, fw, a3=att_a3)
         else:
             both = blk["qkv"](nbuf)
             att = ops.focal_attention(both[:rows], both[rows:], tab, nk, b, t, fh, fw)
         x1 = blk["proj"](att, out_dtype=torch.float32, residual=x)
         n2 = ops.layernorm(x1, blk["n2w"], blk["n2b"], out_dtype=self.dtype)
         hid = blk["fc1"](n2)
-        folded = ops.ffn_fold_gelu(hid, b * t, fh, fw, H, W, 40)
-        if isinstance(blk["fc2"], PackedConvX):
+        fc2_conv = isinstance(blk["fc2"], PackedConvX)
+        folded = ops.ffn_fold_gelu(hid, b * t, fh, fw, H, W, 40, a3=fc2_conv and self._a3(blk["fc2"], b * t, H, W))
+        if fc2_conv:
             y = torch.empty((rows, 512), dtype=torch.float32, device=x.device)
             blk["fc2"]([folded], out=y.view(b * t, fh, fw, 512), residual=x1.view(b * t, fh, fw, 512),
                        out2=None if out2 is None else out2.view(b * t, fh, fw, 512))
diff --git a/e2fgvi_amd/lib.py b/e2fgvi_amd/lib.py
--- a/e2fgvi_amd/lib.py
+++ b/e2fgvi_amd/lib.py
@@ -10,6 +10,7 @@
 DT_F32, DT_BF16 = 0, 1
 DT_BF16X3 = 2
 DT_F16 = 3
+DT_BF16X3A = 4
 
 _fp = C.c_void_p
 
@@ -89,7 +90,9 @@
     "e2fgvi_pack_dcn_weight": (C.c_int, [_fp, _fp, _i32, _i32, _i32, _i32, _i32, _i32, _fp]),
     "e2fgvi_focal_attention": (C.c_int, [_fp, _fp, _fp, _i32, _fp, _fp, _i32, _i32, _i32, _i32, _i32, _fp]),
     "e2fgvi_split3_kv": (C.c_int, [_fp, _fp, _i64, _fp]),
+    "e2fgvi_split3": (C.c_int, [_fp, _fp, _i64, _i32, _i32, _fp]),
     "e2fgvi_focal_attention_x3": (C.c_int, [_fp, _fp, _fp, _i32, _fp, _fp, _i32, _i32, _i32, _i32, _i32, _fp]),
+    "e2fgvi_focal_attention_x3a": (C.c_int, [_fp, _fp, _fp, _i32, _fp, _fp, _i32, _i32, _i32, _i32, _i32, _i32, _fp]),
     "e2fgvi_nchw_to_nhwc": (C.c_int, [_fp, _fp, _i32, _i32, _i32, _i32, _i32, _i32, _f, _f, _fp]),
     "e2fgvi_nhwc_to_nchw": (C.c_int, [_fp, _i32, _fp, _i32, _i32, _i32, _i32, _fp]),
     "e2fgvi_resize_bilinear": (C.c_int, [_fp, _i32, _i32, _i32, _fp, _i32, _i32, _i32, _i32, _i32, _i32, _i32, _i32, _fp, _fp, _fp]),
diff --git a/e2fgvi_amd/ops.py b/e2fgvi_amd/ops.py
--- a/e2fgvi_amd/ops.py
+++ b/e2fgvi_amd/ops.py
@@ -40,6 +40,8 @@
 XTUNE_ROWSHIFT = (11, 16, 17, 12, 13, 18)
 X3_ENABLED = os.environ.get("E2FGVI_X3", "1") != "0"
 X3_MARGIN = 0.97
+X3A_ENABLED = X3_ENABLED and os.environ.get("E2FGVI_X3A", "1") != "0"
+X3A_TILES = (1, 4)
 X3_BASE = 30000
 W3_BASE = 40000
 W3_CANDIDATES = (132, 164, 32, 5132, 6064)
@@ -291,7 +293,7 @@
 
 
 _Plan = collections.namedtuple("_Plan", "family tile static from_table use_wino")
-_Call = collections.namedtuple("_Call", "d srcs kw kv_planes")
+_Call = collections.namedtuple("_Call", "d srcs kw kv_planes a3", defaults=(None,))
 
 
 class PackedConv(_ConvLayer):
@@ -430,12 +432,19 @@
             N, H, W, cin_g * self.groups, self.Cout, self.KH, self.stride, self.groups), macs=macs, issued=issued, tile=asked)
 
     def __call__(self, sources, out=None, out_coff=0, residual=None, res_coff=0, act=ACT_NONE, slope=0.0,
-                 out_nchw=False, tile=0, kv_planes=None, out_dtype=None):
+                 out_nchw=False, tile=0, kv_planes=None, out_dtype=None, a3=None):
         if out_dtype not in (None, torch.float32):
             raise ValueError("PackedConv writes fp32 results")
         srcs, out = self._srcs_out(sources, out, out_nchw, torch.float32)
         N, H, W, _ = srcs[0][0].shape
         kw = dict(out_coff=out_coff, res_coff=res_coff, act=act, slope=slope, out_nchw=out_nchw)
+        if all(t.dtype == torch.bfloat16 for t, _ in srcs):
+            t3 = tile or self.a3_plan(N, H, W, residual is not None, act)
+            if not (t3 in X3A_TILES and self._alt3() is not None):
+                raise ValueError("%s: pre-split sources, but the call's plan is not the split-operand GEMM on a tile with an A3 form" % self.name)
+            self.alt3(srcs, out=out, residual=residual, tile=t3, planes=kv_planes,
+                      split_from=(self.Cout - kv_planes.shape[2]) if kv_planes is not None else 0, **kw)
+            return out
         chunks = list(_image_chunks(N, max(H * W * t.shape[3] * 4 for t, _ in srcs)))
         if len(chunks) > 1:
             for n0, n1 in chunks:
@@ -443,7 +452,7 @@
                      tile=tile, **kw)
         else:
             kw.update(out=out, residual=residual)
-            call = _Call(self._desc(srcs, **kw), srcs, kw, kv_planes)
+            call = _Call(self._desc(srcs, **kw), srcs, kw, kv_planes, a3)
             if self._launch(call, self._select(call, tile)):
                 return out
         if kv_planes is not None:
@@ -470,8 +479,7 @@
         x3 = self.try_x3 and X3_ENABLED
         if not (tile == 0 and (static == 0 or not self.tune) and (self.tune or x3) and N * Ho * Wo >= 2048):
             return plan
-        key = (self.Cout, tuple(self.cpg), self.KH, self.KW, self.stride, self.pad, self.groups, self.bk,
-               int(4.0 * math.log2(N * Ho * Wo)), residual is not None, kw["act"], use_wino, bool(self.tune), int(static)) + (("x3",) if x3 else ())
+        key = self._table_key(N * Ho * Wo, residual is not None, kw["act"], use_wino, static, x3)
         best = _decision(key)
         from_table = best is not None
         if best is None and AUTOTUNE and not torch.cuda.is_current_stream_capturing() and (
@@ -482,8 +490,21 @@
             plan = plan._replace(family=family, tile=arg)
         return plan._replace(from_table=from_table)
 
+    def _table_key(self, M, has_res, act, use_wino, static, x3):
+        return (self.Cout, tuple(self.cpg), self.KH, self.KW, self.stride, self.pad, self.groups, self.bk,
+                int(4.0 * math.log2(M)), has_res, act, use_wino, bool(self.tune), int(static)) + (("x3",) if x3 else ())
+
+    def a3_plan(self, N, H, W, residual=False, act=ACT_NONE):
+        Ho, Wo = self.out_hw(H, W)
+        x3 = self.try_x3 and X3_ENABLED
+        use_wino = self.algo == "winograd" or (self.algo == "auto" and H % 2 == 0 and W % 2 == 0)
+        if not (X3A_ENABLED and x3 and not use_wino and N * Ho * Wo >= 2048 and not any(c % 8 for c in self.cpg)):
+            return 0
+        family, tile = _decode(_decision(self._table_key(N * Ho * Wo, bool(residual), act, False, 0, x3)) or 0)
+        return tile if family == "x3" and tile in X3A_TILES else 0
+
     def _tune(self, call, own, use_wino, x3):
-        d, srcs, kw, kv_planes = call
+        d, srcs, kw, kv_planes = call[:4]
         best = self._autotune(d, use_wino) if self.tune else own[1]
         base = own if own[0] == "w4" else ("own", best)
         mine = None
@@ -552,10 +573,12 @@
         return lib.e2fgvi_conv2d_nhwc(C.byref(d), st), "conv2d_nhwc"
 
     def _launch(self, call, plan):
-        d, srcs, kw, kv_planes = call
+        d, srcs, kw, kv_planes = call[:4]
         family, tile = plan.family, plan.tile
         try:
             if family == "x3" and self._alt3() is not None:
+                if call.a3 is not None and X3A_ENABLED and tile in X3A_TILES:
+                    srcs = [(a, c) for a, (_, c) in zip(call.a3, srcs)]
                 self.alt3(srcs, tile=tile, planes=kv_planes, split_from=(self.Cout - kv_planes.shape[2]) if kv_planes is not None else 0,
                           **kw)
                 return True
@@ -621,6 +644,7 @@
         self._mode = mode = _L.DT_BF16X3 if self.x3 else _DT_CODE[dtype]
         conv2d_x = lib.e2fgvi_conv2d_x
         self._fn = lambda desc_ref, stream: conv2d_x(desc_ref, mode, stream)
+        self._fn_a3 = lambda desc_ref, stream: conv2d_x(desc_ref, _L.DT_BF16X3A, stream)
         self._w_raw = w if (self.f32 and not self.x3) else None
         self._taps_arg = taps
         self.taps = (len(self.cpg) == 1 and groups == 1 and self.cpg[0] <= 56 and self.KW > 1
@@ -653,8 +677,13 @@
         return _lazy(vars(self), "alt3", self.name + " (split-operand GEMM alternative)",
                      lambda: self._x_alternative(taps=self._taps_arg, x3=True))
 
-    def _desc(self, srcs, out, out_coff, residual, res_coff, act, slope, out2, out_nchw):
-        d = self._fill(_L.ConvXDesc(), self.dtype, _chk_any, srcs, out, out_coff, act, slope, out_nchw)
+    def _desc(self, srcs, out, out_coff, residual, res_coff, act, slope, out2, out_nchw, a3=False):
+        d = self._fill(_L.ConvXDesc(), torch.bfloat16 if a3 else self.dtype, _chk_any, srcs, out, out_coff, act, slope, out_nchw)
+        if a3:
+            for i, (t, coff) in enumerate(srcs):
+                if t.shape[3] % 24 or coff % 8 or self.cpg[i] % 8:
+                    raise ValueError("pre-split source %d: [N, H, W, 3 C] bf16 with C, the channel offset and cpg in multiples of 8" % i)
+                d.src_ld[i] = t.shape[3] // 3
         d.wpacked = None if self._wp is None else self._wp.data_ptr()
         d.dst_dtype = _dt(out)
         if out2 is not None:
@@ -684,7 +713,16 @@
         N, H, W, _ = srcs[0][0].shape
         Ho, Wo = self.out_hw(H, W)
         kw = dict(out_coff=out_coff, res_coff=res_coff, act=act, slope=slope, out_nchw=out_nchw)
-        chunks = list(_image_chunks(N, max(H * W * t.shape[3] * (4 if self.f32 else 2) for t, _ in srcs)))
+        a3 = self.f32 and all(t.dtype == torch.bfloat16 for t, _ in srcs)
+        if a3 and not self.x3:
+            t3 = tile or self.a3_plan(N, H, W, out_dtype=out.dtype, out_nchw=out_nchw)
+            if not (t3 in X3A_TILES and self._alt3() is not None):
+                raise ValueError("%s: pre-split sources, but the call's plan is not the split-operand GEMM on a tile with an A3 form" % self.name)
+            return self.alt3(srcs, out=out, out_dtype=out_dtype, residual=residual, out2=out2, tile=t3, planes=planes,
+                             split_from=split_from, **kw)
+        if a3 and tile and tile not in X3A_TILES:
+            raise ValueError("%s: pre-split sources run on tiles %s only" % (self.name, (X3A_TILES,)))
+        chunks = list(_image_chunks(N, max(H * W * t.shape[3] * t.element_size() for t, _ in srcs)))
         if len(chunks) > 1:
             if planes is not None:
                 raise ValueError("split planes: the batch spans >= 4 GiB (call in chunks)")
@@ -693,10 +731,11 @@
                      out2=None if out2 is None else out2[n0:n1], tile=tile, **kw)
             return out
         kw.update(out=out, residual=residual, out2=out2)
-        d = self._desc(srcs, **kw)
+        d = self._desc(srcs, a3=a3, **kw)
+        fn = self._fn_a3 if a3 else self._fn
         if planes is not None:
             self._set_planes(d, planes, split_from, N * Ho * Wo)
-        if tile == 0 and self.tune and N * Ho * Wo >= 2048:
+        if tile == 0 and self.tune and N * Ho * Wo >= 2048 and not a3:
             family, tile = self._select(d, srcs, kw)
             if family == "x3":
                 try:
@@ -705,20 +744,32 @@
                     tile = 0
         d.tile = tile
         if _L.TRACE is not None:
-            _L.annotate(**self._work(d))
+            _L.annotate(**self._work(d, a3))
         d.wpacked = self.wpacked.data_ptr()
-        rc = self._fn(C.byref(d), _stream())
-        if rc != 0 and d.tile and self.tune:
+        rc = fn(C.byref(d), _stream())
+        if rc != 0 and d.tile and self.tune and not a3:
             d.tile = 0
-            rc = self._fn(C.byref(d), _stream())
+            rc = fn(C.byref(d), _stream())
         _L.check(rc, "conv2d_x")
         return out
+
+    def _table_key(self, M, out_key, out_nchw, x3):
+        return (("x3" if self.x3 else ("x32+3" if x3 else "x32")) if self.f32 else "x", self.Cout, tuple(self.cpg), self.KH, self.KW, self.stride, self.pad, self.groups,
+                int(4.0 * math.log2(M)), out_key, out_nchw, self.taps)
+
+    def a3_plan(self, N, H, W, out_dtype=torch.float32, out_nchw=False):
+        Ho, Wo = self.out_hw(H, W)
+        x3 = self.try_x3 and X3_ENABLED and self.f32 and not self.x3
+        if not (X3A_ENABLED and x3 and self.tune and N * Ho * Wo >= 2048 and not any(c % 8 for c in self.cpg)):
+            return 0
+        out_key = _L.DT_BF16 if out_dtype == torch.float16 else _DT_CODE[out_dtype]
+        family, tile = _decode(_decision(self._table_key(N * Ho * Wo, out_key, out_nchw, x3)) or 0)
+        return tile if family == "x3" and tile in X3A_TILES else 0
 
     def _select(self, d, srcs, kw):
         out, residual = kw["out"], kw["residual"]
         x3 = self.try_x3 and X3_ENABLED and self.f32 and not self.x3
-        key = (("x3" if self.x3 else ("x32+3" if x3 else "x32")) if self.f32 else "x", self.Cout, tuple(self.cpg), self.KH, self.KW, self.stride, self.pad, self.groups,
-               int(4.0 * math.log2(d.N * d.Ho * d.Wo)), _dt_key(out), kw["out_nchw"], self.taps)
+        key = self._table_key(d.N * d.Ho * d.Wo, _dt_key(out), kw["out_nchw"], x3)
         best = _decision(key)
         if best is None and AUTOTUNE and not torch.cuda.is_current_stream_capturing() and (
                 residual is None or residual.data_ptr() != out.data_ptr()):
@@ -736,14 +787,14 @@
                 best = X3_BASE + min(res3, key=res3.get)
         return best
 
-    def _work(self, d):
+    def _work(self, d, a3=False):
         N, H, W, Ho, Wo, tile = d.N, d.H, d.W, d.Ho, d.Wo, d.tile
         cin_g, cout_g, K2 = sum(self.cpg), self.Cout // self.groups, self.KH * self.KW
         kc = 32 if self.f32 else 64
         cin_p = sum(-(-c // kc) * kc for c in self.cpg)
         if self.taps:
             cin_p = -(-K2 * (self.cpg[0] // (4 if self.f32 else 8)) // 8) * kc / K2
-        return dict(layer=self.name, kernel="conv_%s tile=%d%s" % (("f32x3" if self.x3 else "f32x") if self.f32 else
+        return dict(layer=self.name, kernel="conv_%s tile=%d%s" % (("f32x3a" if a3 else "f32x3" if self.x3 else "f32x") if self.f32 else
                                                                    "f16x" if self.f16 else "bf16x", tile, " taps" if self.taps else ""),
                     shape="N%d %dx%d %d->%d k%d s%d g%d" % (N, H, W, cin_g * self.groups, self.Cout, self.KH, self.stride, self.groups),
                     macs=N * Ho * Wo * self.Cout * cin_g * K2, tile=int(tile),
@@ -863,17 +914,18 @@
     def __init__(self, weight, bias, bk=None, precision="fp32"):
         super().__init__(weight, bias, [weight.shape[1]], bk=bk, precision=precision)
 
-    def __call__(self, x, out=None, residual=None, act=ACT_NONE, slope=0.0, tile=0, kv_planes=None, out_dtype=None):
+    def __call__(self, x, out=None, residual=None, act=ACT_NONE, slope=0.0, tile=0, kv_planes=None, out_dtype=None, a3=None):
         if out_dtype not in (None, torch.float32):
             raise ValueError("PackedLinear writes fp32 results")
-        _chk(x, "x")
+        _chk(x, "x", torch.bfloat16 if x.dtype == torch.bfloat16 else torch.float32)
         rows = x.numel() // x.shape[-1]
         x4 = x.view(rows, 1, 1, x.shape[-1])
         if out is None:
             out = torch.empty((rows, self.Cout), dtype=torch.float32, device=x.device)
         o4 = out.view(rows, 1, 1, out.shape[-1])
         r4 = None if residual is None else residual.view(rows, 1, 1, residual.shape[-1])
-        super().__call__([x4], out=o4, residual=r4, act=act, slope=slope, tile=tile, kv_planes=kv_planes)
+        super().__call__([x4], out=o4, residual=r4, act=act, slope=slope, tile=tile, kv_planes=kv_planes,
+                         a3=None if a3 is None else [a3.view(rows, 1, 1, a3.shape[-1])])
         return out
 
 
@@ -1041,7 +1093,22 @@
     return out
 
 
-def focal_attention_x3(qkv, planes, key_tab, nkeys, B, T, fh, fw, out=None, waves=0):
+def split3(x, out=None):
+    lib = _L.load()
+    _chk(x, "x")
+    Cc = x.shape[-1]
+    if Cc % 8:
+        raise ValueError("split3: channels in multiples of 8")
+    if out is None:
+        out = torch.empty(tuple(x.shape[:-1]) + (3 * Cc,), dtype=torch.bfloat16, device=x.device)
+    _chk(out, "a3", torch.bfloat16)
+    if out.numel() != 3 * x.numel():
+        raise ValueError("split3: out must hold 3 bf16 per element")
+    _L.check(lib.e2fgvi_split3(_ptr(x), _ptr(out), x.numel() // Cc, Cc, Cc, _stream()), "split3")
+    return out
+
+
+def focal_attention_x3(qkv, planes, key_tab, nkeys, B, T, fh, fw, out=None, waves=0, a3=False):
     lib = _L.load()
     _chk(qkv, "qkv"); _chk(planes, "planes", torch.bfloat16)
     _chk(key_tab, "key_tab", torch.int32); _chk(nkeys, "nkeys", torch.int32)
@@ -1054,14 +1121,16 @@
     if key_tab.shape[0] != nwin or nkeys.shape[0] != nwin:
         raise ValueError("key table must have %d rows" % nwin)
     if out is None:
-        out = torch.empty((rows, 512), dtype=torch.float32, device=qkv.device)
-    _chk(out, "out")
+        out = torch.empty((rows, 1536 if a3 else 512), dtype=torch.bfloat16 if a3 else torch.float32, device=qkv.device)
+    _chk(out, "out", torch.bfloat16 if a3 else torch.float32)
+    if tuple(out.shape) != (rows, 1536 if a3 else 512):
+        raise ValueError("out must be [%d,%d]" % (rows, 1536 if a3 else 512))
     if _L.TRACE is not None:
         work = _attn_work(B, T, fh, fw, nkeys)
         work["issued"] = int(work["issued"] * 6 * 157.3 / 2500.0)
         _L.annotate(layer="attention", kernel="focal_attn_x3", **work)
-    _L.check(lib.e2fgvi_focal_attention_x3(_ptr(qkv), _ptr(planes), _ptr(key_tab), key_tab.shape[1], _ptr(nkeys), _ptr(out),
-                                           B, T, fh, fw, waves, _stream()), "focal_attention_x3")
+    _L.check(lib.e2fgvi_focal_attention_x3a(_ptr(qkv), _ptr(planes), _ptr(key_tab), key_tab.shape[1], _ptr(nkeys), _ptr(out),
+                                            _L.DT_BF16X3A if a3 else _L.DT_F32, B, T, fh, fw, waves, _stream()), "focal_attention_x3")
     return out
 
 
@@ -1240,11 +1309,13 @@
     return out
 
 
-def _ffn_fold(hid, F_, fh, fw, H, W, Cc, gelu):
+def _ffn_fold(hid, F_, fh, fw, H, W, Cc, gelu, a3=False):
     lib = _L.load()
     _chk_any(hid, "hid")
-    out = torch.empty((F_, H, W, Cc), dtype=hid.dtype, device=hid.device)
-    _L.check(lib.e2fgvi_ffn_fold(_ptr(hid), _ptr(out), _dt(hid), gelu, F_, fh, fw, H, W, Cc, _stream()),
+    if a3 and (hid.dtype != torch.float32 or Cc % 8):
+        raise ValueError("ffn_fold: the pre-split output is for fp32 rows of C % 8 == 0 channels")
+    out = torch.empty((F_, H, W, 3 * Cc if a3 else Cc), dtype=torch.bfloat16 if a3 else hid.dtype, device=hid.device)
+    _L.check(lib.e2fgvi_ffn_fold(_ptr(hid), _ptr(out), _L.DT_BF16X3A if a3 else _dt(hid), gelu, F_, fh, fw, H, W, Cc, _stream()),
              "ffn_fold_gelu" if gelu else "ffn_fold")
     return out
 
@@ -1253,8 +1324,8 @@
     return _ffn_fold(hid, F_, fh, fw, H, W, Cc, 0)
 
 
-def ffn_fold_gelu(hid, F_, fh, fw, H, W, Cc):
-    return _ffn_fold(hid, F_, fh, fw, H, W, Cc, 1)
+def ffn_fold_gelu(hid, F_, fh, fw, H, W, Cc, a3=False):
+    return _ffn_fold(hid, F_, fh, fw, H, W, Cc, 1, a3)
 
 
 def _ffn_unfold(folded, fh, fw, out, gelu):
diff --git a/include/e2fgvi_hip.h b/include/e2fgvi_hip.h
--- a/include/e2fgvi_hip.h
+++ b/include/e2fgvi_hip.h
@@ -68,6 +68,8 @@
 #define E2FGVI_BF16X3 2
 #define E2FGVI_F16 3
 
+#define E2FGVI_BF16X3A 4
+
 const char* e2fgvi_last_error(void);
 int e2fgvi_abi_version(void);
 
@@ -189,6 +191,7 @@
                          void* dst, int32_t dtype, int32_t F, int32_t fh, int32_t fw, int32_t H, int32_t W,
                          int32_t C, void* stream);
 int e2fgvi_cast(const void* src, int32_t src_dtype, void* dst, int32_t dst_dtype, int64_t n, void* stream);
+int e2fgvi_split3(const float* src, void* a3, int64_t pixels, int32_t C, int32_t ld, void* stream);
 
 typedef struct {
     const void* src[E2FGVI_MAX_SRC];
@@ -234,6 +237,9 @@
 int e2fgvi_split3_kv(const float* qkv_rows, void* planes, int64_t rows, void* stream);
 int e2fgvi_focal_attention_x3(const float* qkv, const void* planes, const int32_t* key_tab, int32_t tab_ld, const int32_t* nkeys,
                               float* out, int32_t B, int32_t T, int32_t fh, int32_t fw, int32_t waves, void* stream);
+int e2fgvi_focal_attention_x3a(const float* qkv, const void* planes, const int32_t* key_tab, int32_t tab_ld, const int32_t* nkeys,
+                               void* out, int32_t out_dtype, int32_t B, int32_t T, int32_t fh, int32_t fw, int32_t waves,
+                               void* stream);
 
 int e2fgvi_focal_attention_16(const void* qkv, const void* kv_pool, const int32_t* key_tab, int32_t tab_ld,
                               const int32_t* nkeys, void* out, int32_t dtype, int32_t B, int32_t T, int32_t fh, int32_t fw,
```

Result: slower. 934.5 frames/s (-3.3%).
